# cherubicXN/neat

Measured on AMD Instinct MI355X. Metric: ray-samples/s (train step) on ABC-neat-a, higher is better.
Workload: dtype bf16; 1 GPU; C2: abc-neat-a networks, 1024 rays x 128 samples per GPU, depth samples given, train step = forward + loss + backward + Adam; rays_per_gpu=1024, samples_per_ray=128, global_rays=1024, parallelism=dp1, weights=synthetic 'rough' (seed 42), launch=hip graph replay, the whole step one launch (forward + loss + backward + Adam)

## Files before the change

include/neat_hip.h:

```cpp
#ifndef NEAT_HIP_H
#define NEAT_HIP_H
#include <stddef.h>
#ifdef __cplusplus
extern "C" {
#endif

#define NEAT_NUM_LAYERS 19
#define NEAT_FEATURE 256

typedef struct neat_net_params {
  const float* v[NEAT_NUM_LAYERS];
  const float* g[NEAT_NUM_LAYERS];
  const float* b[NEAT_NUM_LAYERS];
} neat_net_params;

typedef struct neat_net_grads {
  float* dv[NEAT_NUM_LAYERS];
  float* dg[NEAT_NUM_LAYERS];
  float* db[NEAT_NUM_LAYERS];
} neat_net_grads;

int neat_abi_version(void);

#define NEAT_F32 0
#define NEAT_BF16 1
#define NEAT_BF16X3 2
#define NEAT_F16 3
#define NEAT_F16X3 4
#define NEAT_F16X3_FASTVALUES 5

size_t neat_packed_floats(int precision);
int neat_pack_weights(const neat_net_params* net, float* packed, int precision, void* stream);

int neat_camera_rays(const float* uv, const float* pose, const float* K, int kstride, int R, float* dirs, float* origins ,
                     void* stream);
int neat_eik_points(const float* uniform, const float* origins, const float* dirs, const float* z_eik, const float* extra, int R, int J,
                    float* out, const float* z, int S, const long long* idx, void* stream);

size_t neat_sdf_ws_floats(int P, int mode, int precision);
int neat_sdf_forward(const float* packed, const neat_net_params* net, const float* x, int P, int mode, int precision,
                     float radius, float scale, float* ws,
                     float* out257, float* sdf, float* feat, float* grad, void* stream);
int neat_sdf_backward(const float* packed, const neat_net_params* net, float* ws, int P, int precision,
                      const float* d_out257, const float* d_sdf, const float* d_feat, const float* d_grad,
                      const neat_net_grads* grads, void* stream);
int neat_sdf_backward_x(const float* packed, const neat_net_params* net, float* ws, int P, int precision, float scale,
                        const float* d_out257, const float* d_sdf, const float* d_feat, const float* d_grad,
                        const neat_net_grads* grads, float* d_x, void* stream);

size_t neat_heads_ws_floats(int P, int precision);
int neat_heads_forward(const float* packed, const neat_net_params* net, const float* points, const float* normals,
                       const float* view_dirs, const float* feats, int P, int precision, float* ws,
                       float* rgb, float* lines, void* stream);

size_t neat_render_ws_floats(int R, int S, int E, int precision);
int neat_render_forward(const float* packed, const neat_net_params* net, const float* origins, const float* dirs,
                        const float* z, int R, int S, int precision, const float* beta, float beta_min, float radius, float scale, float* ws,
                        float* points, float* weights, float* sdf, float* rgb, float* lines3d, float* depth,
                        float* xyz, float* normal_map, const float* eik_points, int E, float* eik_grad, void* stream);
int neat_render_backward(const float* packed, const neat_net_params* net, float* ws, const float* dirs,
                         const float* z, int R, int S, int E, int precision, const float* beta, float beta_min,
                         const float* d_rgb, const float* d_lines3d, const float* d_depth, const float* d_xyz,
                         const float* d_eik_grad, const float* d_acc, const neat_net_grads* grads, float* dbeta_ray, float* dbeta, void* stream);

size_t neat_render_eval_ws_floats(int R, int S, int precision);
int neat_render_forward_eval(const float* packed, const neat_net_params* net, const float* origins, const float* dirs,
                             const float* z, int R, int S, int precision, const float* beta, float beta_min, float radius, float scale, float* ws,
                             float* points, float* weights, float* sdf, float* rgb, float* lines3d, float* depth,
                             float* xyz, float* normal_map, void* stream);

int neat_uniform_depths(const float* near_r, float near_s, const float* far_r, float far_s, const float* t, const float* rnd, int R, int N,
                        float* z, void* stream);

int neat_sample_pdf(const float* bins, const float* weights, int nb, int R, const float* u, int u_stride, int N, float* samples,
                    const float* z_merge, int nz, float* z_out, void* stream);

int neat_sampler_bound(const float* z, int n, int R, const float* sdf_old, const float* sdf_new, const int* order, int n_old,
                       const float* beta_in, const float* beta0, float eps, int iters, float* sdf_out, float* beta_out,
                       int* flag, void* stream);
int neat_sampler_resample(const float* z, const float* sdf, int n, int R, const float* beta, int refine, float add_tiny,
                          const float* u, int u_stride, int N, float* samples, float* z_merged, int* order, void* stream);
int neat_sampler_finish(const float* samples, int N, const float* z, int n, const int* pick, int n_extra, float near, float far,
                        int R, const int* eik_idx, float* z_vals, float* z_eik, void* stream);

int neat_sdf_values_gated(const float* packed, const neat_net_params* net, const float* x, int P, int precision, float radius,
                          float scale, float* ws, float* sdf, const int* gate, int gate_value, void* stream);
int neat_sdf_values_rays(const float* packed, const neat_net_params* net, const float* origins, const float* dirs, const float* z, int R,
                         int S, int precision, float radius, float scale, float* ws, float* sdf, const int* gate, int gate_value,
                         void* stream);
int neat_sampler_init(const float* z, int R, int n, const float* beta, float beta_min, float beta_c, float* beta0, float* beta_ray,
                      int* ctl, int nctl, void* stream);
int neat_sampler_bound_dev(const float* z, int n, int R, const float* sdf_old, const float* sdf_new, const int* order, int n_old,
                           const float* beta_in, const float* beta0, float eps, int iters, float* sdf_out, float* beta_out,
                           int* open, const int* gate, int gate_value, void* stream);
int neat_sampler_resample_dev(const float* z, const float* sdf, int n, int R, const float* beta, float add_tiny,
                              const float* u_refine, int N_refine, float* samples_refine, float* z_merged, int* order,
                              const float* u_final, int u_final_stride, int N_final, float* samples_final, float* z_final, int ld_final,
                              int* n_final, const int* open, int* cont, int round, int max_rounds, void* stream);
int neat_sampler_finish_dev(const float* samples, int N, const float* z_final, int ld_final, const int* n_final, const float* keys,
                            int n_extra, int* pick, float near, float far, int R, const int* eik_idx, float* z_vals, float* z_eik,
                            void* stream);

int neat_sdf_ldp(int P, int precision);
int neat_sdf_values_laid_out(const float* packed, const neat_net_params* net, int P, int precision, float radius, float scale, float* ws,
                             float* sdf, const int* gate, int gate_value, void* stream);
int neat_sampler_init_rays(const float* z, int R, int n, const float* beta, float beta_min, float beta_c, float* beta0, float* beta_ray,
                           int* ctl, int nctl, const float* origins, const float* dirs, float* x_fm, int ldp, const float* keys, int n_step,
                           int n_cand, int n_extra, int* pick_all, void* stream);
int neat_sampler_round(const float* z, int n, int R, const float* sdf_old, const float* sdf_new, const int* order, int n_old,
                       const float* beta_in, const float* beta0, float eps, int iters, float* sdf_out, float* beta_out, int* ctl, int round,
                       int max_rounds, float add_tiny, const float* u_refine, int N_refine, float* samples_refine, float* z_merged,
                       int* order_out, const float* origins, const float* dirs, float* x_fm, int ldp, const float* u_final,
                       int u_final_stride, int N_final, float* samples_final, float* z_final, int ld_final, void* stream);
int neat_sampler_finish_picked(const float* samples, int N, const float* z_final, int ld_final, const int* n_final, const int* pick_all,
                               int n_step, int n_extra, float near, float far, int R, const int* eik_idx, float* z_vals, float* z_eik,
                               void* stream);

int neat_encode_lines(const float* lines, int N, int H, int W, float* lmap, int* label, unsigned char* valid, void* stream);

int neat_gather_batch(const int* pool, int npool, const long long* draw, int n, int W, const float* att, const float* rgb, const int* labels,
                      const float* lines, int nlines, float* uv, float* uv_proj, float* rgb_out, float* lines_out, long long* labels_out,
                      long long* pixel_out, void* stream);

int neat_copy_batch(const void* const* src, void* const* dst, const long long* nbytes, int n, void* stream);

int neat_l3d(const float* x, const float* o, const float* d, const float* normal, int R, float* l3d, void* stream);
int neat_junction_cost(const float* cand2d, const float* gt2d, int V, int C, float* cost, void* stream);
int neat_junction_gate(const long long* rows, const long long* cols, int K, const float* cost, int C, const float* cand3d,
                       const float* cand2d, const float* cand2d_calib, int use_median, float* median, unsigned char* good, float* j3d,
                       float* j2d, float* j2d_calib, void* stream);
int neat_loss_terms(const float* rgb, const float* rgb_gt, int R, const float* gtheta, int E, const float* loc3, const float* loc2c, int K,
                    const float* glo3, const float* glo2c, int J, float* scal, float* d_rgb, float* d_gtheta, float* pair_cost,
                    float eik_grad_scale, void* stream);
int neat_loss_lines_terms(const float* pred_px, const float* pred_calib, const float* gt5, const float* Kmat, int L, float threshold, float* out3,
                          float* d_pred_calib, float grad_scale, const float* rgb, const float* rgb_gt, int R, const float* gtheta, int E,
                          const float* loc3, const float* loc2c, int K, const float* glo3, const float* glo2c, int J, float* scal, float* d_rgb,
                          float* d_gtheta, float* pair_cost, float eik_grad_scale, const float* w2c, const float* lines3d, float* d_lines3d,
                          void* stream);
int neat_loss_pairs(const long long* ri, const long long* ci, const int* n_match, int Kmax, const float* loc3, const float* loc2c,
                    const float* loc2, const float* glo3, const float* glo2c, const float* glo2, int J, const float* pair_cost, float* scal,
                    float* d_glo3, float* d_glo2c, const float* line_loss, float w_eik, float w_line, float w_j3, float w_j2, int weighted_grads,
                    float* total, const float* w2c, void* stream);
int neat_ffn_forward(const float* x, int J, const float* W0, const float* b0, const float* W1, const float* b1, const float* W2,
                     const float* b2, float* h1, float* h2, float* y, void* stream);
int neat_ffn_backward(const float* x, int J, const float* W0, const float* W1, const float* W2, const float* h1, const float* h2,
                      const float* dy, float* ws2, float* dx, float* dW0, float* db0, float* dW1, float* db1, float* dW2, float* db2,
                      void* stream);
int neat_inv_small(const float* A, int n, int lda, float* out, void* stream);
int neat_camera_mats(const float* pose, const float* K, int kstride, float* w2c, float* K3, void* stream);
int neat_project2d(const float* K, const float* w2c, const float* X, int N, float* uv, void* stream);
int neat_project2d_backward(const float* K, const float* w2c, const float* X, int N, const float* d_uv, float* d_X, void* stream);
int neat_camera_setup(const float* uv, const float* uv2, const float* pose, const float* K, int kstride, int R, float* dirs, float* origins,
                      float* dirs2, float* w2c, float* K3, void* stream);
int neat_project2d_pair(const float* K, const float* K2, const float* w2c, const float* X, int N, float* uv, float* uv2, void* stream);
int neat_line_loss(const float* pred, const float* gt, const float* weight, int R, float threshold, float* out2, float* per_line,
                   float* d_pred, void* stream);
int neat_line_losses(const float* pred_px, const float* pred_calib, const float* gt5, const float* K, int R, float threshold, float* out3,
                     float* d_pred_calib, float grad_scale, void* stream);

int neat_adam_step(float* params, const float* const* grads, const long long* seg_offsets, const int* seg_steps, int nseg,
                   float* exp_avg, float* exp_avg_sq, float lr, float beta1, float beta2, float eps, void* stream);
int neat_adam_step_coef(float* params, const float* const* grads, const long long* seg_offsets, int nseg, float* exp_avg, float* exp_avg_sq,
                        const float* coef, float beta1, float beta2, float eps, void* stream);

size_t neat_lsap_ws_bytes(int nr, int nc);
int neat_lsap(const float* cost, int nr, int nc, const unsigned char* row_mask, const unsigned char* col_mask, long long* row_ind,
              long long* col_ind, int* n_match, void* ws, void* stream);

size_t neat_dbscan_ws_bytes(int n);
int neat_dbscan_means(const float* points, int n, double eps, float* centres, unsigned char* valid, int* count, void* ws, void* stream);

int neat_parse_match(const float* lines2d, int n, const float* gt, int m, int gt_stride, float threshold, int* label, float* mindis,
                     void* stream);
size_t neat_parse_group_ws_bytes(int n, int m);
int neat_parse_group(const int* label, const float* lines3d, const float* l3d, int n, int m, float* lines, float* scores, int* count,
                     void* ws, void* stream);
size_t neat_parse_vote_ws_bytes(int J, int mcap);
int neat_parse_vote(const float* junctions, int J, const float* lines, const int* count, int mcap, float threshold, int view, int* votes,
                    int* first, void* ws, void* stream);
size_t neat_parse_graph_ws_bytes(int V, int mcap, int J);
int neat_parse_graph(const float* vlines, const float* vscores, const int* vcount, int V, int mcap, float score_threshold,
                     const float* junctions, const int* votes, const int* first, int J, float* lines_out, float* junc_out,
                     unsigned char* graph, int* pairs, float* wfi, int ecap, int* counts, void* ws, void* stream);
size_t neat_parse_visibility_ws_bytes(int ecap, int V);
int neat_parse_visibility(const float* lines, const int* n_lines, int ecap, const float* gt, int gt_stride, const int* gt_off,
                          const float* K3, const float* w2c, int V, float ckdist, int ckview, int* vis_count, float* checked,
                          int* n_checked, void* ws, void* stream);

int neat_grid_points(float* x_fm, int ldp, long long first_node, int count, const int* n, const double* b0, const double* b1, void* stream);
size_t neat_mesh_ws_bytes(int nx, int ny, int nz);
int neat_mesh_count(const float* grid, int nx, int ny, int nz, float level, void* ws, int* counts, void* stream);
int neat_mesh_emit(const float* grid, int nx, int ny, int nz, const double* b0, const double* b1, float level, void* ws, float* verts, int nv,
                   int* faces, int nf, void* stream);
int neat_unit_rows3(float* g, int n, void* stream);

int neat_volume_weights(const float* z, const float* sdf, int R, int S, const float* beta, float* weights, void* stream);

int neat_set_tuning(int key, int value);
int neat_prof_enable(int on);
int neat_prof_collect(int cls, double* total_ms, double* total_flops, int* launches, double* total_bytes);

#ifdef __cplusplus
}
#endif
#endif
```

neat_amd/_lib.py:

```python
import ctypes
import os

NUM_LAYERS = 19
ABI_VERSION = 15
PRECISIONS = {"fp32": 0, "bf16": 1, "bf16x3": 2, "fp16": 3, "fp16x3": 4}
_HERE = os.path.dirname(os.path.abspath(__file__))
LIB_PATH = os.environ.get("NEAT_HIP_LIB") or os.path.join(_HERE, "csrc", "libneat_hip.so")

c_fp = ctypes.c_void_p


class NetParams(ctypes.Structure):
    _fields_ = [("v", c_fp * NUM_LAYERS), ("g", c_fp * NUM_LAYERS), ("b", c_fp * NUM_LAYERS)]


class NetGrads(ctypes.Structure):
    _fields_ = [("dv", c_fp * NUM_LAYERS), ("dg", c_fp * NUM_LAYERS), ("db", c_fp * NUM_LAYERS)]


_SIGNATURES = {
    "neat_abi_version": (ctypes.c_int, []),
    "neat_packed_floats": (ctypes.c_size_t, [ctypes.c_int]),
    "neat_pack_weights": (ctypes.c_int, [ctypes.POINTER(NetParams), c_fp, ctypes.c_int, c_fp]),
    "neat_eik_points": (ctypes.c_int, [c_fp, c_fp, c_fp, c_fp, c_fp, ctypes.c_int, ctypes.c_int, c_fp, c_fp, ctypes.c_int, c_fp, c_fp]),
    "neat_camera_rays": (ctypes.c_int, [c_fp, c_fp, c_fp, ctypes.c_int, ctypes.c_int, c_fp, c_fp, c_fp]),
    "neat_sdf_ws_floats": (ctypes.c_size_t, [ctypes.c_int, ctypes.c_int, ctypes.c_int]),
    "neat_sdf_forward": (ctypes.c_int, [c_fp, ctypes.POINTER(NetParams), c_fp, ctypes.c_int, ctypes.c_int, ctypes.c_int,
                                        ctypes.c_float, ctypes.c_float, c_fp, c_fp, c_fp, c_fp, c_fp, c_fp]),
    "neat_sdf_backward": (ctypes.c_int, [c_fp, ctypes.POINTER(NetParams), c_fp, ctypes.c_int, ctypes.c_int, c_fp, c_fp, c_fp, c_fp,
                                         ctypes.POINTER(NetGrads), c_fp]),
    "neat_sdf_backward_x": (ctypes.c_int, [c_fp, ctypes.POINTER(NetParams), c_fp, ctypes.c_int, ctypes.c_int, ctypes.c_float, c_fp, c_fp,
                                           c_fp, c_fp, ctypes.POINTER(NetGrads), c_fp, c_fp]),
    "neat_heads_ws_floats": (ctypes.c_size_t, [ctypes.c_int, ctypes.c_int]),
    "neat_heads_forward": (ctypes.c_int, [c_fp, ctypes.POINTER(NetParams), c_fp, c_fp, c_fp, c_fp, ctypes.c_int, ctypes.c_int, c_fp,
                                          c_fp, c_fp, c_fp]),
    "neat_render_ws_floats": (ctypes.c_size_t, [ctypes.c_int, ctypes.c_int, ctypes.c_int, ctypes.c_int]),
    "neat_render_forward": (ctypes.c_int, [c_fp, ctypes.POINTER(NetParams), c_fp, c_fp, c_fp, ctypes.c_int, ctypes.c_int, ctypes.c_int,
                                           c_fp, ctypes.c_float, ctypes.c_float, ctypes.c_float, c_fp,
                                           c_fp, c_fp, c_fp, c_fp, c_fp, c_fp, c_fp, c_fp, c_fp, ctypes.c_int, c_fp, c_fp]),
    "neat_render_eval_ws_floats": (ctypes.c_size_t, [ctypes.c_int, ctypes.c_int, ctypes.c_int]),
    "neat_render_forward_eval": (ctypes.c_int, [c_fp, ctypes.POINTER(NetParams), c_fp, c_fp, c_fp, ctypes.c_int, ctypes.c_int, ctypes.c_int,
                                                c_fp, ctypes.c_float, ctypes.c_float, ctypes.c_float, c_fp,
                                                c_fp, c_fp, c_fp, c_fp, c_fp, c_fp, c_fp, c_fp, c_fp]),
    "neat_render_backward": (ctypes.c_int, [c_fp, ctypes.POINTER(NetParams), c_fp, c_fp, c_fp, ctypes.c_int, ctypes.c_int, ctypes.c_int,
                                            ctypes.c_int, c_fp, ctypes.c_float, c_fp, c_fp, c_fp, c_fp, c_fp, c_fp, ctypes.POINTER(NetGrads), c_fp, c_fp,
                                            c_fp]),
    "neat_sampler_bound": (ctypes.c_int, [c_fp, ctypes.c_int, ctypes.c_int, c_fp, c_fp, c_fp, ctypes.c_int, c_fp, c_fp,
                                          ctypes.c_float, ctypes.c_int, c_fp, c_fp, c_fp, c_fp]),
    "neat_sampler_resample": (ctypes.c_int, [c_fp, c_fp, ctypes.c_int, ctypes.c_int, c_fp, ctypes.c_int, ctypes.c_float,
                                             c_fp, ctypes.c_int, ctypes.c_int, c_fp, c_fp, c_fp, c_fp]),
    "neat_sampler_finish": (ctypes.c_int, [c_fp, ctypes.c_int, c_fp, ctypes.c_int, c_fp, ctypes.c_int, ctypes.c_float,
                                           ctypes.c_float, ctypes.c_int, c_fp, c_fp, c_fp, c_fp]),
    "neat_sample_pdf": (ctypes.c_int, [c_fp, c_fp, ctypes.c_int, ctypes.c_int, c_fp, ctypes.c_int, ctypes.c_int, c_fp, c_fp, ctypes.c_int, c_fp, c_fp]),
    "neat_uniform_depths": (ctypes.c_int, [c_fp, ctypes.c_float, c_fp, ctypes.c_float, c_fp, c_fp, ctypes.c_int, ctypes.c_int, c_fp, c_fp]),
    "neat_sdf_values_gated": (ctypes.c_int, [c_fp, ctypes.POINTER(NetParams), c_fp, ctypes.c_int, ctypes.c_int, ctypes.c_float,
                                             ctypes.c_float, c_fp, c_fp, c_fp, ctypes.c_int, c_fp]),
    "neat_sdf_values_rays": (ctypes.c_int, [c_fp, ctypes.POINTER(NetParams), c_fp, c_fp, c_fp, ctypes.c_int, ctypes.c_int, ctypes.c_int,
                                            ctypes.c_float, ctypes.c_float, c_fp, c_fp, c_fp, ctypes.c_int, c_fp]),
    "neat_sampler_init": (ctypes.c_int, [c_fp, ctypes.c_int, ctypes.c_int, c_fp, ctypes.c_float, ctypes.c_float, c_fp, c_fp, c_fp, ctypes.c_int,
                                         c_fp]),
    "neat_sampler_bound_dev": (ctypes.c_int, [c_fp, ctypes.c_int, ctypes.c_int, c_fp, c_fp, c_fp, ctypes.c_int, c_fp, c_fp,
                                              ctypes.c_float, ctypes.c_int, c_fp, c_fp, c_fp, c_fp, ctypes.c_int, c_fp]),
    "neat_sampler_resample_dev": (ctypes.c_int, [c_fp, c_fp, ctypes.c_int, ctypes.c_int, c_fp, ctypes.c_float,
                                                 c_fp, ctypes.c_int, c_fp, c_fp, c_fp,
                                                 c_fp, ctypes.c_int, ctypes.c_int, c_fp, c_fp, ctypes.c_int,
                                                 c_fp, c_fp, c_fp, ctypes.c_int, ctypes.c_int, c_fp]),
    "neat_sampler_finish_dev": (ctypes.c_int, [c_fp, ctypes.c_int, c_fp, ctypes.c_int, c_fp, c_fp, ctypes.c_int, c_fp, ctypes.c_float,
                                               ctypes.c_float, ctypes.c_int, c_fp, c_fp, c_fp, c_fp]),
    "neat_sdf_ldp": (ctypes.c_int, [ctypes.c_int, ctypes.c_int]),
    "neat_adam_step_coef": (ctypes.c_int, [c_fp, ctypes.POINTER(ctypes.c_void_p), ctypes.POINTER(ctypes.c_longlong), ctypes.c_int, c_fp, c_fp,
                                           c_fp, ctypes.c_float, ctypes.c_float, ctypes.c_float, c_fp]),
    "neat_loss_lines_terms": (ctypes.c_int, [c_fp, c_fp, c_fp, c_fp, ctypes.c_int, ctypes.c_float, c_fp, c_fp, ctypes.c_float,
                                             c_fp, c_fp, ctypes.c_int, c_fp, ctypes.c_int, c_fp, c_fp, ctypes.c_int, c_fp, c_fp, ctypes.c_int,
                                             c_fp, c_fp, c_fp, c_fp, ctypes.c_float, c_fp, c_fp, c_fp, c_fp]),
    "neat_camera_setup": (ctypes.c_int, [c_fp, c_fp, c_fp, c_fp, ctypes.c_int, ctypes.c_int, c_fp, c_fp, c_fp, c_fp, c_fp, c_fp]),
    "neat_project2d_pair": (ctypes.c_int, [c_fp, c_fp, c_fp, c_fp, ctypes.c_int, c_fp, c_fp, c_fp]),
    "neat_sdf_values_laid_out": (ctypes.c_int, [c_fp, ctypes.POINTER(NetParams), ctypes.c_int, ctypes.c_int, ctypes.c_float, ctypes.c_float, c_fp, c_fp, c_fp, ctypes.c_int, c_fp]),
    "neat_sampler_init_rays": (ctypes.c_int, [c_fp, ctypes.c_int, ctypes.c_int, c_fp, ctypes.c_float, ctypes.c_float, c_fp, c_fp, c_fp, ctypes.c_int, c_fp, c_fp, c_fp, ctypes.c_int, c_fp, ctypes.c_int, ctypes.c_int, ctypes.c_int, c_fp, c_fp]),
    "neat_sampler_round": (ctypes.c_int, [c_fp, ctypes.c_int, ctypes.c_int, c_fp, c_fp, c_fp, ctypes.c_int, c_fp, c_fp, ctypes.c_float, ctypes.c_int, c_fp, c_fp, c_fp, ctypes.c_int, ctypes.c_int, ctypes.c_float, c_fp, ctypes.c_int, c_fp, c_fp, c_fp, c_fp, c_fp, c_fp, ctypes.c_int, c_fp, ctypes.c_int, ctypes.c_int, c_fp, c_fp, ctypes.c_int, c_fp]),
    "neat_sampler_finish_picked": (ctypes.c_int, [c_fp, ctypes.c_int, c_fp, ctypes.c_int, c_fp, c_fp, ctypes.c_int, ctypes.c_int, ctypes.c_float, ctypes.c_float, ctypes.c_int, c_fp, c_fp, c_fp, c_fp]),
    "neat_encode_lines": (ctypes.c_int, [c_fp, ctypes.c_int, ctypes.c_int, ctypes.c_int, c_fp, c_fp, c_fp, c_fp]),
    "neat_gather_batch": (ctypes.c_int, [c_fp, ctypes.c_int, c_fp, ctypes.c_int, ctypes.c_int, c_fp, c_fp, c_fp, c_fp, ctypes.c_int,
                                         c_fp, c_fp, c_fp, c_fp, c_fp, c_fp, c_fp]),
    "neat_copy_batch": (ctypes.c_int, [c_fp, c_fp, c_fp, ctypes.c_int, c_fp]),
    "neat_ffn_forward": (ctypes.c_int, [c_fp, ctypes.c_int] + [c_fp] * 10),
    "neat_ffn_backward": (ctypes.c_int, [c_fp, ctypes.c_int] + [c_fp] * 15),
    "neat_l3d": (ctypes.c_int, [c_fp, c_fp, c_fp, c_fp, ctypes.c_int, c_fp, c_fp]),
    "neat_junction_cost": (ctypes.c_int, [c_fp, c_fp, ctypes.c_int, ctypes.c_int, c_fp, c_fp]),
    "neat_junction_gate": (ctypes.c_int, [c_fp, c_fp, ctypes.c_int, c_fp, ctypes.c_int, c_fp, c_fp, c_fp, ctypes.c_int, c_fp, c_fp, c_fp,
                                          c_fp, c_fp, c_fp]),
    "neat_loss_terms": (ctypes.c_int, [c_fp, c_fp, ctypes.c_int, c_fp, ctypes.c_int, c_fp, c_fp, ctypes.c_int, c_fp, c_fp, ctypes.c_int,
                                       c_fp, c_fp, c_fp, c_fp, ctypes.c_float, c_fp]),
    "neat_loss_pairs": (ctypes.c_int, [c_fp, c_fp, c_fp, ctypes.c_int, c_fp, c_fp, c_fp, c_fp, c_fp, c_fp, ctypes.c_int, c_fp, c_fp, c_fp,
                                       c_fp, c_fp, ctypes.c_float, ctypes.c_float, ctypes.c_float, ctypes.c_float, ctypes.c_int, c_fp, c_fp, c_fp]),
    "neat_camera_mats": (ctypes.c_int, [c_fp, c_fp, ctypes.c_int, c_fp, c_fp, c_fp]),
    "neat_inv_small": (ctypes.c_int, [c_fp, ctypes.c_int, ctypes.c_int, c_fp, c_fp]),
    "neat_project2d": (ctypes.c_int, [c_fp, c_fp, c_fp, ctypes.c_int, c_fp, c_fp]),
    "neat_project2d_backward": (ctypes.c_int, [c_fp, c_fp, c_fp, ctypes.c_int, c_fp, c_fp, c_fp]),
    "neat_line_loss": (ctypes.c_int, [c_fp, c_fp, c_fp, ctypes.c_int, ctypes.c_float, c_fp, c_fp, c_fp, c_fp]),
    "neat_line_losses": (ctypes.c_int, [c_fp, c_fp, c_fp, c_fp, ctypes.c_int, ctypes.c_float, c_fp, c_fp, ctypes.c_float, c_fp]),
    "neat_adam_step": (ctypes.c_int, [c_fp, ctypes.POINTER(ctypes.c_void_p), ctypes.POINTER(ctypes.c_longlong), ctypes.POINTER(ctypes.c_int),
                                      ctypes.c_int, c_fp, c_fp, ctypes.c_float, ctypes.c_float, ctypes.c_float, ctypes.c_float, c_fp]),
    "neat_lsap_ws_bytes": (ctypes.c_size_t, [ctypes.c_int, ctypes.c_int]),
    "neat_lsap": (ctypes.c_int, [c_fp, ctypes.c_int, ctypes.c_int, c_fp, c_fp, c_fp, c_fp, c_fp, c_fp, c_fp]),
    "neat_dbscan_ws_bytes": (ctypes.c_size_t, [ctypes.c_int]),
    "neat_dbscan_means": (ctypes.c_int, [c_fp, ctypes.c_int, ctypes.c_double, c_fp, c_fp, c_fp, c_fp, c_fp]),
    "neat_parse_match": (ctypes.c_int, [c_fp, ctypes.c_int, c_fp, ctypes.c_int, ctypes.c_int, ctypes.c_float, c_fp, c_fp, c_fp]),
    "neat_parse_group_ws_bytes": (ctypes.c_size_t, [ctypes.c_int, ctypes.c_int]),
    "neat_parse_group": (ctypes.c_int, [c_fp, c_fp, c_fp, ctypes.c_int, ctypes.c_int, c_fp, c_fp, c_fp, c_fp, c_fp]),
    "neat_parse_vote_ws_bytes": (ctypes.c_size_t, [ctypes.c_int, ctypes.c_int]),
    "neat_parse_vote": (ctypes.c_int, [c_fp, ctypes.c_int, c_fp, c_fp, ctypes.c_int, ctypes.c_float, ctypes.c_int, c_fp, c_fp, c_fp, c_fp]),
    "neat_parse_graph_ws_bytes": (ctypes.c_size_t, [ctypes.c_int, ctypes.c_int, ctypes.c_int]),
    "neat_parse_graph": (ctypes.c_int, [c_fp, c_fp, c_fp, ctypes.c_int, ctypes.c_int, ctypes.c_float, c_fp, c_fp, c_fp, ctypes.c_int,
                                        c_fp, c_fp, c_fp, c_fp, c_fp, ctypes.c_int, c_fp, c_fp, c_fp]),
    "neat_parse_visibility_ws_bytes": (ctypes.c_size_t, [ctypes.c_int, ctypes.c_int]),
    "neat_parse_visibility": (ctypes.c_int, [c_fp, c_fp, ctypes.c_int, c_fp, ctypes.c_int, c_fp, c_fp, c_fp, ctypes.c_int, ctypes.c_float,
                                             ctypes.c_int, c_fp, c_fp, c_fp, c_fp, c_fp]),
    "neat_grid_points": (ctypes.c_int, [c_fp, ctypes.c_int, ctypes.c_longlong, ctypes.c_int, ctypes.POINTER(ctypes.c_int),
                                        ctypes.POINTER(ctypes.c_double), ctypes.POINTER(ctypes.c_double), c_fp]),
    "neat_mesh_ws_bytes": (ctypes.c_size_t, [ctypes.c_int, ctypes.c_int, ctypes.c_int]),
    "neat_mesh_count": (ctypes.c_int, [c_fp, ctypes.c_int, ctypes.c_int, ctypes.c_int, ctypes.c_float, c_fp, c_fp, c_fp]),
    "neat_mesh_emit": (ctypes.c_int, [c_fp, ctypes.c_int, ctypes.c_int, ctypes.c_int, ctypes.POINTER(ctypes.c_double),
                                      ctypes.POINTER(ctypes.c_double), ctypes.c_float, c_fp, c_fp, ctypes.c_int, c_fp, ctypes.c_int, c_fp]),
    "neat_unit_rows3": (ctypes.c_int, [c_fp, ctypes.c_int, c_fp]),
    "neat_volume_weights": (ctypes.c_int, [c_fp, c_fp, ctypes.c_int, ctypes.c_int, c_fp, c_fp, c_fp]),
    "neat_set_tuning": (ctypes.c_int, [ctypes.c_int, ctypes.c_int]),
    "neat_prof_enable": (ctypes.c_int, [ctypes.c_int]),
    "neat_prof_collect": (ctypes.c_int, [ctypes.c_int, ctypes.POINTER(ctypes.c_double), ctypes.POINTER(ctypes.c_double),
                                         ctypes.POINTER(ctypes.c_int), ctypes.POINTER(ctypes.c_double)]),
}

_lib = None


def exported_symbols():
    return sorted(_SIGNATURES)


tuning_overrides = []


def lib():
    global _lib
    if _lib is None:
        if not os.path.exists(LIB_PATH):
            raise RuntimeError(
                f"{LIB_PATH} is missing: build it with `python -c 'import __graft_entry__ as g; g.build()'` "
                "(or neat_amd/csrc/build.sh).  neat_amd has no CPU/PyTorch fallback for the hot path.")
        l = ctypes.CDLL(LIB_PATH)
        for name, (res, args) in _SIGNATURES.items():
            fn = getattr(l, name)
            fn.restype, fn.argtypes = res, args
        _lib = l
        applied = []
        for kv in filter(None, os.environ.get("NEAT_TUNING", "").split(",")):
            k, v = kv.split("=")
            check(l.neat_set_tuning(int(k), int(v)), f"NEAT_TUNING {kv}")
            applied.append(kv)
        if applied:
            import sys
            print(f"[neat_amd] NEAT_TUNING overrides applied: {','.join(applied)}", file=sys.stderr, flush=True)
        global tuning_overrides
        tuning_overrides = applied
    return _lib


def check(code, what):
    if code != 0:
        raise RuntimeError(f"libneat_hip: {what} failed with code {code}")
```

neat_amd/csrc/kernels_junction.hpp:

```cpp
#pragma once
#include <hip/hip_runtime.h>
#include "device_util.hpp"

namespace neat {

constexpr int LSAP_WG = 1024;

struct LsapArgs {
  const float* cost;
  int nr, nc;
  const unsigned char* row_mask;
  long long* row_ind;
  long long* col_ind;
  int* n_match;
  double* wsd;
  int* wsi;
  int use_lds, lds_int_off;
  const unsigned char* col_mask;
  int cost_lds_off;
};

struct LsapKey { double val; int it; int un; };

__device__ __forceinline__ bool lsap_better(const LsapKey& a, const LsapKey& b) {
  if (a.it < 0) return false;
  if (b.it < 0) return true;
  if (a.val != b.val) return a.val < b.val;
  if (a.un != b.un) return a.un > b.un;
  return a.un ? a.it > b.it : a.it < b.it;
}

__device__ __forceinline__ LsapKey lsap_shfl_xor(const LsapKey& k, int m) {
  LsapKey o;
  o.val = __shfl_xor(k.val, m);
  o.it = __shfl_xor(k.it, m);
  o.un = __shfl_xor(k.un, m);
  return o;
}

template <class F>
__device__ int lsap_compact(int n, F flag, int* out, int* s_wave, int* s_base) {
  const int tid = threadIdx.x, lane = tid & 63, wave = tid >> 6, nw = blockDim.x >> 6;
  if (tid == 0) *s_base = 0;
  __syncthreads();
  for (int b0 = 0; b0 < n; b0 += blockDim.x) {
    const int i = b0 + tid;
    const bool f = i < n && flag(i);
    const unsigned long long bal = __ballot(f);
    const int before = __popcll(bal & ((1ull << lane) - 1ull));
    if (lane == 0) s_wave[wave] = __popcll(bal);
    __syncthreads();
    int off = *s_base;
    for (int w = 0; w < wave; ++w) off += s_wave[w];
    if (f) out[off + before] = i;
    __syncthreads();
    if (tid == 0) { int t = 0; for (int w = 0; w < nw; ++w) t += s_wave[w]; *s_base += t; }
    __syncthreads();
  }
  const int total = *s_base;
  __syncthreads();
  return total;
}

__global__ __launch_bounds__(LSAP_WG) void lsap_kernel(LsapArgs a) {
  __shared__ int s_wave[LSAP_WG / 64], s_base;
  __shared__ LsapKey s_key[LSAP_WG / 64];
  __shared__ int s_i, s_nrem, s_fail, s_done, s_nvis;
  __shared__ double s_minval;
  const int tid = threadIdx.x, nt = blockDim.x, lane = tid & 63, wave = tid >> 6, nw = nt >> 6;
  const int kmax = min(a.nr, a.nc);
  for (int k = tid; k < kmax; k += nt) { a.row_ind[k] = -1; a.col_ind[k] = -1; }

  extern __shared__ __attribute__((aligned(16))) unsigned char lsap_lds[];
  double* wsd = a.use_lds ? reinterpret_cast<double*>(lsap_lds) : a.wsd;
  int* wsi = a.use_lds ? reinterpret_cast<int*>(lsap_lds + a.lds_int_off) : a.wsi;
  int* rowlist = wsi;
  int* collist = rowlist + a.nr;
  const unsigned char* mask = a.row_mask;
  const unsigned char* cmask = a.col_mask;
  int n_eff, c_eff;
  if (!mask && !cmask) {
    for (int i = tid; i < a.nr; i += nt) rowlist[i] = i;
    for (int j = tid; j < a.nc; j += nt) collist[j] = j;
    n_eff = a.nr; c_eff = a.nc;
  } else {
    n_eff = lsap_compact(a.nr, [&](int i) { return mask ? mask[i] != 0 : true; }, rowlist, s_wave, &s_base);
    c_eff = lsap_compact(a.nc, [&](int j) { return cmask ? cmask[j] != 0 : true; }, collist, s_wave, &s_base);
  }
  const bool T = c_eff < n_eff;
  const int N = T ? c_eff : n_eff, M = T ? n_eff : c_eff;
  if (N == 0) { if (tid == 0) *a.n_match = 0; return; }
  double* u = wsd; double* v = u + N; double* sp = v + M;
  int* path = collist + a.nc; int* col4row = path + M; int* row4col = col4row + N; int* remaining = row4col + M;
  int* vis_row = remaining + M;
  int* vis_col = vis_row + N;
  int* tmp = vis_col + M;
  const float* C = a.cost;
  const int nc0 = a.nc;
  const bool staged = a.use_lds && a.cost_lds_off >= 0;
  const float* Cl = reinterpret_cast<const float*>(lsap_lds + (staged ? a.cost_lds_off : 0));
  if (staged) {
    float* dst = reinterpret_cast<float*>(lsap_lds + a.cost_lds_off);
    const int total = a.nr * a.nc;
    const int total4 = ((reinterpret_cast<size_t>(C) & 15) == 0) ? (total >> 2) : 0;
    const float4* C4 = reinterpret_cast<const float4*>(C);
    float4* d4 = reinterpret_cast<float4*>(dst);
    for (int e = tid; e < total4; e += 4 * nt) {
      float4 x[4];
#pragma unroll
      for (int q = 0; q < 4; ++q) if (e + q * nt < total4) x[q] = C4[e + q * nt];
#pragma unroll
      for (int q = 0; q < 4; ++q) if (e + q * nt < total4) d4[e + q * nt] = x[q];
    }
    for (int e = 4 * total4 + tid; e < total; e += nt) dst[e] = C[e];
  }
  const bool ident = !mask && !cmask;
  auto cost = [&](int i, int j) -> double {
    const int idx = ident ? (T ? j * nc0 + i : i * nc0 + j) : (T ? rowlist[j] * nc0 + collist[i] : rowlist[i] * nc0 + collist[j]);
    return (double)(staged ? Cl[idx] : C[idx]);
  };
  for (int i = tid; i < N; i += nt) { u[i] = 0.0; col4row[i] = -1; }
  for (int j = tid; j < M; j += nt) { v[j] = 0.0; row4col[j] = -1; }
  if (tid == 0) { s_fail = 0; s_done = 0; s_i = 0; s_nrem = M; s_minval = 0.0; s_nvis = 0; }
  __syncthreads();

  for (int cur = 0; cur < N; ++cur) {
    bool first = true;
    while (true) {
      const int i = s_i, nrem = s_nrem;
      const double minval = s_minval, ui = u[i];
      LsapKey best{INFINITY, -1, 0};
      if (first) {
        for (int it = tid; it < M; it += nt) {
          const int j = M - 1 - it;
          const double r = minval + cost(i, j) - ui - v[j];
          const bool lower = r < INFINITY;
          const double spj = lower ? r : INFINITY;
          sp[j] = spj;
          if (lower) path[j] = i;
          remaining[it] = j;
          LsapKey k{spj, it, row4col[j] == -1 ? 1 : 0};
          if (spj < INFINITY && lsap_better(k, best)) best = k;
        }
        first = false;
      } else {
        for (int it = tid; it < nrem; it += nt) {
          const int j = remaining[it];
          const double r = minval + cost(i, j) - ui - v[j];
          double spj = sp[j];
          if (r < spj) { path[j] = i; sp[j] = r; spj = r; }
          LsapKey k{spj, it, row4col[j] == -1 ? 1 : 0};
          if (spj < INFINITY && lsap_better(k, best)) best = k;
        }
      }
      for (int m = 32; m >= 1; m >>= 1) {
        LsapKey o = lsap_shfl_xor(best, m);
        if (lsap_better(o, best)) best = o;
      }
      if (lane == 0) s_key[wave] = best;
      __syncthreads();
      if (tid == 0) {
        LsapKey b = s_key[0];
        for (int w = 1; w < nw; ++w) if (lsap_better(s_key[w], b)) b = s_key[w];
        int nvis = s_nvis;
        vis_row[nvis] = i;
        if (b.it < 0) { s_fail = 1; s_done = N; }
        else {
          const double mv = b.val;
          const int j = remaining[b.it];
          vis_col[nvis] = j;
          ++nvis;
          remaining[b.it] = remaining[nrem - 1];
          if (row4col[j] != -1) { s_i = row4col[j]; s_minval = mv; s_nrem = nrem - 1; s_nvis = nvis; }
          else {
            for (int q = 0; q < nvis; ++q) {
              const int r_ = vis_row[q];
              if (r_ == cur) u[r_] += mv;
              else u[r_] += mv - sp[col4row[r_]];
            }
            for (int q = 0; q < nvis; ++q) { const int c_ = vis_col[q]; v[c_] -= mv - sp[c_]; }
            int jj = j;
            while (true) {
              const int ii = path[jj];
              row4col[jj] = ii;
              const int t = col4row[ii]; col4row[ii] = jj; jj = t;
              if (ii == cur) break;
            }
            s_done = cur + 1; s_i = cur + 1; s_nrem = M; s_minval = 0.0; s_nvis = 0;
          }
        }
      }
      __syncthreads();
      if (s_done > cur) break;
    }
    if (s_fail) break;
  }
  if (s_fail) { if (tid == 0) *a.n_match = -1; return; }
  if (!T) {
    for (int i = tid; i < N; i += nt) { a.row_ind[i] = rowlist[i]; a.col_ind[i] = collist[col4row[i]]; }
  } else {
    const int cnt = lsap_compact(M, [&](int k) { return row4col[k] != -1; }, tmp, s_wave, &s_base);
    for (int q = tid; q < cnt; q += nt) { const int k = tmp[q]; a.row_ind[q] = rowlist[k]; a.col_ind[q] = collist[row4col[k]]; }
  }
  if (tid == 0) *a.n_match = N;
}

#ifndef NEAT_ADAM_PASSES
#define NEAT_ADAM_PASSES 1
#endif
constexpr int ADAM_MAXSEG = 96, ADAM_PASSES = NEAT_ADAM_PASSES;
struct AdamSegs {
  const float* g[ADAM_MAXSEG]; long long off[ADAM_MAXSEG + 1]; float lr_over_bc1[ADAM_MAXSEG], inv_sqrt_bc2[ADAM_MAXSEG]; int nseg;
};

constexpr int ADAM_SEGS_KERNARG_OFFSET = 8;
__global__ void adam_flat_kernel(float* __restrict__ p, AdamSegs segs, float* __restrict__ m, float* __restrict__ v,
                                 long long n, float beta1, float beta2, float eps, const float* __restrict__ coef) {
  __shared__ long long s_off[ADAM_MAXSEG + 1];
  __shared__ const float* s_g[ADAM_MAXSEG];
  __shared__ float s_a1[ADAM_MAXSEG], s_a2[ADAM_MAXSEG];
  typedef const __attribute__((address_space(4))) char* karg_ptr;
  typedef const __attribute__((address_space(4))) AdamSegs* karg_segs;
  const karg_segs tab = (karg_segs)((karg_ptr)__builtin_amdgcn_kernarg_segment_ptr() + ADAM_SEGS_KERNARG_OFFSET);
  for (int t = threadIdx.x; t <= segs.nseg; t += blockDim.x) {
    s_off[t] = tab->off[t];
    if (t < segs.nseg) { s_g[t] = tab->g[t]; s_a1[t] = coef ? coef[2 * t] : tab->lr_over_bc1[t]; s_a2[t] = coef ? coef[2 * t + 1] : tab->inv_sqrt_bc2[t]; }
  }
  __syncthreads();
  for (int pass = 0; pass < ADAM_PASSES; ++pass) {
    const long long i0 = (((long long)blockIdx.x * ADAM_PASSES + pass) * blockDim.x + threadIdx.x) * 4;
    if (i0 >= n) return;
    int lo = 0, hi = segs.nseg - 1;
    while (lo < hi) { const int mid = (lo + hi + 1) >> 1; if (s_off[mid] <= i0) lo = mid; else hi = mid - 1; }
    const long long iend = i0 + 4 < n ? i0 + 4 : n;
    if (iend <= s_off[lo + 1] && iend == i0 + 4) {
      const float* gp = s_g[lo];
      if (!gp) continue;
      const float a1 = s_a1[lo], a2 = s_a2[lo];
      const float* gq = gp + (i0 - s_off[lo]);
      float4 mm = *reinterpret_cast<const float4*>(m + i0), vv = *reinterpret_cast<const float4*>(v + i0), pp = *reinterpret_cast<const float4*>(p + i0);
      float* me = reinterpret_cast<float*>(&mm); float* ve = reinterpret_cast<float*>(&vv); float* pe = reinterpret_cast<float*>(&pp);
      float ge[4];
      if ((reinterpret_cast<size_t>(gq) & 15) == 0) {
        const float4 g4 = *reinterpret_cast<const float4*>(gq);
        ge[0] = g4.x; ge[1] = g4.y; ge[2] = g4.z; ge[3] = g4.w;
      } else {
#pragma unroll
        for (int e = 0; e < 4; ++e) ge[e] = gq[e];
      }
#pragma unroll
      for (int e = 0; e < 4; ++e) {
        const float g = ge[e];
        me[e] = beta1 * me[e] + (1.0f - beta1) * g;
        ve[e] = beta2 * ve[e] + (1.0f - beta2) * g * g;
        pe[e] -= a1 * (me[e] / (sqrtf(ve[e]) * a2 + eps));
      }
      *reinterpret_cast<float4*>(m + i0) = mm; *reinterpret_cast<float4*>(v + i0) = vv; *reinterpret_cast<float4*>(p + i0) = pp;
      continue;
    }
    for (long long i = i0; i < iend; ++i) {
      while (i >= s_off[lo + 1]) ++lo;
      const float* gp = s_g[lo];
      if (!gp) continue;
      const float g = gp[i - s_off[lo]];
      const float mm = beta1 * m[i] + (1.0f - beta1) * g;
      const float vv = beta2 * v[i] + (1.0f - beta2) * g * g;
      m[i] = mm; v[i] = vv;
      p[i] -= s_a1[lo] * (mm / (sqrtf(vv) * s_a2[lo] + eps));
    }
  }
}

__device__ __forceinline__ void project_point(const float* K, const float* M, const float x[3], float cam[3], float& w) {
  float c[3];
#pragma unroll
  for (int i = 0; i < 3; ++i) c[i] = M[4 * i] * x[0] + M[4 * i + 1] * x[1] + M[4 * i + 2] * x[2] + M[4 * i + 3];
#pragma unroll
  for (int i = 0; i < 3; ++i) cam[i] = K[3 * i] * c[0] + K[3 * i + 1] * c[1] + K[3 * i + 2] * c[2];
  w = cam[2];
  if (fabsf(w) < 1e-8f) w += (w >= 0.0f) ? 1e-8f : -1e-8f;
}

__global__ void project2d_kernel(const float* __restrict__ K, const float* __restrict__ w2c, const float* __restrict__ X, int N,
                                 float* __restrict__ uv) {
  const int i = blockIdx.x * blockDim.x + threadIdx.x;
  if (i >= N) return;
  const float x[3] = {X[3 * i], X[3 * i + 1], X[3 * i + 2]};
  float cam[3], w;
  project_point(K, w2c, x, cam, w);
  uv[2 * i] = cam[0] / w; uv[2 * i + 1] = cam[1] / w;
}

__global__ void project2d_pair_kernel(const float* __restrict__ K, const float* __restrict__ K2, const float* __restrict__ w2c,
                                      const float* __restrict__ X, int N, float* __restrict__ uv, float* __restrict__ uv2) {
  const int i = blockIdx.x * blockDim.x + threadIdx.x;
  if (i >= N) return;
  const float x[3] = {X[3 * i], X[3 * i + 1], X[3 * i + 2]};
  float cam[3], w;
  project_point(K, w2c, x, cam, w);
  uv[2 * i] = cam[0] / w; uv[2 * i + 1] = cam[1] / w;
  project_point(K2, w2c, x, cam, w);
  uv2[2 * i] = cam[0] / w; uv2[2 * i + 1] = cam[1] / w;
}

__device__ __forceinline__ void project_bwd_point(const float* K, const float* w2c, const float x[3], float du, float dv, float dX[3]) {
  float cam[3], w;
  project_point(K, w2c, x, cam, w);
  const float dcam[3] = {du / w, dv / w, -(du * (cam[0] / w) + dv * (cam[1] / w)) / w};
  float dc[3];
#pragma unroll
  for (int j = 0; j < 3; ++j) dc[j] = K[j] * dcam[0] + K[3 + j] * dcam[1] + K[6 + j] * dcam[2];
#pragma unroll
  for (int j = 0; j < 3; ++j) dX[j] = w2c[j] * dc[0] + w2c[4 + j] * dc[1] + w2c[8 + j] * dc[2];
}
__global__ void project2d_bwd_kernel(const float* __restrict__ K, const float* __restrict__ w2c, const float* __restrict__ X, int N,
                                     const float* __restrict__ d_uv, float* __restrict__ d_X) {
  const int i = blockIdx.x * blockDim.x + threadIdx.x;
  if (i >= N) return;
  const float x[3] = {X[3 * i], X[3 * i + 1], X[3 * i + 2]};
  float dX[3];
  project_bwd_point(K, w2c, x, d_uv[2 * i], d_uv[2 * i + 1], dX);
#pragma unroll
  for (int j = 0; j < 3; ++j) d_X[3 * i + j] = dX[j];
}
__device__ __forceinline__ void project_bwd_calib(const float* w2c, const float x[3], float du, float dv, float dX[3]) {
  float I3[9] = {1.0f, 0.0f, 0.0f, 0.0f, 1.0f, 0.0f, 0.0f, 0.0f, 1.0f};
#pragma unroll
  for (int k = 0; k < 9; ++k) asm volatile("" : "+v"(I3[k]));
  project_bwd_point(I3, w2c, x, du, dv, dX);
}

__global__ __launch_bounds__(1024) void line_loss_kernel(const float* __restrict__ pred, const float* __restrict__ gt,
                                                         const float* __restrict__ weight, int R, float thr, float* __restrict__ out,
                                                         float* __restrict__ per_line, float* __restrict__ d_pred) {
  __shared__ float s_sum[16], s_cnt[16];
  __shared__ float s_inv;
  const int tid = threadIdx.x, lane = tid & 63, wave = tid >> 6;
  float sum = 0.0f, cnt = 0.0f;
  for (int r = tid; r < R; r += blockDim.x) {
    float p[4], g[4];
#pragma unroll
    for (int c = 0; c < 4; ++c) { p[c] = pred[4 * r + c]; g[c] = gt[4 * r + c]; }
    float ds = 0.0f, df = 0.0f;
#pragma unroll
    for (int c = 0; c < 4; ++c) { const float a = p[c] - g[c], b = p[c] - g[c ^ 2]; ds += a * a; df += b * b; }
    const bool straight = ds < df;
    float l = 0.0f;
#pragma unroll
    for (int c = 0; c < 4; ++c) l += fabsf(p[c] - (straight ? g[c] : g[c ^ 2]));
    l *= 0.25f;
    per_line[r] = l;
    if (l < thr) { sum += l * weight[r]; cnt += 1.0f; }
  }
  sum = wave_sum(sum); cnt = wave_sum(cnt);
  if (lane == 0) { s_sum[wave] = sum; s_cnt[wave] = cnt; }
  __syncthreads();
  if (tid == 0) {
    float a = 0.0f, b = 0.0f;
    for (int w = 0; w < (int)(blockDim.x >> 6); ++w) { a += s_sum[w]; b += s_cnt[w]; }
// ... 543 lines not shown
  __shared__ int lab[DBSCAN_MAXN];
  __shared__ int s_wave[16], s_base;
  const int tid = threadIdx.x, nt = blockDim.x;
  for (int i = tid; i < n; i += nt) lab[i] = dbscan_find(parent, i);
  const int maxc = n / 2;
  for (int k = tid; k < maxc; k += nt) { valid[k] = 0; centres[3 * k] = 0.f; centres[3 * k + 1] = 0.f; centres[3 * k + 2] = 0.f; }
  int* replist = reinterpret_cast<int*>(centres + 3 * maxc);
  if (tid == 0) s_base = 0;
  __syncthreads();
  const int lane = tid & 63, wave = tid >> 6, nw = nt >> 6;
  for (int b0 = 0; b0 < n; b0 += nt) {
    const int i = b0 + tid;
    const bool f = i < n && lab[i] == i && has_nb[i] != 0;
    const unsigned long long bal = __ballot(f);
    const int before = __popcll(bal & ((1ull << lane) - 1ull));
    if (lane == 0) s_wave[wave] = __popcll(bal);
    __syncthreads();
    int off = s_base;
    for (int w = 0; w < wave; ++w) off += s_wave[w];
    if (f) replist[off + before] = i;
    __syncthreads();
    if (tid == 0) { int t = 0; for (int w = 0; w < nw; ++w) t += s_wave[w]; s_base += t; }
    __syncthreads();
  }
  const int nclu = s_base;
  extern __shared__ __attribute__((aligned(8))) unsigned char dbscan_dyn[];
  if (mode == 2) {
    long long* sx = reinterpret_cast<long long*>(dbscan_dyn);
    long long* sy = sx + maxc; long long* sz = sy + maxc;
    int* cnt = reinterpret_cast<int*>(sz + maxc);
    int* rank = cnt + maxc;
    for (int k = tid; k < nclu; k += nt) { sx[k] = 0; sy[k] = 0; sz[k] = 0; cnt[k] = 0; rank[replist[k]] = k; }
    __syncthreads();
    for (int j = tid; j < n; j += nt) {
      if (has_nb[j] == 0) continue;
      const int k = rank[lab[j]];
      atomicAdd(reinterpret_cast<unsigned long long*>(&sx[k]), (unsigned long long)__double2ll_rn((double)pts[3 * j] * 4294967296.0));
      atomicAdd(reinterpret_cast<unsigned long long*>(&sy[k]), (unsigned long long)__double2ll_rn((double)pts[3 * j + 1] * 4294967296.0));
      atomicAdd(reinterpret_cast<unsigned long long*>(&sz[k]), (unsigned long long)__double2ll_rn((double)pts[3 * j + 2] * 4294967296.0));
      atomicAdd(&cnt[k], 1);
    }
    __syncthreads();
    for (int k = tid; k < nclu; k += nt) {
      const double inv = 1.0 / (4294967296.0 * (double)cnt[k]);
      centres[3 * k] = (float)((double)sx[k] * inv); centres[3 * k + 1] = (float)((double)sy[k] * inv); centres[3 * k + 2] = (float)((double)sz[k] * inv);
      valid[k] = 1;
    }
    if (tid == 0) *count = nclu;
    return;
  }
  float* dbscan_pts = reinterpret_cast<float*>(dbscan_dyn);
  const float* P = pts;
  if (mode == 1) {
    for (int i = tid; i < 3 * n; i += nt) dbscan_pts[i] = pts[i];
    P = dbscan_pts;
  }
  __syncthreads();
  for (int k = wave; k < nclu; k += nw) {
    const int r = replist[k];
    float sx = 0.f, sy = 0.f, sz = 0.f; int cnt = 0;
    for (int j = r + lane; j < n; j += 64) {
      const bool m = lab[j] == r;
      sx += m ? P[3 * j] : 0.0f; sy += m ? P[3 * j + 1] : 0.0f; sz += m ? P[3 * j + 2] : 0.0f; cnt += m ? 1 : 0;
    }
#pragma unroll
    for (int off = 32; off > 0; off >>= 1) {
      sx += __shfl_xor(sx, off); sy += __shfl_xor(sy, off); sz += __shfl_xor(sz, off); cnt += __shfl_xor(cnt, off);
    }
    if (lane == 0) {
      const float inv = 1.0f / (float)cnt;
      centres[3 * k] = sx * inv; centres[3 * k + 1] = sy * inv; centres[3 * k + 2] = sz * inv;
      valid[k] = 1;
    }
  }
  if (tid == 0) *count = nclu;
}

__device__ __forceinline__ float block_sum(float v, float* s_red) {
  v = wave_sum(v);
  const int lane = threadIdx.x & 63, wave = threadIdx.x >> 6;
  __syncthreads();
  if (lane == 0) s_red[wave] = v;
  __syncthreads();
  float t = 0.0f;
  for (int w = 0; w < (int)(blockDim.x >> 6); ++w) t += s_red[w];
  return t;
}

struct LossTermsArgs {
  const float* rgb; const float* rgb_gt; int R;
  const float* gtheta; int E;
  const float* loc3; const float* loc2c; int K;
  const float* glo3; const float* glo2c; int J;
  float* scal;
  float* d_rgb; float* d_gtheta; float* pair_cost;
  float eik_grad_scale;
};

__device__ __forceinline__ void loss_terms_body(const LossTermsArgs& a) {
  __shared__ float s_red[16];
  const int tid = threadIdx.x, nt = blockDim.x;
  float acc = 0.0f;
  const float inv_rgb = 1.0f / (float)(3 * a.R);
  for (int i = tid; i < 3 * a.R; i += nt) {
    const float d = a.rgb[i] - a.rgb_gt[i];
    acc += fabsf(d);
    a.d_rgb[i] = (d > 0.0f ? 1.0f : (d < 0.0f ? -1.0f : 0.0f)) * inv_rgb;
  }
  const float rgb_loss = block_sum(acc, s_red) * inv_rgb;
  acc = 0.0f;
  const float inv_e = a.E > 0 ? 1.0f / (float)a.E : 0.0f;
  for (int i = tid; i < a.E; i += nt) {
    const float gx = a.gtheta[3 * i], gy = a.gtheta[3 * i + 1], gz = a.gtheta[3 * i + 2];
    const float nrm = sqrtf(gx * gx + gy * gy + gz * gz);
    acc += (nrm - 1.0f) * (nrm - 1.0f);
    const float c = nrm > 0.0f ? (2.0f * (nrm - 1.0f) * inv_e / nrm) * a.eik_grad_scale : 0.0f;
    a.d_gtheta[3 * i] = c * gx; a.d_gtheta[3 * i + 1] = c * gy; a.d_gtheta[3 * i + 2] = c * gz;
  }
  const float eik = block_sum(acc, s_red) * inv_e;
  if (tid == 0) { a.scal[0] = rgb_loss; a.scal[1] = eik; }
  for (int idx = tid; idx < a.K * a.J; idx += nt) {
    const int k = idx / a.J, j = idx % a.J;
    float c3 = 0.0f, c2 = 0.0f;
#pragma unroll
    for (int c = 0; c < 3; ++c) c3 += fabsf(a.loc3[3 * k + c] - a.glo3[3 * j + c]);
#pragma unroll
    for (int c = 0; c < 2; ++c) c2 += fabsf(a.loc2c[2 * k + c] - a.glo2c[2 * j + c]);
    a.pair_cost[idx] = c3 + 0.1f * c2;
  }
}

__global__ __launch_bounds__(1024) void loss_terms_kernel(LossTermsArgs a) { loss_terms_body(a); }

struct LineLossesArgs { const float* pred_u; const float* pred_c; const float* gt5; const float* K; int R; float thr; float* out; float* d_pred_c; float grad_scale;
                        const float* w2c; const float* X3; float* d_X3; };
__global__ __launch_bounds__(1024) void loss_lines_terms_kernel(LineLossesArgs l, LossTermsArgs t) {
  if (blockIdx.x == 0) line_losses_body(l.pred_u, l.pred_c, l.gt5, l.K, l.R, l.thr, l.out, l.d_pred_c, l.grad_scale, l.w2c, l.X3, l.d_X3);
  else loss_terms_body(t);
}

struct LossPairsArgs {
  const long long* ri; const long long* ci; const int* n_match; int Kmax;
  const float* loc3; const float* loc2c; const float* loc2;
  const float* glo3; const float* glo2c; const float* glo2; int J;
  const float* pair_cost;
  float* scal;
  float* d_glo3; float* d_glo2c;
  const float* line_loss; float w_eik, w_line, w_j3, w_j2;
  int weighted_grads;
  float* total;
  const float* w2c;
};

__global__ __launch_bounds__(1024) void loss_pairs_kernel(LossPairsArgs a) {
  __shared__ float s_red[16];
  const int tid = threadIdx.x, nt = blockDim.x;
  for (int i = tid; i < 3 * a.J; i += nt) a.d_glo3[i] = 0.0f;
  for (int i = tid; i < 2 * a.J; i += nt) a.d_glo2c[i] = 0.0f;
  __syncthreads();
  const int n = max(*a.n_match, 0);
  const float inv = 1.0f / (float)max(n, 1);
  const float g3 = a.weighted_grads ? a.w_j3 : 1.0f, g2 = a.weighted_grads ? a.w_j2 : 1.0f;
  float s3 = 0.0f, s2 = 0.0f, spx = 0.0f, cnt = 0.0f;
  for (int q = tid; q < a.Kmax; q += nt) {
    const long long r = a.ri[q], c = a.ci[q];
    if (r < 0 || c < 0 || q >= n) continue;
#pragma unroll
    for (int e = 0; e < 3; ++e) {
      const float d = a.loc3[3 * r + e] - a.glo3[3 * c + e];
      s3 += fabsf(d);
      a.d_glo3[3 * c + e] = (-(d > 0.0f ? 1.0f : (d < 0.0f ? -1.0f : 0.0f)) * inv) * g3;
    }
#pragma unroll
    for (int e = 0; e < 2; ++e) {
      const float d = a.loc2c[2 * r + e] - a.glo2c[2 * c + e];
      s2 += fabsf(d);
      a.d_glo2c[2 * c + e] = (-(d > 0.0f ? 1.0f : (d < 0.0f ? -1.0f : 0.0f)) * inv) * g2;
      spx += fabsf(a.loc2[2 * r + e] - a.glo2[2 * c + e]);
    }
    if (a.pair_cost[r * a.J + c] < 10.0f) cnt += 1.0f;
  }
  s3 = block_sum(s3, s_red); s2 = block_sum(s2, s_red); spx = block_sum(spx, s_red); cnt = block_sum(cnt, s_red);
  if (a.w2c) {
    for (int j = tid; j < a.J; j += nt) {
      const float x[3] = {a.glo3[3 * j], a.glo3[3 * j + 1], a.glo3[3 * j + 2]};
      float dX[3];
      project_bwd_calib(a.w2c, x, a.d_glo2c[2 * j], a.d_glo2c[2 * j + 1], dX);
#pragma unroll
      for (int e = 0; e < 3; ++e) a.d_glo3[3 * j + e] += dX[e];
    }
  }
  if (tid == 0) {
    a.scal[2] = s3 * inv; a.scal[3] = s2 * inv; a.scal[4] = spx * inv; a.scal[5] = cnt;
    const float tot = a.scal[0] + a.w_eik * a.scal[1] + a.w_line * a.line_loss[0] + a.w_j3 * (s3 * inv) + a.w_j2 * (s2 * inv);
    a.scal[6] = tot;
    if (a.total) a.total[0] = tot;
  }
}

__global__ void l3d_kernel(const float* __restrict__ x, const float* __restrict__ o, const float* __restrict__ d,
                           const float* __restrict__ nrm, int R, float* __restrict__ l3d) {
  const int r = blockIdx.x * blockDim.x + threadIdx.x;
  if (r >= R) return;
  float den = 0.0f, num = 0.0f;
#pragma unroll
  for (int c = 0; c < 3; ++c) { den += d[3 * r + c] * nrm[3 * r + c]; num += (x[3 * r + c] - o[3 * r + c]) * nrm[3 * r + c]; }
  den += den >= 0.0f ? 1e-6f : -1e-6f;
  const float t = num / den;
#pragma unroll
  for (int c = 0; c < 3; ++c) l3d[3 * r + c] = o[3 * r + c] + d[3 * r + c] * t;
}

__global__ void junction_cost_kernel(const float* __restrict__ cand2d, const float* __restrict__ gt2d, int V, int C, float* __restrict__ cost) {
  const int idx = blockIdx.x * blockDim.x + threadIdx.x;
  if (idx >= V * C) return;
  const int v = idx / C, c = idx % C;
  const float dx = cand2d[2 * c] - gt2d[2 * v], dy = cand2d[2 * c + 1] - gt2d[2 * v + 1];
  cost[idx] = __fsqrt_rn(__fadd_rn(__fmul_rn(dx, dx), __fmul_rn(dy, dy)));
}

struct JunctionGateArgs {
  const long long* rows; const long long* cols; int K;
  const float* cost; int C;
  const float* cand3d; const float* cand2d; const float* cand2dc;
  int use_median;
  float* median;
  unsigned char* good;
  float* j3d; float* j2d; float* j2dc;
};

__global__ __launch_bounds__(1024) void junction_gate_kernel(JunctionGateArgs a) {
  __shared__ float s_m[2048];
  __shared__ int s_n;
  __shared__ float s_med;
  const int tid = threadIdx.x, nt = blockDim.x;
  if (tid == 0) { s_n = 0; s_med = 10.0f; }
  __syncthreads();
  for (int k = tid; k < a.K; k += nt) {
    const long long r = a.rows[k], c = a.cols[k];
    const bool ok = r >= 0 && c >= 0;
    s_m[k] = ok ? a.cost[r * a.C + c] : NAN;
    if (ok) atomicAdd(&s_n, 1);
  }
  __syncthreads();
  const int n = s_n;
  if (a.use_median && n > 0) {
    const int want = (n - 1) / 2;
    for (int k = tid; k < a.K; k += nt) {
      const float v = s_m[k];
      if (v != v) continue;
      int rank = 0;
      for (int j = 0; j < a.K; ++j) { const float w = s_m[j]; if (w == w && (w < v || (w == v && j < k))) ++rank; }
      if (rank == want) s_med = v;
    }
  }
  __syncthreads();
  const float thr = a.use_median ? s_med : 10.0f;
  if (tid == 0 && a.use_median) a.median[0] = s_med;
  for (int k = tid; k < a.K; k += nt) {
    const float v = s_m[k];
    const bool ok = v == v;
    a.good[k] = (ok && v < thr) ? 1 : 0;
    const long long c = ok ? a.cols[k] : 0;
#pragma unroll
    for (int e = 0; e < 3; ++e) a.j3d[3 * k + e] = ok ? a.cand3d[3 * c + e] : 0.0f;
#pragma unroll
    for (int e = 0; e < 2; ++e) { a.j2d[2 * k + e] = ok ? a.cand2d[2 * c + e] : 0.0f; a.j2dc[2 * k + e] = ok ? a.cand2dc[2 * c + e] : 0.0f; }
  }
}

}
```

neat_amd/csrc/neat_aux.hip:

```cpp
#include "kernels_sampler.hpp"
#include "kernels_junction.hpp"
#include "kernels_parse.hpp"
#include "kernels_mesh.hpp"
#include "../../include/neat_hip.h"
#include <algorithm>
#include <cmath>
#include <limits.h>
#include <math.h>

using namespace neat;

__attribute__((visibility("hidden"))) int neat_aux_set_tuning(int key, int value);

namespace {

int g_ffn_mfma = 1;
int g_sampler_ablate = 0;

#define NEAT_CHECK(expr) do { hipError_t e_ = (expr); if (e_ != hipSuccess) return (int)e_; } while (0)
inline dim3 grid1(int n, int b = 256) { return dim3((n + b - 1) / b); }

__global__ void volume_weights_kernel(const float* __restrict__ z, const float* __restrict__ sdf, int R, int S,
                                      const float* __restrict__ beta_ptr, float* __restrict__ weights) {
  const float beta = *beta_ptr;
  const int lane = threadIdx.x & 63;
  const int r = blockIdx.x * 4 + (threadIdx.x >> 6);
  if (r >= R) return;
  float carry = 0.0f;
  for (int i0 = 0; i0 < S; i0 += 64) {
    const int i = i0 + lane;
    const bool ok = i < S;
    const int p = r * S + (ok ? i : S - 1);
    const float delta = (i + 1 < S) ? z[p + 1] - z[p] : 1e10f;
    const float e = ok ? delta * laplace_sigma(sdf[p], beta) : 0.0f;
    const float incl = wave_incl_scan(e, lane);
    float excl = __shfl_up(incl, 1);
    if (lane == 0) excl = 0.0f;
    if (ok) weights[p] = (1.0f - expf(-e)) * expf(-(carry + excl));
    carry += __shfl(incl, 63);
  }
}

}

int neat_aux_set_tuning(int key, int value) {
  if (key == 28 && (value == 0 || value == 1)) { g_ffn_mfma = value; return 0; }
  if (key == 30 && value >= 0 && value <= 7) { g_sampler_ablate = value; return 0; }
  return -1;
}

extern "C" {

int neat_camera_rays(const float* uv, const float* pose, const float* K, int kstride, int R, float* dirs, float* origins, void* stream) {
  if (R <= 0) return 0;
  hipLaunchKernelGGL(camera_rays_kernel, grid1(R), dim3(256), 0, (hipStream_t)stream, uv, pose, K, kstride, R, dirs, origins);
  return (int)hipGetLastError();
}

int neat_eik_points(const float* uniform, const float* origins, const float* dirs, const float* z_eik, const float* extra, int R, int J,
                    float* out, const float* z, int S, const long long* idx, void* stream) {
  if (R <= 0 || J < 0) return R == 0 && J == 0 ? 0 : -1;
  if (!uniform || !origins || !dirs || !out || (J > 0 && !extra)) return -1;
  if (!z_eik && (!z || !idx || S <= 0)) return -1;
  hipLaunchKernelGGL(eik_points_kernel, grid1((2 * R + J) * 3), dim3(256), 0, (hipStream_t)stream, uniform, origins, dirs, z_eik, extra, R, J, out,
                     z, S, idx);
  return (int)hipGetLastError();
}

int neat_sampler_bound(const float* z, int n, int R, const float* sdf_old, const float* sdf_new, const int* order, int n_old,
                       const float* beta_in, const float* beta0, float eps, int iters, float* sdf_out, float* beta_out,
                       int* flag, void* stream) {
  if (R <= 0) return 0;
  if (n < 2 || n > SMAX || !z || !sdf_new || !beta_in || !beta0 || !sdf_out || !beta_out || !flag) return -1;
  SamplerBoundArgs a{z, n, R, sdf_old, sdf_new, order, n_old, beta_in, beta0, eps, iters, sdf_out, beta_out, flag, nullptr, 0};
  hipLaunchKernelGGL(sampler_bound_kernel, dim3(R), dim3(BOUND_T), 0, (hipStream_t)stream, a);
  return (int)hipGetLastError();
}

int neat_sampler_resample(const float* z, const float* sdf, int n, int R, const float* beta, int refine, float add_tiny,
                          const float* u, int u_stride, int N, float* samples, float* z_merged, int* order, void* stream) {
  if (R <= 0) return 0;
  if (n < 2 || n > SMAX || N < 1 || N > SMAX || !z || !sdf || !beta || !u || !samples || (refine && (!z_merged || !order))) return -1;
  SamplerResampleArgs a{};
  a.z = z; a.sdf = sdf; a.n = n; a.R = R; a.beta = beta; a.refine = refine; a.add_tiny = add_tiny; a.u = u; a.u_stride = u_stride; a.N = N;
  a.samples = samples; a.z_merged = z_merged; a.order = order;
  hipLaunchKernelGGL(sampler_resample_kernel, dim3(R), dim3(BOUND_T), 0, (hipStream_t)stream, a);
  return (int)hipGetLastError();
}

int neat_sampler_finish(const float* samples, int N, const float* z, int n, const int* pick, int n_extra, float near, float far,
                        int R, const int* eik_idx, float* z_vals, float* z_eik, void* stream) {
  if (R <= 0) return 0;
  if (N + 2 + n_extra > SMAX || !samples || !z || (n_extra > 0 && !pick) || !eik_idx || !z_vals || !z_eik) return -1;
  SamplerFinishArgs a{samples, N, z, n, pick, n_extra, near, far, R, eik_idx, z_vals, z_eik, n};
  hipLaunchKernelGGL(sampler_finish_kernel, dim3(R), dim3(64), 0, (hipStream_t)stream, a);
  return (int)hipGetLastError();
}

int neat_sample_pdf(const float* bins, const float* weights, int nb, int R, const float* u, int u_stride, int N, float* samples,
                    const float* z_merge, int nz, float* z_out, void* stream) {
  if (R <= 0) return 0;
  if (nb < 2 || nb > SMAX || N < 1 || N > SMAX || !bins || !weights || !u || !samples || (z_merge && (!z_out || nz < 0 || nz + N > SMAX))) return -1;
  SamplePdfArgs a{bins, weights, nb, R, u, u_stride, N, samples, z_merge, nz, z_out};
  hipLaunchKernelGGL(sample_pdf_kernel, dim3(R), dim3(64), 0, (hipStream_t)stream, a);
  return (int)hipGetLastError();
}

int neat_uniform_depths(const float* near_r, float near_s, const float* far_r, float far_s, const float* t, const float* rnd, int R, int N,
                        float* z, void* stream) {
  if (R <= 0 || N <= 0) return 0;
  if (!t || !z) return -1;
  hipLaunchKernelGGL(uniform_depths_kernel, dim3((R * N + 255) / 256), dim3(256), 0, (hipStream_t)stream, near_r, near_s, far_r, far_s, t, rnd, R, N, z);
  return (int)hipGetLastError();
}

int neat_sampler_init(const float* z, int R, int n, const float* beta, float beta_min, float beta_c, float* beta0, float* beta_ray,
                      int* ctl, int nctl, void* stream) {
  return neat_sampler_init_rays(z, R, n, beta, beta_min, beta_c, beta0, beta_ray, ctl, nctl, nullptr, nullptr, nullptr, 0, nullptr, 0, 0, 0,
                                nullptr, stream);
}

int neat_sampler_init_rays(const float* z, int R, int n, const float* beta, float beta_min, float beta_c, float* beta0, float* beta_ray,
                           int* ctl, int nctl, const float* origins, const float* dirs, float* x_fm, int ldp, const float* keys, int n_step,
                           int n_cand, int n_extra, int* pick_all, void* stream) {
  if (R <= 0 || n < 2 || n > SMAX || !z || !beta || !beta0 || !beta_ray || nctl < 0 || (nctl > 0 && !ctl)) return -1;
  if (x_fm && (!origins || !dirs || (long long)ldp < (long long)R * n)) return -1;
  const bool picks = keys != nullptr;
  if (picks && (!pick_all || n_step < 1 || n_cand < 1 || n_extra < 2 || n_extra > n_step || n_step * n_cand > SMAX)) return -1;
  SamplerInitArgs a{z, R, n, beta, beta_min, beta_c, beta0, beta_ray, ctl, nctl, origins, dirs, x_fm, ldp, keys, n_step, n_cand, n_extra, pick_all,
                    (R + 3) / 4, picks ? (n_step * n_cand + 255) / 256 : 0};
  hipLaunchKernelGGL(sampler_init_kernel, dim3(a.init_blocks + n_cand * a.pick_parts), dim3(256), 0, (hipStream_t)stream, a);
  return (int)hipGetLastError();
}

int neat_sampler_round(const float* z, int n, int R, const float* sdf_old, const float* sdf_new, const int* order, int n_old,
                       const float* beta_in, const float* beta0, float eps, int iters, float* sdf_out, float* beta_out, int* ctl, int round,
                       int max_rounds, float add_tiny, const float* u_refine, int N_refine, float* samples_refine, float* z_merged,
                       int* order_out, const float* origins, const float* dirs, float* x_fm, int ldp, const float* u_final,
                       int u_final_stride, int N_final, float* samples_final, float* z_final, int ld_final, void* stream) {
  if (R <= 0) return 0;
  const bool last = round + 1 >= max_rounds;
  if (n < 2 || n > SMAX || !z || !sdf_new || (order && !sdf_old) || !beta_in || !beta0 || !sdf_out || !beta_out || !ctl || round < 0 ||
      round >= max_rounds || N_final < 1 || N_final > SMAX || !u_final || !samples_final || !z_final || ld_final < n) return -1;
  if (!last && (N_refine < 1 || n + N_refine > SMAX || !u_refine || !samples_refine || !z_merged || !order_out ||
                (x_fm && (!origins || !dirs || (long long)ldp < (long long)R * N_refine)))) return -1;
  SamplerRoundArgs a{z, n, R, sdf_old, sdf_new, order, n_old, beta_in, beta0, eps, iters, sdf_out, beta_out, ctl, round, max_rounds, add_tiny,
                     u_refine, N_refine, samples_refine, z_merged, order_out, origins, dirs, x_fm, ldp, u_final, u_final_stride, N_final,
                     samples_final, z_final, ld_final, g_sampler_ablate};
  hipLaunchKernelGGL(sampler_round_kernel, dim3(R), dim3(BOUND_T), 0, (hipStream_t)stream, a);
  return (int)hipGetLastError();
}

int neat_sampler_finish_picked(const float* samples, int N, const float* z_final, int ld_final, const int* n_final, const int* pick_all,
                               int n_step, int n_extra, float near, float far, int R, const int* eik_idx, float* z_vals, float* z_eik,
                               void* stream) {
  if (R <= 0) return 0;
  if (N + 2 + n_extra > SMAX || ld_final > SMAX || !samples || !z_final || !n_final || n_extra == 1 || n_extra < 0 || n_step < 1 || !eik_idx ||
      !z_vals || !z_eik) return -1;
  SamplerFinishArgs a{samples, N, z_final, 0, pick_all, n_extra, near, far, R, eik_idx, z_vals, z_eik, ld_final};
  a.n_final = n_final; a.n_step = n_step;
  hipLaunchKernelGGL(sampler_finish_kernel, dim3(R), dim3(64), 0, (hipStream_t)stream, a);
  return (int)hipGetLastError();
}

int neat_sampler_bound_dev(const float* z, int n, int R, const float* sdf_old, const float* sdf_new, const int* order, int n_old,
                           const float* beta_in, const float* beta0, float eps, int iters, float* sdf_out, float* beta_out,
                           int* open, const int* gate, int gate_value, void* stream) {
  if (R <= 0) return 0;
  if (n < 2 || n > SMAX || !z || !sdf_new || !beta_in || !beta0 || !sdf_out || !beta_out || !open) return -1;
  SamplerBoundArgs a{z, n, R, sdf_old, sdf_new, order, n_old, beta_in, beta0, eps, iters, sdf_out, beta_out, open, gate, gate_value};
  hipLaunchKernelGGL(sampler_bound_kernel, dim3(R), dim3(BOUND_T), 0, (hipStream_t)stream, a);
  return (int)hipGetLastError();
}

int neat_sampler_resample_dev(const float* z, const float* sdf, int n, int R, const float* beta, float add_tiny,
                              const float* u_refine, int N_refine, float* samples_refine, float* z_merged, int* order,
                              const float* u_final, int u_final_stride, int N_final, float* samples_final, float* z_final, int ld_final,
                              int* n_final, const int* open, int* cont, int round, int max_rounds, void* stream) {
  if (R <= 0) return 0;
  if (n < 2 || n > SMAX || N_refine < 1 || N_final < 1 || n + N_refine > SMAX || ld_final < n || !z || !sdf || !beta || !u_refine || !u_final ||
      !samples_refine || !z_merged || !order || !samples_final || !z_final || !n_final || !open || !cont || round < 0 || round >= max_rounds)
    return -1;
  SamplerResampleArgs a{};
  a.z = z; a.sdf = sdf; a.n = n; a.R = R; a.beta = beta; a.refine = 1; a.add_tiny = add_tiny;
  a.u = u_refine; a.u_stride = 0; a.N = N_refine; a.samples = samples_refine; a.z_merged = z_merged; a.order = order;
  a.open = open; a.cont = cont; a.round = round; a.max_rounds = max_rounds;
  a.u_final = u_final; a.u_final_stride = u_final_stride; a.N_final = N_final; a.samples_final = samples_final;
  a.z_final = z_final; a.ld_final = ld_final; a.n_final = n_final;
  hipLaunchKernelGGL(sampler_resample_kernel, dim3(R), dim3(BOUND_T), 0, (hipStream_t)stream, a);
  return (int)hipGetLastError();
}

int neat_sampler_finish_dev(const float* samples, int N, const float* z_final, int ld_final, const int* n_final, const float* keys,
                            int n_extra, int* pick, float near, float far, int R, const int* eik_idx, float* z_vals, float* z_eik,
                            void* stream) {
  if (R <= 0) return 0;
  if (N + 2 + n_extra > SMAX || ld_final > SMAX || !samples || !z_final || !n_final || (n_extra > 0 && !pick) || n_extra == 1 || !eik_idx ||
      !z_vals || !z_eik) return -1;
  if (n_extra > 0) hipLaunchKernelGGL(sampler_pick_kernel, dim3(1), dim3(1024), 0, (hipStream_t)stream, n_final, keys, n_extra, pick);
  SamplerFinishArgs a{samples, N, z_final, 0, pick, n_extra, near, far, R, eik_idx, z_vals, z_eik, ld_final};
// ... 106 lines not shown
  if (!x || !W0 || !W1 || !W2 || !h1 || !h2 || !dy || !ws2 || !dx || !dW0 || !db0 || !dW1 || !db1 || !dW2 || !db2) return -1;
  float* d_a1 = ws2; float* d_a2 = ws2 + (size_t)J * FFN_H;
  hipStream_t st = (hipStream_t)stream;
  if (J > FFN_FUSED_MIN_ROWS)
    hipLaunchKernelGGL(ffn_backward_data_kernel, dim3((J + FFN_RB - 1) / FFN_RB), dim3(FFN_H), 0, st, dy, J, W0, W1, W2, h1, h2, d_a1, d_a2, dx);
  else {
    const dim3 gh((J + FFN_RB - 1) / FFN_RB, FFN_H / 32);
    const float* nobias = nullptr; const float* nogate = nullptr; float* noy2 = nullptr;
    hipLaunchKernelGGL(ffn_dense_kernel<true>, gh, dim3(256), 0, st, dy, J, 3, FFN_H, W2, nobias, h2, 0, d_a2, noy2);
    if (g_ffn_mfma) {
      const dim3 gm((J + 31) / 32, FFN_H / 32);
      hipLaunchKernelGGL(ffn_mfma_kernel<true>, gm, dim3(256), 0, st, (const float*)d_a2, J, W1, nobias, h1, 0, d_a1);
      hipLaunchKernelGGL(ffn_mfma_kernel<true>, gm, dim3(256), 0, st, (const float*)d_a1, J, W0, nobias, nogate, 0, dx);
    } else {
      hipLaunchKernelGGL(ffn_dense_kernel<true>, gh, dim3(256), 0, st, (const float*)d_a2, J, FFN_H, FFN_H, W1, nobias, h1, 0, d_a1, noy2);
      hipLaunchKernelGGL(ffn_dense_kernel<true>, gh, dim3(256), 0, st, (const float*)d_a1, J, FFN_H, FFN_H, W0, nobias, nogate, 0, dx, noy2);
    }
  }
  if (g_ffn_mfma)
    hipLaunchKernelGGL(ffn_wgrad_mfma_kernel, dim3(FFN_H / 32, FFN_H / 32, 3), dim3(64 * FFN_WNW), 0, (hipStream_t)stream, x, h1, h2, d_a1, d_a2, dy, J, dW0, db0,
                       dW1, db1, dW2, db2);
  else
  hipLaunchKernelGGL(ffn_backward_weights_kernel, dim3(FFN_H / FFN_RN, 3), dim3(64 * FFN_JG), 0, (hipStream_t)stream, x, h1, h2, d_a1, d_a2, dy, J, dW0, db0,
                     dW1, db1, dW2, db2);
  return (int)hipGetLastError();
}

int neat_loss_terms(const float* rgb, const float* rgb_gt, int R, const float* gtheta, int E, const float* loc3, const float* loc2c, int K,
                    const float* glo3, const float* glo2c, int J, float* scal, float* d_rgb, float* d_gtheta, float* pair_cost,
                    float eik_grad_scale, void* stream) {
  if (R <= 0 || !rgb || !rgb_gt || !scal || !d_rgb || E < 0 || K < 0 || J < 0) return -1;
  if ((E > 0 && (!gtheta || !d_gtheta)) || (K > 0 && J > 0 && (!loc3 || !loc2c || !glo3 || !glo2c || !pair_cost))) return -1;
  LossTermsArgs a{rgb, rgb_gt, R, gtheta, E, loc3, loc2c, (J > 0 ? K : 0), glo3, glo2c, J, scal, d_rgb, d_gtheta, pair_cost, eik_grad_scale};
  hipLaunchKernelGGL(loss_terms_kernel, dim3(1), dim3(1024), 0, (hipStream_t)stream, a);
  return (int)hipGetLastError();
}

int neat_loss_lines_terms(const float* pred_px, const float* pred_calib, const float* gt5, const float* Kmat, int L, float threshold, float* out3,
                          float* d_pred_calib, float grad_scale, const float* rgb, const float* rgb_gt, int R, const float* gtheta, int E,
                          const float* loc3, const float* loc2c, int K, const float* glo3, const float* glo2c, int J, float* scal, float* d_rgb,
                          float* d_gtheta, float* pair_cost, float eik_grad_scale, const float* w2c, const float* lines3d, float* d_lines3d,
                          void* stream) {
  if (L <= 0 || !pred_px || !pred_calib || !gt5 || !Kmat || !out3 || !d_pred_calib) return -1;
  if (d_lines3d && (!w2c || !lines3d)) return -1;
  if (R <= 0 || !rgb || !rgb_gt || !scal || !d_rgb || E < 0 || K < 0 || J < 0) return -1;
  if ((E > 0 && (!gtheta || !d_gtheta)) || (K > 0 && J > 0 && (!loc3 || !loc2c || !glo3 || !glo2c || !pair_cost))) return -1;
  LineLossesArgs l{pred_px, pred_calib, gt5, Kmat, L, threshold, out3, d_pred_calib, grad_scale, w2c, lines3d, d_lines3d};
  LossTermsArgs a{rgb, rgb_gt, R, gtheta, E, loc3, loc2c, (J > 0 ? K : 0), glo3, glo2c, J, scal, d_rgb, d_gtheta, pair_cost, eik_grad_scale};
  hipLaunchKernelGGL(loss_lines_terms_kernel, dim3(2), dim3(1024), 0, (hipStream_t)stream, l, a);
  return (int)hipGetLastError();
}

int neat_loss_pairs(const long long* ri, const long long* ci, const int* n_match, int Kmax, const float* loc3, const float* loc2c,
                    const float* loc2, const float* glo3, const float* glo2c, const float* glo2, int J, const float* pair_cost, float* scal,
                    float* d_glo3, float* d_glo2c, const float* line_loss, float w_eik, float w_line, float w_j3, float w_j2, int weighted_grads,
                    float* total, const float* w2c, void* stream) {
  if (Kmax < 0 || J <= 0 || !ri || !ci || !n_match || !loc3 || !loc2c || !loc2 || !glo3 || !glo2c || !glo2 || !pair_cost || !scal ||
      !d_glo3 || !d_glo2c || !line_loss) return -1;
  LossPairsArgs a{ri, ci, n_match, Kmax, loc3, loc2c, loc2, glo3, glo2c, glo2, J, pair_cost, scal, d_glo3, d_glo2c, line_loss, w_eik, w_line,
                  w_j3, w_j2, weighted_grads, total, w2c};
  hipLaunchKernelGGL(loss_pairs_kernel, dim3(1), dim3(1024), 0, (hipStream_t)stream, a);
  return (int)hipGetLastError();
}

int neat_l3d(const float* x, const float* o, const float* d, const float* normal, int R, float* l3d, void* stream) {
  if (R <= 0) return 0;
  if (!x || !o || !d || !normal || !l3d) return -1;
  hipLaunchKernelGGL(l3d_kernel, dim3((R + 255) / 256), dim3(256), 0, (hipStream_t)stream, x, o, d, normal, R, l3d);
  return (int)hipGetLastError();
}

int neat_junction_cost(const float* cand2d, const float* gt2d, int V, int C, float* cost, void* stream) {
  if (V <= 0 || C <= 0) return 0;
  if (!cand2d || !gt2d || !cost) return -1;
  hipLaunchKernelGGL(junction_cost_kernel, dim3((V * C + 255) / 256), dim3(256), 0, (hipStream_t)stream, cand2d, gt2d, V, C, cost);
  return (int)hipGetLastError();
}

int neat_junction_gate(const long long* rows, const long long* cols, int K, const float* cost, int C, const float* cand3d,
                       const float* cand2d, const float* cand2d_calib, int use_median, float* median, unsigned char* good, float* j3d,
                       float* j2d, float* j2d_calib, void* stream) {
  if (K <= 0) return 0;
  if (K > 2048 || !rows || !cols || !cost || !cand3d || !cand2d || !cand2d_calib || !good || !j3d || !j2d || !j2d_calib ||
      (use_median && !median)) return -1;
  JunctionGateArgs a{rows, cols, K, cost, C, cand3d, cand2d, cand2d_calib, use_median, median, good, j3d, j2d, j2d_calib};
  hipLaunchKernelGGL(junction_gate_kernel, dim3(1), dim3(1024), 0, (hipStream_t)stream, a);
  return (int)hipGetLastError();
}

int neat_inv_small(const float* A, int n, int lda, float* out, void* stream) {
  if (!A || !out || n < 1 || n > 4 || lda < n) return -1;
  hipLaunchKernelGGL(inv_small_kernel, dim3(1), dim3(64), 0, (hipStream_t)stream, A, n, lda, out);
  return (int)hipGetLastError();
}

int neat_camera_mats(const float* pose, const float* K, int kstride, float* w2c, float* K3, void* stream) {
  if (!pose || !K || !w2c || !K3 || kstride < 3) return -1;
  hipLaunchKernelGGL(camera_mats_kernel, dim3(1), dim3(64), 0, (hipStream_t)stream, pose, K, kstride, w2c, K3);
  return (int)hipGetLastError();
}

int neat_project2d(const float* K, const float* w2c, const float* X, int N, float* uv, void* stream) {
  if (N <= 0) return 0;
  if (!K || !w2c || !X || !uv) return -1;
  hipLaunchKernelGGL(project2d_kernel, dim3((N + 255) / 256), dim3(256), 0, (hipStream_t)stream, K, w2c, X, N, uv);
  return (int)hipGetLastError();
}

int neat_project2d_pair(const float* K, const float* K2, const float* w2c, const float* X, int N, float* uv, float* uv2, void* stream) {
  if (N <= 0) return 0;
  if (!K || !K2 || !w2c || !X || !uv || !uv2) return -1;
  hipLaunchKernelGGL(project2d_pair_kernel, dim3((N + 255) / 256), dim3(256), 0, (hipStream_t)stream, K, K2, w2c, X, N, uv, uv2);
  return (int)hipGetLastError();
}

int neat_camera_setup(const float* uv, const float* uv2, const float* pose, const float* K, int kstride, int R, float* dirs, float* origins,
                      float* dirs2, float* w2c, float* K3, void* stream) {
  if (R <= 0 || !uv || !pose || !K || !dirs || !origins || (uv2 && !dirs2) || !w2c || !K3 || kstride < 3) return -1;
  hipLaunchKernelGGL(camera_setup_kernel, grid1(R), dim3(256), 0, (hipStream_t)stream, uv, uv2, pose, K, kstride, R, dirs, origins, dirs2, w2c, K3);
  return (int)hipGetLastError();
}

int neat_project2d_backward(const float* K, const float* w2c, const float* X, int N, const float* d_uv, float* d_X, void* stream) {
  if (N <= 0) return 0;
  if (!K || !w2c || !X || !d_uv || !d_X) return -1;
  hipLaunchKernelGGL(project2d_bwd_kernel, dim3((N + 255) / 256), dim3(256), 0, (hipStream_t)stream, K, w2c, X, N, d_uv, d_X);
  return (int)hipGetLastError();
}

int neat_line_loss(const float* pred, const float* gt, const float* weight, int R, float threshold, float* out2, float* per_line,
                   float* d_pred, void* stream) {
  if (R <= 0 || !pred || !gt || !weight || !out2 || !per_line || !d_pred) return -1;
  hipLaunchKernelGGL(line_loss_kernel, dim3(1), dim3(1024), 0, (hipStream_t)stream, pred, gt, weight, R, threshold, out2, per_line, d_pred);
  return (int)hipGetLastError();
}

int neat_line_losses(const float* pred_px, const float* pred_calib, const float* gt5, const float* K, int R, float threshold, float* out3,
                     float* d_pred_calib, float grad_scale, void* stream) {
  if (R <= 0 || !pred_px || !pred_calib || !gt5 || !K || !out3 || !d_pred_calib) return -1;
  hipLaunchKernelGGL(line_losses_kernel, dim3(1), dim3(1024), 0, (hipStream_t)stream, pred_px, pred_calib, gt5, K, R, threshold, out3, d_pred_calib, grad_scale);
  return (int)hipGetLastError();
}

size_t neat_lsap_ws_bytes(int nr, int nc) {
  const size_t mx = (size_t)(nr > nc ? nr : nc), mn = (size_t)(nr < nc ? nr : nc);
  return (mn + 2 * mx) * sizeof(double) + ((size_t)nr + (size_t)nc + 5 * mx + 2 * mn) * sizeof(int);
}

int neat_lsap(const float* cost, int nr, int nc, const unsigned char* row_mask, const unsigned char* col_mask, long long* row_ind,
              long long* col_ind, int* n_match, void* ws, void* stream) {
  if (nr < 0 || nc < 0 || !n_match) return -1;
  if (nr == 0 || nc == 0) return (int)hipMemsetAsync(n_match, 0, sizeof(int), (hipStream_t)stream);
  if (!cost || !row_ind || !col_ind || !ws) return -1;
  const size_t mx = (size_t)(nr > nc ? nr : nc), mn = (size_t)(nr < nc ? nr : nc);
  LsapArgs a{cost, nr, nc, row_mask, row_ind, col_ind, n_match, (double*)ws, (int*)((double*)ws + mn + 2 * mx)};
  a.col_mask = col_mask;
  const size_t dbytes = (mn + 2 * mx) * sizeof(double), ibytes = ((size_t)nr + (size_t)nc + 5 * mx + 2 * mn) * sizeof(int);
  size_t lds = 0;
  constexpr size_t LSAP_LDS_MAX = 156 * 1024;
  a.cost_lds_off = -1;
  if (dbytes + ibytes <= LSAP_LDS_MAX) {
    NEAT_CHECK(lds_limit<&lsap_kernel>((int)LSAP_LDS_MAX));
    a.use_lds = 1; a.lds_int_off = (int)dbytes; lds = (dbytes + ibytes + 15) & ~(size_t)15;
    const size_t cbytes = (size_t)nr * nc * sizeof(float);
    if (lds + cbytes <= LSAP_LDS_MAX) { a.cost_lds_off = (int)lds; lds += cbytes; }
  }
  int threads = (int)((mx + 1) / 2 + 63) / 64 * 64;
  threads = threads < 64 ? 64 : (threads > LSAP_WG ? LSAP_WG : threads);
  hipLaunchKernelGGL(lsap_kernel, dim3(1), dim3(threads), lds, (hipStream_t)stream, a);
  return (int)hipGetLastError();
}

size_t neat_dbscan_ws_bytes(int n) { return (size_t)n * 2 * sizeof(int); }

int neat_dbscan_means(const float* points, int n, double eps, float* centres, unsigned char* valid, int* count, void* ws, void* stream) {
  if (n <= 0 || n > DBSCAN_MAXN || !points || !centres || !valid || !count || !ws || !(eps > 0.0)) return -1;
  int* parent = (int*)ws; int* has_nb = parent + n;
  hipLaunchKernelGGL(dbscan_init_kernel, dim3((n + 255) / 256), dim3(256), 0, (hipStream_t)stream, parent, has_nb, n);
  hipLaunchKernelGGL(dbscan_union_kernel, dim3(n), dim3(128), 0, (hipStream_t)stream, points, n, eps * eps, parent, has_nb);
  const size_t acc_bytes = (size_t)(n / 2) * 28 + (size_t)n * 4, pbytes = (size_t)n * 12;
  const int mode = acc_bytes <= 96 * 1024 ? 2 : (pbytes <= 96 * 1024 ? 1 : 0);
  if (mode) NEAT_CHECK(lds_limit<&dbscan_finish_kernel>(96 * 1024));
  hipLaunchKernelGGL(dbscan_finish_kernel, dim3(1), dim3(1024), mode == 2 ? acc_bytes : (mode == 1 ? pbytes : 0), (hipStream_t)stream, points, n,
                     parent, has_nb, centres, valid, count, mode);
  return (int)hipGetLastError();
}

int neat_volume_weights(const float* z, const float* sdf, int R, int S, const float* beta, float* weights, void* stream) {
  if (R <= 0 || S <= 0) return 0;
  hipLaunchKernelGGL(volume_weights_kernel, dim3((R + 3) / 4), dim3(256), 0, (hipStream_t)stream, z, sdf, R, S, beta, weights);
  return (int)hipGetLastError();
}

static inline size_t parse_al(size_t b) { return (b + 255) & ~(size_t)255; }
static inline int parse_tiles(int n) { return (2 * n + PARSE_TILE - 1) / PARSE_TILE; }

int neat_parse_match(const float* lines2d, int n, const float* gt, int m, int gt_stride, float threshold, int* label, float* mindis,
                     void* stream) {
  if (n < 0 || m < 0 || (m > 0 && (!gt || gt_stride < 4))) return -1;
  if (n == 0) return 0;
  if (!lines2d || !label || !mindis) return -1;
  hipLaunchKernelGGL(parse_match_kernel, grid1(n, PARSE_WG), dim3(PARSE_WG), 0, (hipStream_t)stream, lines2d, n, gt, m, gt_stride, threshold,
                     label, mindis);
  return (int)hipGetLastError();
}

size_t neat_parse_group_ws_bytes(int n, int m) {
  if (n < 0 || m < 0) return 0;
  const size_t nt = (size_t)parse_tiles(n);
  return parse_al((nt * m + 3 * (size_t)m) * sizeof(int)) + parse_al(2 * (size_t)n * sizeof(int));
}

int neat_parse_group(const int* label, const float* lines3d, const float* l3d, int n, int m, float* lines, float* scores, int* count,
                     void* ws, void* stream) {
  if (n < 0 || m < 0 || !count) return -1;
  hipStream_t st = (hipStream_t)stream;
  if (n == 0 || m == 0) return (int)hipMemsetAsync(count, 0, sizeof(int), st);
  if (!label || !lines3d || !l3d || !lines || !scores || !ws) return -1;
  const int nt = parse_tiles(n);
  int* run = (int*)ws;
  int* cnt = run + (size_t)nt * m;
  int* start = cnt + m;
  int* slot = start + m;
  int* order = (int*)((char*)ws + parse_al(((size_t)nt * m + 3 * (size_t)m) * sizeof(int)));
  NEAT_CHECK(hipMemsetAsync(run, 0, (size_t)nt * m * sizeof(int), st));
  hipLaunchKernelGGL(parse_group_tile_kernel, dim3(nt), dim3(PARSE_WG), 0, st, label, 2 * n, m, run, order, 0);
  hipLaunchKernelGGL(parse_group_scan_kernel, dim3(1), dim3(1024), 0, st, run, nt, m, cnt, start, slot, count);
  hipLaunchKernelGGL(parse_group_tile_kernel, dim3(nt), dim3(PARSE_WG), 0, st, label, 2 * n, m, run, order, 1);
  hipLaunchKernelGGL(parse_group_reduce_kernel, dim3(m), dim3(PARSE_WG), 0, st, order, cnt, start, slot, lines3d, l3d, n, lines, scores);
  return (int)hipGetLastError();
}

size_t neat_parse_vote_ws_bytes(int J, int mcap) {
  if (J <= 0 || mcap <= 0) return 0;
  const size_t nc = 2 * (size_t)mcap, k = std::min((size_t)J, nc);
  return parse_al((size_t)J * nc * sizeof(float)) + parse_al(nc) + 2 * parse_al(k * sizeof(long long)) + parse_al(sizeof(int)) +
         parse_al(neat_lsap_ws_bytes(J, (int)nc));
}

int neat_parse_vote(const float* junctions, int J, const float* lines, const int* count, int mcap, float threshold, int view, int* votes,
                    int* first, void* ws, void* stream) {
  if (J < 0 || mcap < 0 || view < 0) return -1;
  if (J == 0 || mcap == 0) return 0;
  if (!junctions || !lines || !count || !votes || !first || !ws) return -1;
  hipStream_t st = (hipStream_t)stream;
  const int nc = 2 * mcap, k = std::min(J, nc);
  char* p = (char*)ws;
  float* cost = (float*)p; p += parse_al((size_t)J * nc * sizeof(float));
  unsigned char* cmask = (unsigned char*)p; p += parse_al(nc);
  long long* rows = (long long*)p; p += parse_al((size_t)k * sizeof(long long));
  long long* cols = (long long*)p; p += parse_al((size_t)k * sizeof(long long));
  int* n_match = (int*)p; p += parse_al(sizeof(int));
  const size_t total = (size_t)J * nc;
  hipLaunchKernelGGL(parse_vote_cost_kernel, dim3((unsigned)((total + 255) / 256)), dim3(256), 0, st, junctions, J, lines, count, nc, cost, cmask);
  NEAT_CHECK(hipGetLastError());
  const int e = neat_lsap(cost, J, nc, nullptr, cmask, rows, cols, n_match, p, stream);
  if (e != 0) return e;
  hipLaunchKernelGGL(parse_vote_apply_kernel, grid1(k), dim3(256), 0, st, rows, cols, n_match, k, cost, nc, threshold, view, votes, first);
  return (int)hipGetLastError();
}

size_t neat_parse_graph_ws_bytes(int V, int mcap, int J) {
  if (V < 0 || mcap < 0 || J < 0) return 0;
  return parse_al((size_t)V * mcap * sizeof(int)) + parse_al((size_t)J * sizeof(int));
}

int neat_parse_graph(const float* vlines, const float* vscores, const int* vcount, int V, int mcap, float score_threshold,
                     const float* junctions, const int* votes, const int* first, int J, float* lines_out, float* junc_out,
                     unsigned char* graph, int* pairs, float* wfi, int ecap, int* counts, void* ws, void* stream) {
  if (V < 0 || mcap < 0 || J < 0 || ecap < 0 || !counts) return -1;
  hipStream_t st = (hipStream_t)stream;
  if ((V > 0 && mcap > 0 && (!vlines || !vscores || !vcount || !lines_out || !ws)) ||
      (J > 0 && (!junctions || !votes || !first || !junc_out || !graph || !ws)) || (ecap > 0 && (!pairs || !wfi))) return -1;
  NEAT_CHECK(hipMemsetAsync(counts, 0, 3 * sizeof(int), st));
  const int ncap = V * mcap;
  if (ncap == 0 && J == 0) return 0;
  int* idx = (int*)ws;
  int* rowcnt = (int*)((char*)ws + parse_al((size_t)V * mcap * sizeof(int)));
  hipLaunchKernelGGL(parse_select_kernel, dim3(2), dim3(1024), 0, st, vlines, vscores, vcount, V, mcap, score_threshold, junctions, votes, first,
                     J, lines_out, junc_out, idx, counts);
  if (J == 0 || ncap == 0) return (int)hipGetLastError();
  NEAT_CHECK(hipMemsetAsync(graph, 0, (size_t)J * J, st));
  hipLaunchKernelGGL(parse_graph_mark_kernel, grid1(ncap, PARSE_WG), dim3(PARSE_WG), 0, st, lines_out, junc_out, counts, ncap, J, graph);
  hipLaunchKernelGGL(parse_edge_count_kernel, dim3(J), dim3(64), 0, st, graph, counts, J, rowcnt);
  hipLaunchKernelGGL(parse_edge_write_kernel, dim3(J), dim3(64), 0, st, graph, counts, J, rowcnt, J, junc_out, ecap, pairs, wfi);
  return (int)hipGetLastError();
}

size_t neat_parse_visibility_ws_bytes(int ecap, int V) {
  if (ecap < 0 || V < 0) return 0;
  return parse_al((size_t)V * ecap) + parse_al((size_t)ecap * sizeof(int));
}

int neat_parse_visibility(const float* lines, const int* n_lines, int ecap, const float* gt, int gt_stride, const int* gt_off,
                          const float* K3, const float* w2c, int V, float ckdist, int ckview, int* vis_count, float* checked,
                          int* n_checked, void* ws, void* stream) {
  if (ecap < 0 || V < 0 || !n_checked) return -1;
  hipStream_t st = (hipStream_t)stream;
  if (ecap == 0) return (int)hipMemsetAsync(n_checked, 0, sizeof(int), st);
  if (!lines || !vis_count || !checked || !ws || (V > 0 && (!gt_off || !K3 || !w2c || gt_stride < 4))) return -1;
  unsigned char* vis = (unsigned char*)ws;
  int* idx = (int*)((char*)ws + parse_al((size_t)V * ecap));
  if (V > 0)
    hipLaunchKernelGGL(parse_vis_kernel, dim3((ecap + PARSE_WG - 1) / PARSE_WG, V), dim3(PARSE_WG), 0, st, lines, n_lines, ecap, gt, gt_stride,
                       gt_off, K3, w2c, ckdist, vis);
  hipLaunchKernelGGL(parse_vis_count_kernel, dim3(1), dim3(1024), 0, st, lines, n_lines, ecap, V, vis, ckview, vis_count, idx, checked, n_checked);
  return (int)hipGetLastError();
}

static bool mesh_axes(const int* n, const double* b0, const double* b1, MeshAxes* g) {
  if (!n || !b0 || !b1) return false;
  for (int a = 0; a < 3; ++a) {
    if (n[a] < 2 || !std::isfinite(b0[a]) || !std::isfinite(b1[a])) return false;
    g->n[a] = n[a]; g->b0[a] = b0[a]; g->b1[a] = b1[a]; g->step[a] = (b1[a] - b0[a]) / (double)(n[a] - 1);
  }
  return true;
}
static inline long long mesh_nodes(int nx, int ny, int nz) {
  if (nx < 2 || ny < 2 || nz < 2) return 0;
  const long long n = (long long)nx * ny;
  if (n > INT_MAX) return 0;
  const long long N = n * nz;
// ... 65 lines not shown
```

neat_amd/csrc/neat_net.hip:

```cpp
#include <mutex>
#include <unordered_map>
#if defined(NEAT_HALF) && NEAT_HALF
#define neat neat_f16
#include "f16_symbols.h"
#endif
#include "kernels_bf16.hpp"
#include "kernels_dw.hpp"
#include "fused_launch.hpp"
#include "../../include/neat_hip.h"
#include <algorithm>
#include <initializer_list>
#include <utility>
#include <math.h>
#include <stdio.h>
#include <stdlib.h>
#include <vector>

using namespace neat;

namespace {

constexpr int L_REND = 9, L_ATTR = 14;
const int kO[NLAYERS] = {256, 256, 256, 217, 256, 256, 256, 256, 257, 256, 256, 256, 256, 3, 256, 256, 256, 256, 6};
const int kI[NLAYERS] = {39, 256, 256, 256, 256, 256, 256, 256, 256, 289, 256, 256, 256, 256, 265, 256, 256, 256, 256};
// ... 1270 lines not shown
                                   const float* __restrict__ d_feat, const float* __restrict__ mask, int P, int ldp,
                                   float* __restrict__ abar8, const float* __restrict__ cot_slot) {
  const float scale = cot_scale_of(cot_slot);
  const int p = blockIdx.x * blockDim.x + threadIdx.x;
  const int n = blockIdx.y;
  if (p >= ldp) return;
  float v = 0.0f;
  if (p < P) {
    if (d_out257) v += d_out257[(size_t)p * 257 + n];
    if (n == 0) { if (d_sdf) v += d_sdf[p] * (1.0f - mask[p]); }
    else if (d_feat) v += d_feat[(size_t)p * 256 + (n - 1)];
  }
  abar8[(size_t)n * ldp + p] = v * scale;
}

struct InputGradArgs {
  const float *x_fm, *ae0, *aes, *e0, *es, *gh, *mask;
  const float *d_sdf, *d_grad, *cot_slot;
  float scale; int P, ldp;
  float* d_x;
};
__global__ __launch_bounds__(256) void sdf_input_grad_kernel(InputGradArgs a) {
  const int p = blockIdx.x * blockDim.x + threadIdx.x;
  if (p >= a.P) return;
  const size_t ldp = (size_t)a.ldp;
  const float inv = 1.0f / cot_scale_of(a.cot_slot);
  float xv[3], dx[3];
#pragma unroll
  for (int c = 0; c < 3; ++c) {
    const float xc = a.x_fm[c * ldp + p], gc = a.gh[c * ldp + p];
    xv[c] = xc;
    float acc = a.ae0[c * ldp + p] + a.aes[c * ldp + p];
    float f = 1.0f;
#pragma unroll
    for (int k = 0; k < 6; ++k) {
      const size_t rs = (size_t)(3 + 6 * k + c) * ldp + p, rc = (size_t)(6 + 6 * k + c) * ldp + p;
      const float sa = a.ae0[rs] + a.aes[rs], ca = a.ae0[rc] + a.aes[rc];
      const float su = a.e0[rs] + a.es[rs], cu = a.e0[rc] + a.es[rc];
      const float sn = sinf(xc * f), cs = cosf(xc * f);
      acc += f * (cs * sa - sn * ca) - f * f * (sn * su + cs * cu) * gc;
      f *= 2.0f;
    }
    dx[c] = acc * inv;
  }
  if (a.mask[p] != 0.0f) {
    const float nr = sqrtf(xv[0] * xv[0] + xv[1] * xv[1] + xv[2] * xv[2]);
    if (nr > 0.0f) {
      const float ds = a.d_sdf ? a.d_sdf[p] : 0.0f;
      float cg[3] = {0.f, 0.f, 0.f};
      if (a.d_grad) { cg[0] = a.d_grad[3 * (size_t)p]; cg[1] = a.d_grad[3 * (size_t)p + 1]; cg[2] = a.d_grad[3 * (size_t)p + 2]; }
      const float rn = 1.0f / nr;
      const float dot = (xv[0] * cg[0] + xv[1] * cg[1] + xv[2] * cg[2]) * rn;
#pragma unroll
      for (int c = 0; c < 3; ++c) {
        const float xh = xv[c] * rn;
        dx[c] -= a.scale * (xh * ds + (cg[c] - xh * dot) * rn);
      }
    }
  }
#pragma unroll
  for (int c = 0; c < 3; ++c) a.d_x[3 * (size_t)p + c] = dx[c];
}

hipError_t sdf_input_grad(const Ctx& c, const SdfWs& w, float scale, const float* d_sdf, const float* d_grad, const float* slot, float* d_x) {
  const PackLayout& L = c.L();
  hipError_t e;
  if ((e = layer(c, L.tr[0], EPI_LINEAR, in(w.m[0], 256), NOIN, nullptr, PE_ROWS, F(w.Eh))) != hipSuccess) return e;
  if ((e = layer(c, L.tr[4], EPI_REV, in(w.m[4], 256), NOIN, nullptr, 256, w.vh[6], F(w.abar8), 217, w.h[4])) != hipSuccess) return e;
  InputGradArgs a{};
  a.x_fm = w.x; a.ae0 = w.Eh; a.aes = w.abar8; a.e0 = w.e0; a.es = w.es; a.gh = w.gh; a.mask = w.mask;
  a.d_sdf = d_sdf; a.d_grad = d_grad; a.cot_slot = slot;
  a.scale = scale; a.P = c.P; a.ldp = c.ldp; a.d_x = d_x;
  ProfSlot* ps = prof_begin(c.st, 0, 0.0, (double)c.P * (4 * PE_ROWS * 4.0 + 3 * 4.0 + 3 * 4.0 + 4.0 + 4.0 + 3 * 4.0 + 3 * 4.0));
  hipLaunchKernelGGL(sdf_input_grad_kernel, grid1(c.P), dim3(256), 0, c.st, a);
  prof_end(c.st, ps);
  dbg_sync(c.st, "sdf input grad", c.P, 0, 0);
  return hipGetLastError();
}

__global__ void zero_word_kernel(float* p) { if (threadIdx.x == 0) *p = 0.0f; }
const float* cot_scale_begin(const Ctx& c, float* slot, std::initializer_list<std::pair<const float*, long long>> arrays) {
  if (!NEAT_HALF) return nullptr;
  if (arrays.size() > (size_t)COT_MAX_ARRAYS) abort();
  static const bool use_memset = getenv("NEAT_COT_MEMSET") != nullptr;
  if (use_memset) (void)hipMemsetAsync(slot, 0, sizeof(float), c.st);
  else hipLaunchKernelGGL(zero_word_kernel, dim3(1), dim3(64), 0, c.st, slot);
  CotMaxArgs a{};
  long long total = 0;
  for (const auto& it : arrays) { if (a.narr >= COT_MAX_ARRAYS) break; a.p[a.narr] = it.first; a.n[a.narr] = it.first ? it.second : 0; total += a.n[a.narr]; ++a.narr; }
  a.slot = slot;
  const int blocks = (int)std::min<long long>(1024, (total + 2047) / 2048);
  if (blocks > 0) hipLaunchKernelGGL(cot_max_kernel, dim3(blocks), dim3(256), 0, c.st, a);
  return slot;
}
struct GradUnscaleArgs { float* p[3 * NLAYERS]; int n[3 * NLAYERS]; const float* slot; };
__global__ void grad_unscale_kernel(GradUnscaleArgs a) {
  float* p = a.p[blockIdx.y];
  const int n = a.n[blockIdx.y];
  if (!p) return;
  const float inv = 1.0f / cot_scale_of(a.slot);
  for (int i = blockIdx.x * blockDim.x + threadIdx.x; i < n; i += gridDim.x * blockDim.x) p[i] *= inv;
}
void grad_unscale(const Ctx& c, const neat_net_grads* gr, int first, int count, const float* slot) {
  if (!slot) return;
  GradUnscaleArgs a{};
  for (int l = 0; l < NLAYERS; ++l) {
    const bool on = l >= first && l < first + count && gr->dv[l];
    a.p[3 * l] = on ? gr->dv[l] : nullptr; a.n[3 * l] = kO[l] * kI[l];
    a.p[3 * l + 1] = on ? gr->dg[l] : nullptr; a.n[3 * l + 1] = kO[l];
    a.p[3 * l + 2] = on ? gr->db[l] : nullptr; a.n[3 * l + 2] = kO[l];
  }
  a.slot = slot;
  hipLaunchKernelGGL(grad_unscale_kernel, dim3(64, 3 * NLAYERS), dim3(256), 0, c.st, a);
}

void export_out8(const Ctx& c, const SdfWs& w, float* out257, float* feat) {
  const int P = c.P;
  if (c.prec) {
    if (out257 || feat)
      hipLaunchKernelGGL(export_out8_kernel, dim3((P + 255) / 256, 32), dim3(256), 0, c.st, (const float*)w.sdfraw, reinterpret_cast<const u16*>(w.feat.p),
                         reinterpret_cast<const u16*>(w.featlo.p), P, c.ldp, out257, feat);
  } else {
    if (out257) hipLaunchKernelGGL(fm_to_rm_kernel, grid1(P), dim3(256), 0, c.st, w.sdfraw, P, 257, c.ldp, out257, 0);
    if (feat) hipLaunchKernelGGL(fm_to_rm_kernel, grid1(P), dim3(256), 0, c.st, w.feat.f(), P, 256, c.ldp, feat, 0);
  }
}

Ctx make_ctx(const Prec& pr, const float* packed, const neat_net_params* net, int P, void* stream) {
  Ctx c{(hipStream_t)stream, packed, net, P, round_ldp(P, pr.prec), pr.prec};
  c.x3 = pr.x3; c.hx3 = pr.hx3;
  return c;
}

}

#if !NEAT_HALF
#define NEAT_TWIN(fn) extern "C" decltype(fn) f16_##fn;
#include "twin_list.h"
#undef NEAT_TWIN
__attribute__((visibility("hidden"))) int neat_aux_set_tuning(int key, int value);
#define NEAT_F16_FWD(call) if (precision == 3) { precision = BF16; return f16_##call; } if (precision == HX3 || precision == HX3_FASTVALUES) return f16_##call;
#else
#define NEAT_F16_FWD(call)
#endif

extern "C" {

#if !NEAT_HALF
int neat_abi_version(void) { return 15; }
#endif

int neat_set_tuning(int key, int value) {
#if !NEAT_HALF
  if (key == 28 || key == 30) return neat_aux_set_tuning(key, value);
  f16_neat_set_tuning(key, value);
#endif
  if (key == 0 && (value == 2 || value == 4)) { g_pt_bf16 = value; return 0; }
  if (key == 1 && (value == 0 || value == 1)) { g_wgrad_h3 = value; return 0; }
  if (key == 2 && (value == 0 || value == 1)) { g_layer_ws = value; return 0; }
  if (key == 3 && value >= 1 && value <= 4096) { g_ws_grid = value; return 0; }
  if (key == 4 && value >= 0 && value <= 4) { g_fused_ws = value; return 0; }
  if (key == 6 && value >= 0 && value <= 2) { g_wreduce_direct = value; return 0; }
  if (key == 7 && (value == 0 || value == 1)) { g_wgrad_interleave = value; return 0; }
  if (key == 8 && (value == -1 || value == 0 || value == 2 || value == 3 || value == 6)) { g_wgrad_batch = value; return 0; }
  if (key == 5 && (value == 0 || (value >= 2 && value <= 4))) { g_fused_nt = value; return 0; }
  if (key == 9 && value >= 0 && value <= 2) { g_ws_interleave = value; return 0; }
  if (key == 10 && (value == 0 || value == 1)) { g_fused_interleave = value; return 0; }
  if (key == 11 && value >= 0 && value <= 63) { g_ws_aux_nt = value; return 0; }
  if (key == 12 && (value == 0 || value == 1)) { g_ws_wide_store = value; return 0; }
  if (key == 13 && (value == 0 || value == 1)) { g_fused_adj = value; return 0; }
  if (key == 14 && value >= 0 && value <= 2) { g_head_chain = value; return 0; }
  if (key == 15 && (value == 0 || value == 1)) { g_head_wgrad_order = value; return 0; }
  if (key == 16 && value >= 0 && value <= 2) { g_dw_fused = value; return 0; }
  if (key == 17 && value >= 0 && value <= 7) { g_dw_ablate = value; return 0; }
  if (key == 18 && value >= 1 && value <= 16) { g_dw_nsub = value; return 0; }
  if (key == 19 && (value == 0 || value == 1)) { g_wgrad_k320 = value; return 0; }
  if (key == 20 && (value == 0 || value == 1)) { g_head_l4_batched = value; return 0; }
  if (key == 21 && value >= 0 && value <= 4) { g_wgrad_narrow = value; return 0; }
  if (key == 22 && (value == 0 || value == 1)) { g_dw_lin8 = value; return 0; }
  if (key == 23 && (value == 0 || (value >= 16 && value <= DW_MAXGRID))) { g_dw_grid = value; return 0; }
  if (key == 24 && (value == 0 || value == 1)) { g_chain_pp = value; return 0; }
  if (key == 25 && (value == 0 || value == 1)) { g_dw_segments = value; return 0; }
  return -1;
}

int neat_prof_enable(int on) {
#if !NEAT_HALF
  f16_neat_prof_enable(on);
#endif
  g_prof.on = on != 0;
  g_prof.used = 0;
  return 0;
}

int neat_prof_collect(int cls, double* total_ms, double* total_flops, int* launches, double* total_bytes) {
  double ms = 0.0, fl = 0.0, by = 0.0;
  int n = 0;
  for (size_t i = 0; i < g_prof.used; ++i) {
    ProfSlot& s = g_prof.pool[i];
    if (s.cls != cls) continue;
    hipError_t e = hipEventSynchronize(s.e1);
    if (e != hipSuccess) return (int)e;
    float t = 0.0f;
    if ((e = hipEventElapsedTime(&t, s.e0, s.e1)) != hipSuccess) return (int)e;
    ms += t; fl += s.flops; by += s.bytes; ++n;
  }
#if !NEAT_HALF
  {
    double ms2 = 0.0, fl2 = 0.0, by2 = 0.0;
    int n2 = 0;
    const int rc = f16_neat_prof_collect(cls, &ms2, &fl2, &n2, &by2);
    if (rc != 0) return rc;
    ms += ms2; fl += fl2; by += by2; n += n2;
  }
#endif
  if (total_ms) *total_ms = ms;
  if (total_flops) *total_flops = fl;
  if (launches) *launches = n;
  if (total_bytes) *total_bytes = by;
  return 0;
}

size_t neat_packed_floats(int precision) {
  NEAT_F16_FWD(neat_packed_floats(precision))
  const Prec pr = resolve(precision);
  return (!pr.ok || pr.hx3 == 2) ? 0 : pack_layout(pr.prec, pr.hx3 != 0).total;
}

int neat_pack_weights(const neat_net_params* net, float* packed, int precision, void* stream) {
  NEAT_F16_FWD(neat_pack_weights(net, packed, precision, stream))
  const Prec pr = resolve(precision);
  if (pr.hx3 == 2) return -1;
  if (!net || !packed || !pr.ok) return -1;
  hipStream_t st = (hipStream_t)stream;
  const PackLayout& L = pack_layout(pr.prec, pr.hx3 != 0);
  RowScaleArgs ra;
  ra.net = to_ptrs(net);
  ra.rowscale = packed + L.rowscale_off;
  for (int l = 0; l <= NLAYERS; ++l) ra.row_off[l] = L.row_off[l];
  hipLaunchKernelGGL(rowscale_kernel, dim3((L.row_off[NLAYERS] + 3) / 4), dim3(WG), 0, st, ra);
  PackArgs2 pa;
  pa.net = ra.net; pa.rowscale = ra.rowscale;
  for (int l = 0; l <= NLAYERS; ++l) pa.row_off[l] = L.row_off[l];
  for (int i = 0; i < L.npacks; ++i) pa.d[i] = L.d[i];
  pa.npacks = L.npacks; pa.out = packed;
  hipLaunchKernelGGL(pack_kernel2, dim3(L.nblocks, 4), dim3(WG), 0, st, pa);
  if (L.npacks_lo > 0) {
    if (L.npacks_lo > MAXPACKS2) return -1;
    for (int i = 0; i < L.npacks_lo; ++i) pa.d[i] = L.d[L.npacks + i];
    pa.npacks = L.npacks_lo;
    hipLaunchKernelGGL(pack_kernel2, dim3(L.nblocks_lo, 4), dim3(WG), 0, st, pa);
  }
  return (int)hipGetLastError();
}

size_t neat_sdf_ws_floats(int P, int mode, int precision) {
  NEAT_F16_FWD(neat_sdf_ws_floats(P, mode, precision))
  const Prec pr = resolve(precision);
  return !pr.ok ? 0 : sdf_ws(nullptr, round_ldp(P, pr.prec), mode, pr.prec, pr.hx3 == 1).total;
}

struct RayPoints { const float* origins; const float* dirs; const float* z; int R, S; };
static int sdf_forward_impl(const float* packed, const neat_net_params* net, const float* x, const RayPoints* rp, int P, int mode, int precision,
                            float radius, float scale, float* ws, float* out257, float* sdf, float* feat, float* grad, void* stream,
                            bool laid_out = false) {
  const Prec pr = resolve(precision);
  if (pr.hx3 == 2 && mode != 0) return -1;
  if (P <= 0) return 0;
  if (!packed || !net || (!x && !rp && !laid_out) || !ws || !pr.ok) return -1;
  Ctx c = make_ctx(pr, packed, net, P, stream);
  SdfWs w = sdf_ws(ws, c.ldp, mode, pr.prec, pr.hx3);
  if (laid_out) {}
  else if (x) hipLaunchKernelGGL(rm_to_fm_kernel, grid1(c.ldp), dim3(256), 0, c.st, x, P, 3, c.ldp, w.x);
  else hipLaunchKernelGGL(points_from_rays_kernel, grid1(c.ldp), dim3(256), 0, c.st, rp->origins, rp->dirs, rp->z, rp->R, rp->S, c.ldp, w.x,
                          (float*)nullptr, (const float*)nullptr, 0);
  if (mode == 0 && pr.prec) {
    NEAT_CHECK(sdf_primal(c, w, false, radius, scale, sdf));
    return (int)hipGetLastError();
  }
  if (mode == 0) {
    NEAT_CHECK(sdf_primal(c, w, false));
    FINALIZE_LAUNCH(c, w.x, w.sdfraw, (const float*)nullptr,
                       (const float*)nullptr, P, c.ldp, radius, scale, w.sdf, (float*)nullptr, (float*)nullptr, sdf, (float*)nullptr,
                       P, (float*)nullptr);
    return (int)hipGetLastError();
  }
  NEAT_CHECK(sdf_primal(c, w, true));
  NEAT_CHECK(sdf_adjoint(c, w));
  FINALIZE_LAUNCH(c, w.x, w.sdfraw, w.e0, w.es, P, c.ldp, radius, scale,
                     w.sdf, w.g, w.mask, sdf, grad, P, (float*)nullptr);
  export_out8(c, w, out257, feat);
  return (int)hipGetLastError();
}

int neat_sdf_forward(const float* packed, const neat_net_params* net, const float* x, int P, int mode, int precision,
                     float radius, float scale, float* ws, float* out257, float* sdf, float* feat, float* grad,
                     void* stream) {
  NEAT_F16_FWD(neat_sdf_forward(packed, net, x, P, mode, precision, radius, scale, ws, out257, sdf, feat, grad, stream))
  if (P > 0 && !x) return -1;
  return sdf_forward_impl(packed, net, x, nullptr, P, mode, precision, radius, scale, ws, out257, sdf, feat, grad, stream);
}

int neat_sdf_values_rays(const float* packed, const neat_net_params* net, const float* origins, const float* dirs, const float* z, int R,
                         int S, int precision, float radius, float scale, float* ws, float* sdf, const int* gate, int gate_value,
                         void* stream) {
  NEAT_F16_FWD(neat_sdf_values_rays(packed, net, origins, dirs, z, R, S, precision, radius, scale, ws, sdf, gate, gate_value, stream))
  if (R <= 0 || S <= 0) return 0;
// ... 208 lines not shown
```

neat_amd/networks.py:

```python
import math

import numpy as np
import os

import torch
from torch import nn

from . import ops, rend_util
from .conf import ConfTree, from_dict
from .density import LaplaceDensity
from .ray_sampler import ErrorBoundSampler, HierarchicalSampler


def _wn_linear(in_dim, out_dim, weight_norm=True):
    lin = nn.Linear(in_dim, out_dim)
    if not weight_norm:
        raise NotImplementedError("the HIP path implements the weight-normed layers of the shipped confs")
    return lin


DEFAULT_PRECISION = "fp16x3"


def _wrap_wn(lin):
# ... 337 lines not shown
            w >= 0, torch.ones_like(w), -torch.ones_like(w))
        return (cam / w).reshape(*shape)[..., :2]

    def cluster_dbscan(self, points, eps=0.01, min_samples=2):
        from sklearn.cluster import DBSCAN
        labels = DBSCAN(eps=eps, min_samples=min_samples).fit(points).labels_
        centres = [points[labels == i].mean(axis=0) for i in range(labels.max() + 1)]
        return torch.tensor(np.array(centres).reshape(-1, 3)).float().to(self.latents.device)

    def volume_rendering(self, z_vals, sdf):
        return ops.volume_weights(z_vals, sdf, self.density.get_beta())

    def _rays(self, input, key="uv"):
        if input[key].is_cuda and input["pose"].shape[1:] == (4, 4):
            dirs, _, origins = ops.camera_rays(input[key], input["pose"], input["intrinsics"], with_origins=True)
            return dirs.reshape(-1, 3), origins
        dirs, cam = rend_util.get_camera_params(input[key], input["pose"], input["intrinsics"])
        n = dirs.shape[1]
        return dirs.reshape(-1, 3), cam.unsqueeze(1).repeat(1, n, 1).reshape(-1, 3)

    def _z_vals(self, ray_dirs, cam_loc):
        if self.z_vals_override is not None:
            z = self.z_vals_override
            idx = self._cpu_random("eik_idx", lambda: torch.randint(z.shape[-1], (z.shape[0],)), z.device)
            if z.is_cuda and self.training and not self.junction_eikonal:
                return z, (z, idx)
            return z, z.gather(1, idx.unsqueeze(-1))
        return self.ray_sampler.get_z_vals(ray_dirs, cam_loc, self)

    def render_rgb(self, input):
        assert not self.training
        ray_dirs, cam_loc = self._rays(input)
        z_vals, _ = self._z_vals(ray_dirs, cam_loc)
        return self._render(cam_loc, ray_dirs, z_vals, False)[0]

    def forward(self, input):
        intrinsics, uv, pose = input["intrinsics"], input["uv"], input["pose"]
        setup = None
        if (uv.is_cuda and pose.shape == (1, 4, 4) and intrinsics.dtype == torch.float32 and intrinsics.stride(-1) == 1
                and intrinsics.shape[0] == 1 and "uv_proj" in input and input["uv_proj"].shape == uv.shape):
            setup = ops.camera_setup(uv, input["uv_proj"], pose, intrinsics)
            ray_dirs, cam_loc = setup[0], setup[1]
        else:
            ray_dirs, cam_loc = self._rays(input)
        n_rays = ray_dirs.shape[0]
        z_vals, z_eik = self._z_vals(ray_dirs, cam_loc)
        grad_theta = None
        if self.training and not self.junction_eikonal:
            eik = self._eikonal_points(n_rays, cam_loc, ray_dirs, z_eik, None)
            rgb, lines3d, depth, xyz, weights, sdf_s, points, nmap, grad_theta = self._render(
                cam_loc, ray_dirs, z_vals, False, eik, with_eik=True)
        else:
            rgb, lines3d, depth, xyz, weights, sdf_s, points, nmap = self._render(cam_loc, ray_dirs, z_vals, not self.training)
        output = {"points": points, "rgb_values": rgb, "sdf": sdf_s, "depth": depth, "xyz": xyz}

        points3d = xyz
        main = torch.cuda.current_stream() if xyz.is_cuda else None
        side = self._side_stream(xyz.device) if (main is not None and self.use_side_stream) else None
        if setup is not None:
            w2c, K3 = setup[3], setup[4]
        elif xyz.is_cuda and pose.shape[1:] == (4, 4) and intrinsics.dtype == torch.float32 and intrinsics.stride(-1) == 1:
            w2c, K3 = ops.camera_mats(pose[0], intrinsics[0])
        else:
            w2c = ops.inv_small(pose[0])[:3]
            K3 = intrinsics[0, :3, :3]
        Rm, T = w2c[:, :3], w2c[:, 3:]
        eye = _eye3(K3.device)

        def l3d_block():
            if points3d.is_cuda:
                net = self.implicit_network
                p3_sdf, p3_grad = ops.sdf_point_normals(net.handle(), points3d, net.sdf_bounding_sphere, net.sphere_scale)
            else:
                p3_sdf, _, p3_grad = self.implicit_network.get_outputs(points3d)
            l_dirs, l_orig = (setup[2], cam_loc) if setup is not None else self._rays(input, "uv_proj")
            if points3d.is_cuda:
                l3d = ops.l3d_points(points3d, l_orig, l_dirs, p3_grad)
            else:
                den = (l_dirs * p3_grad).sum(-1)
                den = den + torch.where(den >= 0, torch.full_like(den, 1e-6), torch.full_like(den, -1e-6))
                t = (((points3d - l_orig) * p3_grad).sum(-1) / den).detach()
                l3d = l_orig + l_dirs * t.unsqueeze(-1)
            l3d_score = None
            if self.training and self.use_l3d:
                with torch.no_grad():
                    a, b = l3d - lines3d[:, 0], l3d - lines3d[:, 1]
                    l3d_score = torch.linalg.cross(a, b).norm(dim=-1) / (lines3d[:, 0] - lines3d[:, 1]).norm(dim=-1)
            return p3_sdf, l3d, l3d_score

        j3d_global = None
        if side is not None:
            side_b = self._side_stream(xyz.device, 1)
            side.wait_stream(main)
            side_b.wait_stream(main)
            if self.training:
                if self.use_side_stream & 1:
                    with torch.cuda.stream(side):
                        j3d_global = self._global_junctions()
                    j3d_global.record_stream(main)
                else:
                    j3d_global = self._global_junctions()
            if self.use_side_stream & 2:
                with torch.cuda.stream(side_b):
                    p3_sdf, l3d, l3d_score = l3d_block()
                for tns in (p3_sdf, l3d, l3d_score):
                    if tns is not None:
                        tns.record_stream(main)
            else:
                p3_sdf, l3d, l3d_score = l3d_block()
                side_b = None
            if self.training and self.use_l3d and side_b is not None:
                main.wait_stream(side_b)
                side_b = None
        else:
            side_b = None
            if self.training:
                j3d_global = self._global_junctions()
            p3_sdf, l3d, l3d_score = l3d_block()
        if xyz.is_cuda:
            K3c, w2c3 = K3.contiguous(), w2c.contiguous()
            K3 = K3c
            proj = lambda Kc, X: ops.project2d(Kc, w2c3, X)
            proj_pair = lambda X: ops.project2d_pair(K3c, eye, w2c3, X)
        else:
            K3c = K3
            proj = lambda Kc, X: self.project2D(Kc, Rm, T, X)
            proj_pair = lambda X: (proj(K3c, X), proj(eye, X))
        if xyz.is_cuda:
            lines2d, lines2d_calib = proj_pair(lines3d)
            lines2d = lines2d.detach()
        else:
            lines2d = proj(K3c, lines3d.detach())
            lines2d_calib = proj(eye, lines3d)
        if self.training:
            cand_valid = None
            if self.dbscan_enabled:
                if lines3d.is_cuda and 2 <= 2 * n_rays <= ops.DBSCAN_MAX_POINTS:
                    cand3d, cand_valid, _ = ops.dbscan_means(lines3d.detach().reshape(-1, 3), 0.01)
                else:
                    cand3d = self.cluster_dbscan(lines3d.detach().cpu().numpy().reshape(-1, 3), eps=0.01, min_samples=2)
            elif self.use_l3d:
                thr = l3d_score.median().clamp_min(0.01)
                keep = l3d_score < thr
                cand3d = torch.cat([lines3d[keep].detach().reshape(-1, 3), l3d[keep]], 0)
            else:
                cand3d = lines3d.detach().reshape(-1, 3)
            if self.dbscan_enabled or self.use_l3d:
                cand2d, cand2d_calib = proj_pair(cand3d)
            else:
                cand2d = lines2d.reshape(-1, 2)
                cand2d_calib = lines2d_calib.detach().reshape(-1, 2)
            gt2d = _device_copy(input["wireframe"][0], "vertices", cand2d.device)
            fused_gate = cand2d.is_cuda and min(gt2d.shape[0], cand2d.shape[0]) <= 2048
            cost = ops.junction_cost(cand2d, gt2d) if fused_gate else ((cand2d[None] - gt2d[:, None]) ** 2).sum(-1).sqrt()
            rows, cols, _ = ops.linear_sum_assignment(cost, None, cand_valid)
            if fused_gate:
                median, good, j3_pad, j2_pad, j2c_pad = ops.junction_gate(rows, cols, cost, cand3d, cand2d, cand2d_calib, self.use_median)
                if self.use_median:
                    output["median"] = median
            else:
                if cand_valid is None:
                    matched = cost[rows, cols]
                    pair_ok = None
                else:
                    pair_ok = rows >= 0
                    rows, cols = rows.clamp_min(0), cols.clamp_min(0)
                    matched = torch.where(pair_ok, cost[rows, cols], torch.full_like(cost[rows, cols], float("nan")))
                if self.use_median:
                    if matched.numel() == 0:
                        median = matched.new_tensor(10.0)
                    elif pair_ok is None:
                        median = matched.detach().median()
                    else:
                        median = torch.nanmedian(matched.detach())
                        median = torch.where(torch.isnan(median), torch.full_like(median, 10.0), median)
                    good = matched < median
                    output["median"] = median
                else:
                    good = matched < 10
                if pair_ok is not None:
                    good = good & pair_ok
                j2_pad, j3_pad, j2c_pad = cand2d[cols], cand3d[cols], cand2d_calib[cols]
            if side is not None:
                main.wait_stream(side)
            output = JunctionOutputs(output, good, {"j2d_local": j2_pad, "j3d_local": j3_pad, "j2d_local_calib": j2c_pad})
            output["j3d_global"] = j3d_global
            output["j2d_global"], output["j2d_global_calib"] = proj_pair(j3d_global)
            if xyz.is_cuda:
                output.calib_proj = {"w2c": w2c3, "lines3d": lines3d, "lines2d_calib": lines2d_calib, "j3d_global": j3d_global,
                                     "j2d_global_calib": output["j2d_global_calib"]}
        if side_b is not None:
            main.wait_stream(side_b)
        elif side is not None and not self.training:
            main.wait_stream(side)
        output["l3d"] = l3d
        output["points3d"] = points3d
        output["lines3d"] = lines3d
        output["lines2d_calib"] = lines2d_calib
        output["lines2d"] = lines2d
        output["sdf"] = p3_sdf.flatten()
        output["wireframe-gt"] = input["wireframe"]
        output["K"] = K3

        if self.training:
            if grad_theta is None:
                grad_theta = self._eikonal(n_rays, cam_loc, ray_dirs, z_eik, output["j3d_global"].detach())
            output["grad_theta"] = grad_theta
        else:
            output["normal_map"] = nmap
        return output

    def _global_junctions(self):
        lin = [m for m in self.ffn if isinstance(m, nn.Linear)]
        if (self.latents.is_cuda and len(self.ffn) == 5 and len(lin) == 3 and self.latents.shape[1] == 256
                and tuple(lin[0].weight.shape) == (256, 256) and tuple(lin[1].weight.shape) == (256, 256)
                and tuple(lin[2].weight.shape) == (3, 256)):
            return ops.ffn_junctions(self.latents, lin)
        return self.ffn(self.latents)

    def _side_stream(self, device, idx=0):
        key = (str(device), idx)
        if key not in self._side:
            self._side[key] = torch.cuda.Stream(device=device)
        return self._side[key]

    def _cpu_random(self, name, draw, device):
        if self.static_randoms is None:
            return _to_device_async(draw(), device, name)
        slot = self.static_randoms.get(name)
        if slot is None:
            t = draw()
            slot = {"draw": draw, "dev": t.to(device), "order": len(self.static_randoms)}
            self.static_randoms[name] = slot
        return slot["dev"]

    def _eikonal_points(self, n_rays, cam_loc, ray_dirs, z_eik, junctions):
        r = self.scene_bounding_sphere
        eik = self._cpu_random("eik_uniform", lambda: torch.empty(n_rays, 3).uniform_(-r, r), ray_dirs.device)
        if isinstance(z_eik, tuple):
            if eik.is_cuda:
                return ops.eik_points(eik, cam_loc, ray_dirs, None, junctions, z=z_eik[0], idx=z_eik[1])
            z_eik = z_eik[0].gather(1, z_eik[1].unsqueeze(-1))
        if eik.is_cuda:
            return ops.eik_points(eik, cam_loc, ray_dirs, z_eik, junctions)
        eik = torch.cat([eik, torch.addcmul(cam_loc, z_eik, ray_dirs)], 0)
        if junctions is not None:
            eik = torch.cat([eik, junctions], 0)
        return eik

    def _eikonal(self, n_rays, cam_loc, ray_dirs, z_eik, junctions):
        return self.implicit_network.gradient(self._eikonal_points(n_rays, cam_loc, ray_dirs, z_eik, junctions))
```

neat_amd/ops.py:

```python
import ctypes

import torch

from . import _lib

NET_LAYOUT = (("implicit_network", 9), ("rendering_network", 5), ("attraction_network", 5))
LAYER_OUT = [256, 256, 256, 217, 256, 256, 256, 256, 257, 256, 256, 256, 256, 3, 256, 256, 256, 256, 6]
LAYER_IN = [39, 256, 256, 256, 256, 256, 256, 256, 256, 289, 256, 256, 256, 256, 265, 256, 256, 256, 256]
N_SDF = 9


def _p(t):
    return ctypes.c_void_p(t.data_ptr()) if t is not None else None


def _stream():
    return ctypes.c_void_p(torch.cuda.current_stream().cuda_stream)


def copy_batch(pairs):
    lib = _lib.lib()
    for i0 in range(0, len(pairs), 16):
        chunk = pairs[i0:i0 + 16]
        n = len(chunk)
# ... 610 lines not shown


class LineLossesFn(torch.autograd.Function):

    @staticmethod
    def forward(ctx, pred_px, pred_calib, gt5, K, threshold):
        pu, pc, g, Kc = _f32c(pred_px.detach()), _f32c(pred_calib.detach()), _f32c(gt5.detach()), _f32c(K.detach())
        R = pc.shape[0]
        if pu.shape != (R, 4) or pc.shape != (R, 4) or g.shape != (R, 5) or Kc.numel() != 9:
            raise RuntimeError("line_losses: pred [R,4] x2, gt [R,5], K [3,3]")
        out3 = torch.empty(3, device=pc.device)
        d_pred = torch.empty(R, 4, device=pc.device)
        _lib.check(_lib.lib().neat_line_losses(_p(pu), _p(pc), _p(g), _p(Kc), R, float(threshold), _p(out3), _p(d_pred), 1.0, _stream()),
                   "neat_line_losses")
        ctx.save_for_backward(d_pred)
        ctx.set_materialize_grads(False)
        l2d, count = out3[0], out3[2]
        ctx.mark_non_differentiable(l2d, count)
        return l2d, out3[1], count

    @staticmethod
    def backward(ctx, g_l2d, g_loss, g_count):
        (d_pred,) = ctx.saved_tensors
        return None, (None if g_loss is None else g_loss * d_pred), None, None, None


def line_losses(pred_px, pred_calib, gt5, K, threshold=100.0):
    return LineLossesFn.apply(pred_px, pred_calib, gt5, K, threshold)


def inv_small(A):
    A = A.detach()
    if not A.is_cuda:
        return torch.linalg.inv_ex(A).inverse
    A = _f32c(A)
    n = A.shape[-1]
    out = torch.empty(n, n, device=A.device)
    _lib.check(_lib.lib().neat_inv_small(_p(A), n, n, _p(out), _stream()), "neat_inv_small")
    return out


class FfnFn(torch.autograd.Function):

    @staticmethod
    def forward(ctx, x, W0, b0, W1, b1, W2, b2):
        lib = _lib.lib()
        args = [_f32c(t.detach()) for t in (x, W0, b0, W1, b1, W2, b2)]
        J = args[0].shape[0]
        h1, h2 = torch.empty(J, 256, device=x.device), torch.empty(J, 256, device=x.device)
        y = torch.empty(J, 3, device=x.device)
        _lib.check(lib.neat_ffn_forward(_p(args[0]), J, *[_p(t) for t in args[1:]], _p(h1), _p(h2), _p(y), _stream()), "neat_ffn_forward")
        ctx.save_for_backward(args[0], args[1], args[3], args[5], h1, h2)
        return y

    @staticmethod
    def backward(ctx, dy):
        x, W0, W1, W2, h1, h2 = ctx.saved_tensors
        J = x.shape[0]
        dy = _f32c(dy)
        ws2 = torch.empty(2 * J * 256, device=x.device)
        dx = torch.empty_like(x)
        flat = torch.empty(2 * (256 * 256 + 256) + 3 * 256 + 3, device=x.device)
        dW0, db0, dW1, db1, dW2, db2 = flat.split([65536, 256, 65536, 256, 768, 3])
        _lib.check(_lib.lib().neat_ffn_backward(_p(x), J, _p(W0), _p(W1), _p(W2), _p(h1), _p(h2), _p(dy), _p(ws2), _p(dx), _p(dW0), _p(db0),
                                               _p(dW1), _p(db1), _p(dW2), _p(db2), _stream()), "neat_ffn_backward")
        return dx, dW0.view(256, 256), db0, dW1.view(256, 256), db1, dW2.view(3, 256), db2


def ffn_junctions(x, linears):
    l0, l1, l2 = linears
    return FfnFn.apply(x, l0.weight, l0.bias, l1.weight, l1.bias, l2.weight, l2.bias)


DBSCAN_MAX_POINTS = 8192


def dbscan_means(points, eps):
    lib = _lib.lib()
    pts = _f32c(points.detach().reshape(-1, 3))
    n = pts.shape[0]
    if n > DBSCAN_MAX_POINTS or n < 2:
        raise RuntimeError(f"dbscan_means handles 2..{DBSCAN_MAX_POINTS} points, got {n}")
    buf = torch.empty(n // 2, 4, device=pts.device)
    valid = torch.empty(n // 2, device=pts.device, dtype=torch.uint8)
    count = torch.empty(1, device=pts.device, dtype=torch.int32)
    ws = torch.empty(int(lib.neat_dbscan_ws_bytes(n)), device=pts.device, dtype=torch.uint8)
    flat = buf.view(-1)
    _lib.check(lib.neat_dbscan_means(_p(pts), n, float(eps), _p(flat), _p(valid), _p(count), _p(ws), _stream()), "neat_dbscan_means")
    return flat[:3 * (n // 2)].view(n // 2, 3), valid.view(torch.bool), count


_GRAD_ONE = {}
_UNIT_SEED = [False]


def grad_one(device):
    key = str(device)
    t = _GRAD_ONE.get(key)
    if t is None:
        if torch.device(device).type == "cuda" and torch.cuda.is_current_stream_capturing():
            return torch.ones((), device=device)
        t = _GRAD_ONE[key] = torch.ones((), device=device)
    return t


class unit_seed:

    def __init__(self, device):
        self.one = grad_one(device)

    def __enter__(self):
        self.prev, _UNIT_SEED[0] = _UNIT_SEED[0], True
        return self.one

    def __exit__(self, *exc):
        _UNIT_SEED[0] = self.prev
        return False


class LossTailFn(torch.autograd.Function):

    @staticmethod
    def forward(ctx, rgb, gtheta, glo3, glo2c, pred_calib, pred_px, gt5, Kmat, rgb_gt, loc3, loc2c, loc2, glo2, good,
                w_eik, w_line, w_j3, w_j2, threshold, lines3d=None, w2c=None):
        lib = _lib.lib()
        dev = rgb.device
        c = lambda t: None if t is None else _f32c(t.detach())
        rgb_c, gt_c, gth_c = c(rgb), c(rgb_gt.reshape(-1, 3)), c(gtheta)
        glo3_c, glo2c_c, glo2_c, loc3_c, loc2c_c, loc2_c = c(glo3), c(glo2c), c(glo2), c(loc3), c(loc2c), c(loc2)
        pc, pu, g5, Kc = c(pred_calib.reshape(-1, 4)), c(pred_px.reshape(-1, 4)), c(gt5), c(Kmat)
        R, E = rgb_c.shape[0], 0 if gth_c is None else gth_c.shape[0]
        L = pc.shape[0]
        if pu.shape != (L, 4) or g5.shape != (L, 5) or Kc.numel() != 9:
            raise RuntimeError("loss_tail: lines [L,4] x2, gt [L,5], K [3,3]")
        K = 0 if loc3_c is None else loc3_c.shape[0]
        J = 0 if glo3_c is None else glo3_c.shape[0]
        have_pairs = bool(K and J)
        scal = torch.empty(8, device=dev) if have_pairs else torch.zeros(8, device=dev)
        line3 = torch.empty(3, device=dev)
        fold = lines3d is not None and w2c is not None
        x3_c, w2c_c = (_f32c(lines3d.detach().reshape(-1, 6)), _f32c(w2c.detach())) if fold else (None, None)
        if fold and (x3_c.shape[0] != L or w2c_c.shape != (3, 4)):
            raise RuntimeError("loss_tail: lines3d [L,2,3] and w2c [3,4]")
        sizes = [R * 3, E * 3, J * 3 if have_pairs else 0, J * 2 if have_pairs else 0, L * 4, L * 6 if fold else 0]
        flat = torch.empty(sum(sizes), device=dev)
        d_rgb, d_gth, d_glo3, d_glo2c, d_pred, d_x3 = flat.split(sizes)
        d_gth = d_gth if E else None
        pair_cost = torch.empty(K, J, device=dev) if have_pairs else None
        _lib.check(lib.neat_loss_lines_terms(_p(pu), _p(pc), _p(g5), _p(Kc), L, float(threshold), _p(line3), _p(d_pred), w_line,
                                             _p(rgb_c), _p(gt_c), R, _p(gth_c), E, _p(loc3_c), _p(loc2c_c), K, _p(glo3_c), _p(glo2c_c), J,
                                             _p(scal), _p(d_rgb), _p(d_gth), _p(pair_cost), w_eik, _p(w2c_c), _p(x3_c), _p(d_x3) if fold else None,
                                             _stream()), "neat_loss_lines_terms")
        if have_pairs:
            ri, ci, n_match = linear_sum_assignment(pair_cost, good)
            loss = torch.empty((), device=dev)
            _lib.check(lib.neat_loss_pairs(_p(ri), _p(ci), _p(n_match), ri.shape[0], _p(loc3_c), _p(loc2c_c), _p(loc2_c), _p(glo3_c),
                                           _p(glo2c_c), _p(glo2_c), J, _p(pair_cost), _p(scal), _p(d_glo3), _p(d_glo2c),
                                           _ip(line3, 1), w_eik, w_line, w_j3, w_j2, 1, _p(loss), _p(w2c_c), _stream()), "neat_loss_pairs")
        else:
            loss = scal[0] + w_eik * scal[1] + w_line * line3[1]
        ctx.save_for_backward(flat)
        ctx.sizes = sizes
        ctx.set_materialize_grads(False)
        ctx.shapes = (rgb.shape, None if gtheta is None else gtheta.shape, None if glo3 is None or not have_pairs else glo3.shape,
                      None if glo2c is None or not have_pairs or fold else glo2c.shape, None if fold else pred_calib.shape,
                      lines3d.shape if fold else None)
        ctx.mark_non_differentiable(scal, line3)
        return loss, scal, line3

    @staticmethod
    def backward(ctx, g_loss, g_scal, g_line3):
        if g_loss is None:
            return (None,) * 21
        (flat,) = ctx.saved_tensors
        one = _GRAD_ONE.get(str(flat.device))
        if not (_UNIT_SEED[0] and one is not None and g_loss.data_ptr() == one.data_ptr()):
            flat = flat * g_loss
        g = flat.split(ctx.sizes)
        s_rgb, s_gth, s_glo3, s_glo2c, s_pred, s_x3 = ctx.shapes
        return (g[0].view(s_rgb),
                None if s_gth is None else g[1].view(s_gth),
                None if s_glo3 is None else g[2].view(s_glo3),
                None if s_glo2c is None else g[3].view(s_glo2c),
                None if s_pred is None else g[4].view(s_pred)) + (None,) * 14 + (None if s_x3 is None else g[5].view(s_x3), None)


def loss_tail(rgb, gtheta, glo3, glo2c, pred_calib, pred_px, gt5, Kmat, rgb_gt, loc3, loc2c, loc2, glo2, good, w_eik, w_line, w_j3, w_j2,
              threshold=100.0, lines3d=None, w2c=None):
    return LossTailFn.apply(rgb, gtheta, glo3, glo2c, pred_calib, pred_px, gt5, Kmat, rgb_gt, loc3, loc2c, loc2, glo2, good,
                            float(w_eik), float(w_line), float(w_j3), float(w_j2), float(threshold), lines3d, w2c)


def camera_setup(uv, uv_proj, pose, intrinsics):
    uv_c, pose_c, Kc = _f32c(uv.detach()), _f32c(pose.detach()), intrinsics.detach()
    if pose_c.shape != (1, 4, 4) or Kc.dtype != torch.float32 or not Kc.is_cuda or Kc.stride(-1) != 1 or Kc.shape[0] != 1:
        raise RuntimeError("camera_setup: one 4x4 pose, intrinsics with unit column stride, CUDA float32")
    R, dev = uv_c.shape[1], uv_c.device
    up = _f32c(uv_proj.detach()) if uv_proj is not None else None
    if up is not None and up.shape != uv_c.shape:
        raise RuntimeError("camera_setup: uv_proj must have uv's shape")
    dirs, origins = torch.empty(R, 3, device=dev), torch.empty(R, 3, device=dev)
    dirs2 = torch.empty(R, 3, device=dev) if up is not None else None
    w2c, K3 = torch.empty(3, 4, device=dev), torch.empty(3, 3, device=dev)
    _lib.check(_lib.lib().neat_camera_setup(_p(uv_c), _p(up), _p(pose_c), _p(Kc), int(Kc.stride(-2)), R, _p(dirs), _p(origins), _p(dirs2),
                                            _p(w2c), _p(K3), _stream()), "neat_camera_setup")
    return dirs, origins, dirs2, w2c, K3


class Project2DPairFn(torch.autograd.Function):

    @staticmethod
    def forward(ctx, K3, K3b, w2c, X):
        lib = _lib.lib()
        K3, K3b, w2c = _f32c(K3.detach()), _f32c(K3b.detach()), _f32c(w2c.detach())
        Xc = _f32c(X.detach().reshape(-1, 3))
        uv, uv2 = torch.empty(Xc.shape[0], 2, device=Xc.device), torch.empty(Xc.shape[0], 2, device=Xc.device)
        _lib.check(lib.neat_project2d_pair(_p(K3), _p(K3b), _p(w2c), _p(Xc), Xc.shape[0], _p(uv), _p(uv2), _stream()), "neat_project2d_pair")
        ctx.save_for_backward(K3, K3b, w2c, Xc)
        ctx.shape = X.shape
        ctx.set_materialize_grads(False)
        return uv.reshape(*X.shape[:-1], 2), uv2.reshape(*X.shape[:-1], 2)

    @staticmethod
    def backward(ctx, d_uv, d_uv2):
        if d_uv is None and d_uv2 is None:
            return None, None, None, None
        K3, K3b, w2c, Xc = ctx.saved_tensors
        total = None
        for Kx, d in ((K3, d_uv), (K3b, d_uv2)):
            if d is None:
                continue
            dX = torch.empty_like(Xc)
            _lib.check(_lib.lib().neat_project2d_backward(_p(Kx), _p(w2c), _p(Xc), Xc.shape[0], _p(_f32c(d.reshape(-1, 2))), _p(dX), _stream()),
                       "neat_project2d_backward")
            total = dX if total is None else total + dX
        return None, None, None, total.reshape(ctx.shape)


def project2d_pair(K3, K3b, w2c, X):
    return Project2DPairFn.apply(K3, K3b, w2c, X)


class SdfNormalsFn(torch.autograd.Function):

    @staticmethod
    def forward(ctx, handle, x, radius, scale, *params):
        lib = _lib.lib()
        ctx.set_materialize_grads(False)
        x = _f32c(x.detach())
        P = x.shape[0]
        packed, netp = handle.packed()
        prec = handle.precision
        ws = torch.empty(lib.neat_sdf_ws_floats(P, 1, prec), device=x.device, dtype=torch.float32)
        sdf, grad = torch.empty(P, 1, device=x.device), torch.empty(P, 3, device=x.device)
        _lib.check(lib.neat_sdf_forward(_p(packed), ctypes.byref(netp), _p(x), P, 1, prec, float(radius), float(scale), _p(ws),
                                        None, _p(sdf), None, _p(grad), _stream()), "neat_sdf_forward(normals)")
        ctx.handle, ctx.P, ctx.ws, ctx.packed, ctx.netp, ctx.prec = handle, P, ws, packed, netp, prec
        ctx.keep = params
        return sdf, grad

    @staticmethod
    def backward(ctx, d_sdf, d_grad):
        lib = _lib.lib()
        gr, views, _ = _grad_buffers(ctx.handle, 0, N_SDF, ctx.ws.device)
        d_sdf, d_grad = _f32c(d_sdf), _f32c(d_grad)
        _lib.check(lib.neat_sdf_backward(_p(ctx.packed), ctypes.byref(ctx.netp), _p(ctx.ws), ctx.P, ctx.prec, None, _p(d_sdf), None, _p(d_grad),
                                         ctypes.byref(gr), _stream()), "neat_sdf_backward")
        ctx.ws = None
        return (None, None, None, None, *views)


def sdf_point_normals(handle, x, radius, scale):
    if x.shape[0] == 0:
        return x.new_zeros(0, 1), x.new_zeros(0, 3)
    return SdfNormalsFn.apply(handle, x, radius, scale, *handle.tensors(0, N_SDF))


def camera_mats(pose, intrinsics):
    pose, Kc = _f32c(pose.detach()), intrinsics.detach()
    if Kc.dtype != torch.float32 or not Kc.is_cuda or Kc.stride(-1) != 1 or pose.shape != (4, 4):
        raise RuntimeError("camera_mats: pose [4,4] and intrinsics with unit column stride, CUDA float32")
    w2c, K3 = torch.empty(3, 4, device=pose.device), torch.empty(3, 3, device=pose.device)
    _lib.check(_lib.lib().neat_camera_mats(_p(pose), _p(Kc), int(Kc.stride(-2)), _p(w2c), _p(K3), _stream()), "neat_camera_mats")
    return w2c, K3


def l3d_points(x, origins, dirs, normals):
    x, o, d, n = (_f32c(t.detach().reshape(-1, 3)) for t in (x, origins, dirs, normals))
    out = torch.empty_like(x)
    _lib.check(_lib.lib().neat_l3d(_p(x), _p(o), _p(d), _p(n), x.shape[0], _p(out), _stream()), "neat_l3d")
    return out


def junction_cost(cand2d, gt2d):
    cand2d, gt2d = _f32c(cand2d.detach()), _f32c(gt2d.detach())
    V, C = gt2d.shape[0], cand2d.shape[0]
    cost = torch.empty(V, C, device=cand2d.device)
    _lib.check(_lib.lib().neat_junction_cost(_p(cand2d), _p(gt2d), V, C, _p(cost), _stream()), "neat_junction_cost")
    return cost


def junction_gate(rows, cols, cost, cand3d, cand2d, cand2d_calib, use_median):
    K = rows.shape[0]
    dev = cost.device
    cand3d, cand2d, cand2d_calib = _f32c(cand3d.detach()), _f32c(cand2d.detach()), _f32c(cand2d_calib.detach())
    median = torch.empty(1, device=dev) if use_median else None
    good = torch.empty(K, device=dev, dtype=torch.uint8)
    j3d, j2d, j2dc = torch.empty(K, 3, device=dev), torch.empty(K, 2, device=dev), torch.empty(K, 2, device=dev)
    _lib.check(_lib.lib().neat_junction_gate(_p(rows), _p(cols), K, _p(cost), cost.shape[1], _p(cand3d), _p(cand2d), _p(cand2d_calib),
                                             1 if use_median else 0, _p(median), _p(good), _p(j3d), _p(j2d), _p(j2dc), _stream()),
               "neat_junction_gate")
    return (median.reshape(()) if use_median else None), good.view(torch.bool), j3d, j2d, j2dc


def _i32(t):
    if t.dtype != torch.int32 or not t.is_cuda:
        raise RuntimeError("neat_amd parse ops need CUDA int32 tensors: got %s on %s" % (t.dtype, t.device))
    return t.contiguous()


def _ws(nbytes, device):
    return torch.empty(max(int(nbytes), 8), device=device, dtype=torch.uint8)


def _rows4(gt):
    gt = _f32c(gt.detach()) if gt.stride(-1) != 1 or gt.dtype != torch.float32 or not gt.is_cuda else gt.detach()
    if gt.dim() != 2 or gt.shape[1] < 4:
        raise RuntimeError("parse ops: ground-truth lines [m, >= 4]")
    if gt.shape[0] > 1 and gt.stride(0) < 4:
        gt = gt.contiguous()
    return gt, (int(gt.stride(0)) if gt.shape[0] > 1 else int(gt.shape[1]))


def parse_match(lines2d, gt, threshold):
    lines2d = _f32c(lines2d.detach().reshape(-1, 4))
    n, dev = lines2d.shape[0], lines2d.device
    gt, stride = _rows4(gt)
    label = torch.empty(2 * n, device=dev, dtype=torch.int32)
    mindis = torch.empty(2 * n, device=dev)
    _lib.check(_lib.lib().neat_parse_match(_p(lines2d), n, _p(gt), gt.shape[0], stride, float(threshold), _p(label), _p(mindis), _stream()),
               "neat_parse_match")
    return label, mindis


def parse_group(label, lines3d, l3d, m, out=None):
    lines3d, l3d, label = _f32c(lines3d.detach().reshape(-1, 6)), _f32c(l3d.detach().reshape(-1, 3)), _i32(label)
    n, dev = lines3d.shape[0], lines3d.device
    if label.numel() != 2 * n or l3d.shape[0] != n:
        raise RuntimeError("parse_group: label [2n], lines3d [n,2,3], l3d [n,3]")
    if out is None:
        out = (torch.empty(max(m, 1), 2, 3, device=dev), torch.empty(max(m, 1), device=dev), torch.empty(1, device=dev, dtype=torch.int32))
    lines, scores, count = out
    lib = _lib.lib()
    ws = _ws(lib.neat_parse_group_ws_bytes(n, m), dev)
    _lib.check(lib.neat_parse_group(_p(label), _p(lines3d), _p(l3d), n, m, _p(lines), _p(scores), _p(count), _p(ws), _stream()),
               "neat_parse_group")
    return lines, scores, count


def parse_vote(junctions, lines, count, threshold, view, votes, first):
    junctions, lines = _f32c(junctions.detach()), _f32c(lines.detach())
    J, mcap = junctions.shape[0], lines.shape[0]
    lib = _lib.lib()
    ws = _ws(lib.neat_parse_vote_ws_bytes(J, mcap), junctions.device)
    _lib.check(lib.neat_parse_vote(_p(junctions), J, _p(lines), _p(_i32(count)), mcap, float(threshold), int(view), _p(votes), _p(first),
                                   _p(ws), _stream()), "neat_parse_vote")


def parse_graph(vlines, vscores, vcount, score_threshold, junctions, votes, first):
    vlines, vscores, junctions = _f32c(vlines.detach()), _f32c(vscores.detach()), _f32c(junctions.detach())
    V, mcap, J = vlines.shape[0], vlines.shape[1], junctions.shape[0]
    dev = junctions.device
    ncap = V * mcap
    ecap = min(ncap, J * (J + 1) // 2)
    lib = _lib.lib()
    res = {"lines": torch.empty(max(ncap, 1), 2, 3, device=dev), "junctions": torch.empty(max(J, 1), 3, device=dev),
           "graph": torch.empty(max(J * J, 1), device=dev, dtype=torch.uint8), "pairs": torch.empty(max(ecap, 1), 2, device=dev, dtype=torch.int32),
           "wfi": torch.empty(max(ecap, 1), 2, 3, device=dev), "counts": torch.empty(3, device=dev, dtype=torch.int32), "ecap": ecap}
    ws = _ws(lib.neat_parse_graph_ws_bytes(V, mcap, J), dev)
    _lib.check(lib.neat_parse_graph(_p(vlines), _p(vscores), _p(_i32(vcount)), V, mcap, float(score_threshold), _p(junctions), _p(_i32(votes)),
                                    _p(_i32(first)), J, _p(res["lines"]), _p(res["junctions"]), _p(res["graph"]), _p(res["pairs"]),
                                    _p(res["wfi"]), ecap, _p(res["counts"]), _p(ws), _stream()), "neat_parse_graph")
    return res


def parse_visibility(lines, n_lines, gt_packed, gt_off, K3, w2c, ckdist, ckview):
    lines = _f32c(lines.detach().reshape(-1, 6))
    ecap, dev = lines.shape[0], lines.device
    V = int(gt_off.shape[0]) - 1
    gt, stride = _rows4(gt_packed) if gt_packed.shape[0] > 0 else (gt_packed, 4)
    K3, w2c = _f32c(K3.detach()), _f32c(w2c.detach())
    vis_count = torch.empty(max(ecap, 1), device=dev, dtype=torch.int32)
    checked = torch.empty(max(ecap, 1), 2, 3, device=dev)
    n_checked = torch.empty(1, device=dev, dtype=torch.int32)
    lib = _lib.lib()
    ws = _ws(lib.neat_parse_visibility_ws_bytes(ecap, V), dev)
    _lib.check(lib.neat_parse_visibility(_p(lines), _p(_i32(n_lines)) if n_lines is not None else None, ecap,
                                         _p(gt) if gt.numel() > 0 else None, stride, _p(_i32(gt_off)), _p(K3), _p(w2c), V,
                                         float(ckdist), int(ckview), _p(vis_count), _p(checked), _p(n_checked), _p(ws), _stream()),
               "neat_parse_visibility")
    return vis_count[:ecap], checked[:ecap], n_checked


def _axes3(n, b0, b1):
    n3 = [int(v) for v in n]
    lo = [float(v) for v in (b0 if hasattr(b0, "__len__") else (b0,) * 3)]
    hi = [float(v) for v in (b1 if hasattr(b1, "__len__") else (b1,) * 3)]
    if len(n3) != 3 or len(lo) != 3 or len(hi) != 3:
        raise ValueError("a grid has three axes: n, b0, b1 of length 3 (or scalar bounds)")
    return (ctypes.c_int * 3)(*n3), (ctypes.c_double * 3)(*lo), (ctypes.c_double * 3)(*hi), n3


def grid_points(x_fm, ldp, first_node, count, n, b0, b1):
    cn, c0, c1, _ = _axes3(n, b0, b1)
    _lib.check(_lib.lib().neat_grid_points(_p(x_fm), int(ldp), int(first_node), int(count), cn, c0, c1, _stream()), "neat_grid_points")


def mesh_extract(grid, b0, b1, level=0.0):
    if grid.dim() != 3:
        raise ValueError("mesh_extract: grid [nx, ny, nz]")
    grid = _f32c(grid.detach())
    cn, c0, c1, (nx, ny, nz) = _axes3(grid.shape, b0, b1)
    lib, dev = _lib.lib(), grid.device
    nbytes = lib.neat_mesh_ws_bytes(nx, ny, nz)
    if nbytes == 0:
        raise ValueError("mesh_extract: every axis needs at least 2 nodes and the grid fewer than 2^31 nodes, got %s" % ((nx, ny, nz),))
    ws = _ws(nbytes, dev)
    counts = torch.empty(2, device=dev, dtype=torch.int32)
    _lib.check(lib.neat_mesh_count(_p(grid), nx, ny, nz, float(level), _p(ws), _p(counts), _stream()), "neat_mesh_count")
    nv, nf = counts.tolist()
    if nv < 0 or nf < 0:
        raise RuntimeError("mesh_extract: more vertices or faces than int32 indexes; extract the grid in parts")
    verts = torch.empty(nv, 3, device=dev)
    faces = torch.empty(nf, 3, device=dev, dtype=torch.int32)
    _lib.check(lib.neat_mesh_emit(_p(grid), nx, ny, nz, c0, c1, float(level), _p(ws), _p(verts) if nv else None, nv,
                                  _p(faces) if nf else None, nf, _stream()), "neat_mesh_emit")
    return verts, faces


def unit_rows3_(g):
    if g.dim() != 2 or g.shape[1] != 3 or g.dtype != torch.float32 or not g.is_cuda or not g.is_contiguous():
        raise RuntimeError("unit_rows3_: contiguous CUDA float32 [n, 3]")
    _lib.check(_lib.lib().neat_unit_rows3(_p(g), g.shape[0], _stream()), "neat_unit_rows3")
    return g
```

Measured before the change: 50.78 million ray-samples/s.

## Fuse junction cost, LSAP and gating into single kernels; add single-wave LSAP

After: 49.26 million ray-samples/s. 0.97x the previous value.

```diff
diff --git a/include/neat_hip.h b/include/neat_hip.h
--- a/include/neat_hip.h
+++ b/include/neat_hip.h
@@ -166,6 +166,13 @@
 size_t neat_lsap_ws_bytes(int nr, int nc);
 int neat_lsap(const float* cost, int nr, int nc, const unsigned char* row_mask, const unsigned char* col_mask, long long* row_ind,
               long long* col_ind, int* n_match, void* ws, void* stream);
+int neat_junction_match(const float* cand2d, const float* gt2d, int V, int C, const unsigned char* cand_mask, const float* cand3d,
+                        const float* cand2d_calib, int use_median, float* cost, long long* rows, long long* cols, int* n_match,
+                        float* median, unsigned char* good, float* j3d, float* j2d, float* j2d_calib, void* ws, void* stream);
+int neat_loss_match_pairs(const unsigned char* row_mask, int K, long long* ri, long long* ci, int* n_match, const float* loc3,
+                          const float* loc2c, const float* loc2, const float* glo3, const float* glo2c, const float* glo2, int J,
+                          const float* pair_cost, float* scal, float* d_glo3, float* d_glo2c, const float* line_loss, float w_eik,
+                          float w_line, float w_j3, float w_j2, int weighted_grads, float* total, const float* w2c, void* ws, void* stream);
 
 size_t neat_dbscan_ws_bytes(int n);
 int neat_dbscan_means(const float* points, int n, double eps, float* centres, unsigned char* valid, int* count, void* ws, void* stream);
diff --git a/neat_amd/_lib.py b/neat_amd/_lib.py
--- a/neat_amd/_lib.py
+++ b/neat_amd/_lib.py
@@ -103,6 +103,10 @@
                                       ctypes.c_int, c_fp, c_fp, ctypes.c_float, ctypes.c_float, ctypes.c_float, ctypes.c_float, c_fp]),
     "neat_lsap_ws_bytes": (ctypes.c_size_t, [ctypes.c_int, ctypes.c_int]),
     "neat_lsap": (ctypes.c_int, [c_fp, ctypes.c_int, ctypes.c_int, c_fp, c_fp, c_fp, c_fp, c_fp, c_fp, c_fp]),
+    "neat_junction_match": (ctypes.c_int, [c_fp, c_fp, ctypes.c_int, ctypes.c_int, c_fp, c_fp, c_fp, ctypes.c_int] + [c_fp] * 11),
+    "neat_loss_match_pairs": (ctypes.c_int, [c_fp, ctypes.c_int, c_fp, c_fp, c_fp, c_fp, c_fp, c_fp, c_fp, c_fp, c_fp, ctypes.c_int, c_fp, c_fp,
+                                             c_fp, c_fp, c_fp, ctypes.c_float, ctypes.c_float, ctypes.c_float, ctypes.c_float, ctypes.c_int,
+                                             c_fp, c_fp, c_fp, c_fp]),
     "neat_dbscan_ws_bytes": (ctypes.c_size_t, [ctypes.c_int]),
     "neat_dbscan_means": (ctypes.c_int, [c_fp, ctypes.c_int, ctypes.c_double, c_fp, c_fp, c_fp, c_fp, c_fp]),
     "neat_parse_match": (ctypes.c_int, [c_fp, ctypes.c_int, c_fp, ctypes.c_int, ctypes.c_int, ctypes.c_float, c_fp, c_fp, c_fp]),
diff --git a/neat_amd/csrc/kernels_junction.hpp b/neat_amd/csrc/kernels_junction.hpp
--- a/neat_amd/csrc/kernels_junction.hpp
+++ b/neat_amd/csrc/kernels_junction.hpp
@@ -18,6 +18,8 @@
   int use_lds, lds_int_off;
   const unsigned char* col_mask;
   int cost_lds_off;
+  int onewave;
+  int prestaged;
 };
 
 struct LsapKey { double val; int it; int un; };
@@ -62,12 +64,21 @@
   return total;
 }
 
-__global__ __launch_bounds__(LSAP_WG) void lsap_kernel(LsapArgs a) {
+struct LsapCtx {
+  int N, M;
+  bool T, ident, staged;
+  double* u; double* v; double* sp;
+  int* rowlist; int* collist; int* path; int* col4row; int* row4col; int* remaining; int* vis_row; int* vis_col; int* tmp;
+  const float* C; const float* Cl; int nc0;
+  __device__ __forceinline__ double cost(int i, int j) const {
+    const int idx = ident ? (T ? j * nc0 + i : i * nc0 + j) : (T ? rowlist[j] * nc0 + collist[i] : rowlist[i] * nc0 + collist[j]);
+    return (double)(staged ? Cl[idx] : C[idx]);
+  }
+};
+
+__device__ __forceinline__ bool lsap_prologue(const LsapArgs& a, LsapCtx& c) {
   __shared__ int s_wave[LSAP_WG / 64], s_base;
-  __shared__ LsapKey s_key[LSAP_WG / 64];
-  __shared__ int s_i, s_nrem, s_fail, s_done, s_nvis;
-  __shared__ double s_minval;
-  const int tid = threadIdx.x, nt = blockDim.x, lane = tid & 63, wave = tid >> 6, nw = nt >> 6;
+  const int tid = threadIdx.x, nt = blockDim.x;
   const int kmax = min(a.nr, a.nc);
   for (int k = tid; k < kmax; k += nt) { a.row_ind[k] = -1; a.col_ind[k] = -1; }
 
@@ -89,17 +100,20 @@
   }
   const bool T = c_eff < n_eff;
   const int N = T ? c_eff : n_eff, M = T ? n_eff : c_eff;
-  if (N == 0) { if (tid == 0) *a.n_match = 0; return; }
-  double* u = wsd; double* v = u + N; double* sp = v + M;
-  int* path = collist + a.nc; int* col4row = path + M; int* row4col = col4row + N; int* remaining = row4col + M;
-  int* vis_row = remaining + M;
-  int* vis_col = vis_row + N;
-  int* tmp = vis_col + M;
+  if (N == 0) { if (tid == 0) *a.n_match = 0; return false; }
+  c.N = N; c.M = M; c.T = T;
+  c.rowlist = rowlist; c.collist = collist;
+  c.u = wsd; c.v = c.u + N; c.sp = c.v + M;
+  c.path = collist + a.nc; c.col4row = c.path + M; c.row4col = c.col4row + N; c.remaining = c.row4col + M;
+  c.vis_row = c.remaining + M;
+  c.vis_col = c.vis_row + N;
+  c.tmp = c.vis_col + M;
   const float* C = a.cost;
-  const int nc0 = a.nc;
+  c.C = C; c.nc0 = a.nc;
   const bool staged = a.use_lds && a.cost_lds_off >= 0;
-  const float* Cl = reinterpret_cast<const float*>(lsap_lds + (staged ? a.cost_lds_off : 0));
-  if (staged) {
+  c.staged = staged;
+  c.Cl = reinterpret_cast<const float*>(lsap_lds + (staged ? a.cost_lds_off : 0));
+  if (staged && !a.prestaged) {
     float* dst = reinterpret_cast<float*>(lsap_lds + a.cost_lds_off);
     const int total = a.nr * a.nc;
     const int total4 = ((reinterpret_cast<size_t>(C) & 15) == 0) ? (total >> 2) : 0;
@@ -114,13 +128,23 @@
     }
     for (int e = 4 * total4 + tid; e < total; e += nt) dst[e] = C[e];
   }
-  const bool ident = !mask && !cmask;
-  auto cost = [&](int i, int j) -> double {
-    const int idx = ident ? (T ? j * nc0 + i : i * nc0 + j) : (T ? rowlist[j] * nc0 + collist[i] : rowlist[i] * nc0 + collist[j]);
-    return (double)(staged ? Cl[idx] : C[idx]);
-  };
-  for (int i = tid; i < N; i += nt) { u[i] = 0.0; col4row[i] = -1; }
-  for (int j = tid; j < M; j += nt) { v[j] = 0.0; row4col[j] = -1; }
+  c.ident = !mask && !cmask;
+  for (int i = tid; i < N; i += nt) { c.u[i] = 0.0; c.col4row[i] = -1; }
+  for (int j = tid; j < M; j += nt) { c.v[j] = 0.0; c.row4col[j] = -1; }
+  return true;
+}
+
+__device__ __forceinline__ void lsap_search_wg(const LsapArgs& a, const LsapCtx& c) {
+  __shared__ int s_wave[LSAP_WG / 64], s_base;
+  __shared__ LsapKey s_key[LSAP_WG / 64];
+  __shared__ int s_i, s_nrem, s_fail, s_done, s_nvis;
+  __shared__ double s_minval;
+  const int tid = threadIdx.x, nt = blockDim.x, lane = tid & 63, wave = tid >> 6, nw = nt >> 6;
+  const int N = c.N, M = c.M;
+  const bool T = c.T;
+  double* u = c.u; double* v = c.v; double* sp = c.sp;
+  int* rowlist = c.rowlist; int* collist = c.collist; int* path = c.path; int* col4row = c.col4row; int* row4col = c.row4col;
+  int* remaining = c.remaining; int* vis_row = c.vis_row; int* vis_col = c.vis_col; int* tmp = c.tmp;
   if (tid == 0) { s_fail = 0; s_done = 0; s_i = 0; s_nrem = M; s_minval = 0.0; s_nvis = 0; }
   __syncthreads();
 
@@ -133,7 +157,7 @@
       if (first) {
         for (int it = tid; it < M; it += nt) {
           const int j = M - 1 - it;
-          const double r = minval + cost(i, j) - ui - v[j];
+          const double r = minval + c.cost(i, j) - ui - v[j];
           const bool lower = r < INFINITY;
           const double spj = lower ? r : INFINITY;
           sp[j] = spj;
@@ -146,7 +170,7 @@
       } else {
         for (int it = tid; it < nrem; it += nt) {
           const int j = remaining[it];
-          const double r = minval + cost(i, j) - ui - v[j];
+          const double r = minval + c.cost(i, j) - ui - v[j];
           double spj = sp[j];
           if (r < spj) { path[j] = i; sp[j] = r; spj = r; }
           LsapKey k{spj, it, row4col[j] == -1 ? 1 : 0};
@@ -205,6 +229,123 @@
   if (tid == 0) *a.n_match = N;
 }
 
+__device__ __forceinline__ void lsap_wave_sync() {
+  __builtin_amdgcn_fence(__ATOMIC_RELEASE, "workgroup");
+  __builtin_amdgcn_wave_barrier();
+  __builtin_amdgcn_fence(__ATOMIC_ACQUIRE, "workgroup");
+}
+
+constexpr int LSAP_WU = 8;
+__device__ __forceinline__ void lsap_search_wave(const LsapArgs& a, const LsapCtx& c) {
+  const int lane = threadIdx.x & 63;
+  const int N = c.N, M = c.M;
+  double* u = c.u; double* v = c.v; double* sp = c.sp;
+  int* path = c.path; int* col4row = c.col4row; int* row4col = c.row4col;
+  int* remaining = c.remaining; int* vis_row = c.vis_row; int* vis_col = c.vis_col;
+  bool fail = false;
+  for (int cur = 0; cur < N && !fail; ++cur) {
+    int i = cur, nrem = M, nvis = 0;
+    double minval = 0.0;
+    bool first = true;
+    while (true) {
+      const double ui = u[i];
+      LsapKey best{INFINITY, -1, 0};
+      for (int b0 = lane; b0 < nrem; b0 += 64 * LSAP_WU) {
+        int jj[LSAP_WU], un[LSAP_WU];
+        double cc[LSAP_WU], vv[LSAP_WU], ss[LSAP_WU];
+#pragma unroll
+        for (int q = 0; q < LSAP_WU; ++q) {
+          const int it = b0 + 64 * q;
+          jj[q] = it < nrem ? (first ? M - 1 - it : remaining[it]) : 0;
+        }
+#pragma unroll
+        for (int q = 0; q < LSAP_WU; ++q) {
+          const int j = jj[q];
+          cc[q] = c.cost(i, j); vv[q] = v[j]; un[q] = row4col[j] == -1 ? 1 : 0;
+          ss[q] = first ? (double)INFINITY : sp[j];
+        }
+#pragma unroll
+        for (int q = 0; q < LSAP_WU; ++q) {
+          const int it = b0 + 64 * q, j = jj[q];
+          if (it < nrem) {
+            const double r = minval + cc[q] - ui - vv[q];
+            double spj = ss[q];
+            const bool lower = r < spj;
+            if (lower) { path[j] = i; spj = r; }
+            if (lower || first) sp[j] = spj;
+            if (first) remaining[it] = j;
+            LsapKey k{spj, it, un[q]};
+            if (spj < INFINITY && lsap_better(k, best)) best = k;
+          }
+        }
+      }
+      first = false;
+      lsap_wave_sync();
+      for (int m = 32; m >= 1; m >>= 1) {
+        LsapKey o = lsap_shfl_xor(best, m);
+        if (lsap_better(o, best)) best = o;
+      }
+      if (lane == 0) vis_row[nvis] = i;
+      if (best.it < 0) { fail = true; break; }
+      const double mv = best.val;
+      const int j = remaining[best.it], last = remaining[nrem - 1], r4 = row4col[j];
+      if (lane == 0) { vis_col[nvis] = j; remaining[best.it] = last; }
+      ++nvis;
+      lsap_wave_sync();
+      if (r4 != -1) { i = r4; minval = mv; --nrem; continue; }
+      for (int q = lane; q < nvis; q += 64) {
+        const int r_ = vis_row[q];
+        if (r_ == cur) u[r_] += mv;
+        else u[r_] += mv - sp[col4row[r_]];
+        const int c_ = vis_col[q];
+        v[c_] -= mv - sp[c_];
+      }
+      lsap_wave_sync();
+      if (lane == 0) {
+        int jp = j;
+        while (true) {
+          const int ii = path[jp];
+          row4col[jp] = ii;
+          const int t = col4row[ii]; col4row[ii] = jp; jp = t;
+          if (ii == cur) break;
+        }
+      }
+      lsap_wave_sync();
+      break;
+    }
+  }
+  if (fail) { if (lane == 0) *a.n_match = -1; return; }
+  if (!c.T) {
+    for (int r = lane; r < N; r += 64) { a.row_ind[r] = c.rowlist[r]; a.col_ind[r] = c.collist[col4row[r]]; }
+  } else {
+    int base = 0;
+    for (int k0 = 0; k0 < M; k0 += 64) {
+      const int k = k0 + lane;
+      const bool f = k < M && row4col[k] != -1;
+      const unsigned long long bal = __ballot(f);
+      if (f) {
+        const int q = base + __popcll(bal & ((1ull << lane) - 1ull));
+        a.row_ind[q] = c.rowlist[k]; a.col_ind[q] = c.collist[row4col[k]];
+      }
+      base += __popcll(bal);
+    }
+  }
+  if (lane == 0) *a.n_match = N;
+}
+
+__device__ __forceinline__ void lsap_body(const LsapArgs& a) {
+  LsapCtx c;
+  if (!lsap_prologue(a, c)) return;
+  if (a.onewave) {
+    __syncthreads();
+    if (threadIdx.x < 64) lsap_search_wave(a, c);
+  } else {
+    lsap_search_wg(a, c);
+  }
+}
+
+__global__ __launch_bounds__(LSAP_WG) void lsap_kernel(LsapArgs a) { lsap_body(a); }
+
 #ifndef NEAT_ADAM_PASSES
 #define NEAT_ADAM_PASSES 1
 #endif
@@ -1054,7 +1195,7 @@
   const float* w2c;
 };
 
-__global__ __launch_bounds__(1024) void loss_pairs_kernel(LossPairsArgs a) {
+__device__ __forceinline__ void loss_pairs_body(const LossPairsArgs& a) {
   __shared__ float s_red[16];
   const int tid = threadIdx.x, nt = blockDim.x;
   for (int i = tid; i < 3 * a.J; i += nt) a.d_glo3[i] = 0.0f;
@@ -1100,6 +1241,15 @@
   }
 }
 
+__global__ __launch_bounds__(1024) void loss_pairs_kernel(LossPairsArgs a) { loss_pairs_body(a); }
+
+struct LossMatchPairsArgs { LsapArgs l; LossPairsArgs p; };
+__global__ __launch_bounds__(LSAP_WG) void loss_match_pairs_kernel(LossMatchPairsArgs a) {
+  lsap_body(a.l);
+  __syncthreads();
+  loss_pairs_body(a.p);
+}
+
 __global__ void l3d_kernel(const float* __restrict__ x, const float* __restrict__ o, const float* __restrict__ d,
                            const float* __restrict__ nrm, int R, float* __restrict__ l3d) {
   const int r = blockIdx.x * blockDim.x + threadIdx.x;
@@ -1113,12 +1263,16 @@
   for (int c = 0; c < 3; ++c) l3d[3 * r + c] = o[3 * r + c] + d[3 * r + c] * t;
 }
 
+__device__ __forceinline__ float junction_cost_at(const float* __restrict__ cand2d, const float* __restrict__ gt2d, int C, int idx) {
+  const int v = idx / C, c = idx % C;
+  const float dx = cand2d[2 * c] - gt2d[2 * v], dy = cand2d[2 * c + 1] - gt2d[2 * v + 1];
+  return __fsqrt_rn(__fadd_rn(__fmul_rn(dx, dx), __fmul_rn(dy, dy)));
+}
+
 __global__ void junction_cost_kernel(const float* __restrict__ cand2d, const float* __restrict__ gt2d, int V, int C, float* __restrict__ cost) {
   const int idx = blockIdx.x * blockDim.x + threadIdx.x;
   if (idx >= V * C) return;
-  const int v = idx / C, c = idx % C;
-  const float dx = cand2d[2 * c] - gt2d[2 * v], dy = cand2d[2 * c + 1] - gt2d[2 * v + 1];
-  cost[idx] = __fsqrt_rn(__fadd_rn(__fmul_rn(dx, dx), __fmul_rn(dy, dy)));
+  cost[idx] = junction_cost_at(cand2d, gt2d, C, idx);
 }
 
 struct JunctionGateArgs {
@@ -1131,8 +1285,7 @@
   float* j3d; float* j2d; float* j2dc;
 };
 
-__global__ __launch_bounds__(1024) void junction_gate_kernel(JunctionGateArgs a) {
-  __shared__ float s_m[2048];
+__device__ __forceinline__ void junction_gate_body(const JunctionGateArgs& a, float* s_m) {
   __shared__ int s_n;
   __shared__ float s_med;
   const int tid = threadIdx.x, nt = blockDim.x;
@@ -1171,4 +1324,26 @@
   }
 }
 
-}
+__global__ __launch_bounds__(1024) void junction_gate_kernel(JunctionGateArgs a) {
+  __shared__ float s_m[2048];
+  junction_gate_body(a, s_m);
+}
+
+struct JunctionMatchArgs { const float* cand2d; const float* gt2d; LsapArgs l; JunctionGateArgs g; };
+__global__ __launch_bounds__(LSAP_WG) void junction_match_kernel(JunctionMatchArgs a) {
+  extern __shared__ __attribute__((aligned(16))) unsigned char lsap_lds[];
+  const int total = a.l.nr * a.l.nc;
+  float* cost = const_cast<float*>(a.l.cost);
+  float* stage = (a.l.use_lds && a.l.cost_lds_off >= 0) ? reinterpret_cast<float*>(lsap_lds + a.l.cost_lds_off) : nullptr;
+  for (int idx = threadIdx.x; idx < total; idx += blockDim.x) {
+    const float d = junction_cost_at(a.cand2d, a.gt2d, a.l.nc, idx);
+    cost[idx] = d;
+    if (stage) stage[idx] = d;
+  }
+  __syncthreads();
+  lsap_body(a.l);
+  __syncthreads();
+  junction_gate_body(a.g, reinterpret_cast<float*>(lsap_lds));
+}
+
+}
diff --git a/neat_amd/csrc/neat_aux.hip b/neat_amd/csrc/neat_aux.hip
--- a/neat_amd/csrc/neat_aux.hip
+++ b/neat_amd/csrc/neat_aux.hip
@@ -15,6 +15,8 @@
 namespace {
 
 int g_ffn_mfma = 1;
+int g_lsap_path = 1;
+constexpr size_t LSAP_WAVE_MAX_SMALL = 64, LSAP_WAVE_MAX_LARGE = 4096;
 int g_sampler_ablate = 0;
 
 #define NEAT_CHECK(expr) do { hipError_t e_ = (expr); if (e_ != hipSuccess) return (int)e_; } while (0)
@@ -41,11 +43,40 @@
   }
 }
 
+template <auto Kern>
+static int lsap_plan(const float* cost, int nr, int nc, const unsigned char* row_mask, const unsigned char* col_mask, long long* row_ind,
+                     long long* col_ind, int* n_match, void* ws, bool full_wg, LsapArgs& a, size_t& lds, int& threads) {
+  const size_t mx = (size_t)(nr > nc ? nr : nc), mn = (size_t)(nr < nc ? nr : nc);
+  a = LsapArgs{cost, nr, nc, row_mask, row_ind, col_ind, n_match, (double*)ws, (int*)((double*)ws + mn + 2 * mx)};
+  a.col_mask = col_mask;
+  const size_t dbytes = (mn + 2 * mx) * sizeof(double), ibytes = ((size_t)nr + (size_t)nc + 5 * mx + 2 * mn) * sizeof(int);
+  lds = 0;
+  constexpr size_t LSAP_LDS_MAX = 156 * 1024;
+  a.cost_lds_off = -1;
+  a.use_lds = 0; a.lds_int_off = 0; a.prestaged = 0;
+  if (dbytes + ibytes <= LSAP_LDS_MAX) {
+    NEAT_CHECK(lds_limit<Kern>((int)LSAP_LDS_MAX));
+    a.use_lds = 1; a.lds_int_off = (int)dbytes; lds = (dbytes + ibytes + 15) & ~(size_t)15;
+    const size_t cbytes = (size_t)nr * nc * sizeof(float);
+    if (lds + cbytes <= LSAP_LDS_MAX) { a.cost_lds_off = (int)lds; lds += cbytes; }
+  }
+  a.onewave = g_lsap_path == 2 || (g_lsap_path == 1 && mn <= LSAP_WAVE_MAX_SMALL && mx <= LSAP_WAVE_MAX_LARGE && a.cost_lds_off >= 0);
+  if (full_wg) threads = LSAP_WG;
+  else if (a.onewave) {
+    threads = a.cost_lds_off >= 0 ? (int)(((size_t)nr * nc / 16 + 63) / 64 * 64) : 64;
+  } else {
+    threads = (int)((mx + 1) / 2 + 63) / 64 * 64;
+  }
+  threads = threads < 64 ? 64 : (threads > LSAP_WG ? LSAP_WG : threads);
+  return 0;
+}
+
 }
 
 int neat_aux_set_tuning(int key, int value) {
   if (key == 28 && (value == 0 || value == 1)) { g_ffn_mfma = value; return 0; }
   if (key == 30 && value >= 0 && value <= 7) { g_sampler_ablate = value; return 0; }
+  if (key == 31 && value >= 0 && value <= 2) { g_lsap_path = value; return 0; }
   return -1;
 }
 
@@ -458,22 +489,44 @@
   if (nr < 0 || nc < 0 || !n_match) return -1;
   if (nr == 0 || nc == 0) return (int)hipMemsetAsync(n_match, 0, sizeof(int), (hipStream_t)stream);
   if (!cost || !row_ind || !col_ind || !ws) return -1;
-  const size_t mx = (size_t)(nr > nc ? nr : nc), mn = (size_t)(nr < nc ? nr : nc);
-  LsapArgs a{cost, nr, nc, row_mask, row_ind, col_ind, n_match, (double*)ws, (int*)((double*)ws + mn + 2 * mx)};
-  a.col_mask = col_mask;
-  const size_t dbytes = (mn + 2 * mx) * sizeof(double), ibytes = ((size_t)nr + (size_t)nc + 5 * mx + 2 * mn) * sizeof(int);
-  size_t lds = 0;
-  constexpr size_t LSAP_LDS_MAX = 156 * 1024;
-  a.cost_lds_off = -1;
-  if (dbytes + ibytes <= LSAP_LDS_MAX) {
-    NEAT_CHECK(lds_limit<&lsap_kernel>((int)LSAP_LDS_MAX));
-    a.use_lds = 1; a.lds_int_off = (int)dbytes; lds = (dbytes + ibytes + 15) & ~(size_t)15;
-    const size_t cbytes = (size_t)nr * nc * sizeof(float);
-    if (lds + cbytes <= LSAP_LDS_MAX) { a.cost_lds_off = (int)lds; lds += cbytes; }
-  }
-  int threads = (int)((mx + 1) / 2 + 63) / 64 * 64;
-  threads = threads < 64 ? 64 : (threads > LSAP_WG ? LSAP_WG : threads);
+  LsapArgs a; size_t lds; int threads;
+  const int e = lsap_plan<&lsap_kernel>(cost, nr, nc, row_mask, col_mask, row_ind, col_ind, n_match, ws, false, a, lds, threads);
+  if (e != 0) return e;
   hipLaunchKernelGGL(lsap_kernel, dim3(1), dim3(threads), lds, (hipStream_t)stream, a);
+  return (int)hipGetLastError();
+}
+
+int neat_junction_match(const float* cand2d, const float* gt2d, int V, int C, const unsigned char* cand_mask, const float* cand3d,
+                        const float* cand2d_calib, int use_median, float* cost, long long* rows, long long* cols, int* n_match,
+                        float* median, unsigned char* good, float* j3d, float* j2d, float* j2d_calib, void* ws, void* stream) {
+  if (V <= 0 || C <= 0 || V > 2048 || C > 2048) return -1;
+  if (!cand2d || !gt2d || !cand3d || !cand2d_calib || !cost || !rows || !cols || !n_match || !good || !j3d || !j2d || !j2d_calib || !ws ||
+      (use_median && !median)) return -1;
+  JunctionMatchArgs a;
+  a.cand2d = cand2d; a.gt2d = gt2d;
+  size_t lds; int threads;
+  const int e = lsap_plan<&junction_match_kernel>(cost, V, C, nullptr, cand_mask, rows, cols, n_match, ws, true, a.l, lds, threads);
+  if (e != 0) return e;
+  if (!a.l.use_lds) return -1;
+  a.l.prestaged = a.l.cost_lds_off >= 0 ? 1 : 0;
+  a.g = JunctionGateArgs{rows, cols, V < C ? V : C, cost, C, cand3d, cand2d, cand2d_calib, use_median, median, good, j3d, j2d, j2d_calib};
+  hipLaunchKernelGGL(junction_match_kernel, dim3(1), dim3(threads), lds, (hipStream_t)stream, a);
+  return (int)hipGetLastError();
+}
+
+int neat_loss_match_pairs(const unsigned char* row_mask, int K, long long* ri, long long* ci, int* n_match, const float* loc3,
+                          const float* loc2c, const float* loc2, const float* glo3, const float* glo2c, const float* glo2, int J,
+                          const float* pair_cost, float* scal, float* d_glo3, float* d_glo2c, const float* line_loss, float w_eik,
+                          float w_line, float w_j3, float w_j2, int weighted_grads, float* total, const float* w2c, void* ws, void* stream) {
+  if (K <= 0 || J <= 0 || !ri || !ci || !n_match || !loc3 || !loc2c || !loc2 || !glo3 || !glo2c || !glo2 || !pair_cost || !scal ||
+      !d_glo3 || !d_glo2c || !line_loss || !ws) return -1;
+  LossMatchPairsArgs a;
+  size_t lds; int threads;
+  const int e = lsap_plan<&loss_match_pairs_kernel>(pair_cost, K, J, row_mask, nullptr, ri, ci, n_match, ws, true, a.l, lds, threads);
+  if (e != 0) return e;
+  a.p = LossPairsArgs{ri, ci, n_match, K < J ? K : J, loc3, loc2c, loc2, glo3, glo2c, glo2, J, pair_cost, scal, d_glo3, d_glo2c, line_loss,
+                      w_eik, w_line, w_j3, w_j2, weighted_grads, total, w2c};
+  hipLaunchKernelGGL(loss_match_pairs_kernel, dim3(1), dim3(threads), lds, (hipStream_t)stream, a);
   return (int)hipGetLastError();
 }
 
diff --git a/neat_amd/csrc/neat_net.hip b/neat_amd/csrc/neat_net.hip
--- a/neat_amd/csrc/neat_net.hip
+++ b/neat_amd/csrc/neat_net.hip
@@ -1446,7 +1446,7 @@
 
 int neat_set_tuning(int key, int value) {
 #if !NEAT_HALF
-  if (key == 28 || key == 30) return neat_aux_set_tuning(key, value);
+  if (key == 28 || key == 30 || key == 31) return neat_aux_set_tuning(key, value);
   f16_neat_set_tuning(key, value);
 #endif
   if (key == 0 && (value == 2 || value == 4)) { g_pt_bf16 = value; return 0; }
diff --git a/neat_amd/networks.py b/neat_amd/networks.py
--- a/neat_amd/networks.py
+++ b/neat_amd/networks.py
@@ -513,13 +513,20 @@
                 cand2d_calib = lines2d_calib.detach().reshape(-1, 2)
             gt2d = _device_copy(input["wireframe"][0], "vertices", cand2d.device)
             fused_gate = cand2d.is_cuda and min(gt2d.shape[0], cand2d.shape[0]) <= 2048
-            cost = ops.junction_cost(cand2d, gt2d) if fused_gate else ((cand2d[None] - gt2d[:, None]) ** 2).sum(-1).sqrt()
-            rows, cols, _ = ops.linear_sum_assignment(cost, None, cand_valid)
-            if fused_gate:
+            one_launch = fused_gate and 0 < min(gt2d.shape[0], cand2d.shape[0]) and max(gt2d.shape[0], cand2d.shape[0]) <= 2048
+            if one_launch:
+                cost, rows, cols, _, median, good, j3_pad, j2_pad, j2c_pad = ops.junction_match(cand2d, gt2d, cand_valid, cand3d, cand2d_calib,
+                                                                                               self.use_median)
+                if self.use_median:
+                    output["median"] = median
+            else:
+                cost = ops.junction_cost(cand2d, gt2d) if fused_gate else ((cand2d[None] - gt2d[:, None]) ** 2).sum(-1).sqrt()
+                rows, cols, _ = ops.linear_sum_assignment(cost, None, cand_valid)
+            if fused_gate and not one_launch:
                 median, good, j3_pad, j2_pad, j2c_pad = ops.junction_gate(rows, cols, cost, cand3d, cand2d, cand2d_calib, self.use_median)
                 if self.use_median:
                     output["median"] = median
-            else:
+            elif not fused_gate:
                 if cand_valid is None:
                     matched = cost[rows, cols]
                     pair_ok = None
diff --git a/neat_amd/ops.py b/neat_amd/ops.py
--- a/neat_amd/ops.py
+++ b/neat_amd/ops.py
@@ -786,11 +786,15 @@
                                              _p(scal), _p(d_rgb), _p(d_gth), _p(pair_cost), w_eik, _p(w2c_c), _p(x3_c), _p(d_x3) if fold else None,
                                              _stream()), "neat_loss_lines_terms")
         if have_pairs:
-            ri, ci, n_match = linear_sum_assignment(pair_cost, good)
+            kp = min(K, J)
+            ri, ci = torch.empty(kp, device=dev, dtype=torch.int64), torch.empty(kp, device=dev, dtype=torch.int64)
+            n_match = torch.empty(1, device=dev, dtype=torch.int32)
+            ws = torch.empty(max(int(lib.neat_lsap_ws_bytes(K, J)), 8), device=dev, dtype=torch.uint8)
             loss = torch.empty((), device=dev)
-            _lib.check(lib.neat_loss_pairs(_p(ri), _p(ci), _p(n_match), ri.shape[0], _p(loc3_c), _p(loc2c_c), _p(loc2_c), _p(glo3_c),
-                                           _p(glo2c_c), _p(glo2_c), J, _p(pair_cost), _p(scal), _p(d_glo3), _p(d_glo2c),
-                                           _ip(line3, 1), w_eik, w_line, w_j3, w_j2, 1, _p(loss), _p(w2c_c), _stream()), "neat_loss_pairs")
+            _lib.check(lib.neat_loss_match_pairs(_p(_as_u8(good)), K, _p(ri), _p(ci), _p(n_match), _p(loc3_c), _p(loc2c_c), _p(loc2_c),
+                                                 _p(glo3_c), _p(glo2c_c), _p(glo2_c), J, _p(pair_cost), _p(scal), _p(d_glo3), _p(d_glo2c),
+                                                 _ip(line3, 1), w_eik, w_line, w_j3, w_j2, 1, _p(loss), _p(w2c_c), _p(ws), _stream()),
+                       "neat_loss_match_pairs")
         else:
             loss = scal[0] + w_eik * scal[1] + w_line * line3[1]
         ctx.save_for_backward(flat)
@@ -945,6 +949,27 @@
                                              1 if use_median else 0, _p(median), _p(good), _p(j3d), _p(j2d), _p(j2dc), _stream()),
                "neat_junction_gate")
     return (median.reshape(()) if use_median else None), good.view(torch.bool), j3d, j2d, j2dc
+
+
+def junction_match(cand2d, gt2d, cand_valid, cand3d, cand2d_calib, use_median):
+    lib = _lib.lib()
+    cand2d, gt2d = _f32c(cand2d.detach()), _f32c(gt2d.detach())
+    cand3d, cand2d_calib = _f32c(cand3d.detach()), _f32c(cand2d_calib.detach())
+    V, C = gt2d.shape[0], cand2d.shape[0]
+    K = min(V, C)
+    dev = cand2d.device
+    cost = torch.empty(V, C, device=dev)
+    rows, cols = torch.empty(K, device=dev, dtype=torch.int64), torch.empty(K, device=dev, dtype=torch.int64)
+    n_match = torch.empty(1, device=dev, dtype=torch.int32)
+    median = torch.empty(1, device=dev) if use_median else None
+    good = torch.empty(K, device=dev, dtype=torch.uint8)
+    j3d, j2d, j2dc = torch.empty(K, 3, device=dev), torch.empty(K, 2, device=dev), torch.empty(K, 2, device=dev)
+    cmask = _as_u8(cand_valid)
+    ws = torch.empty(max(int(lib.neat_lsap_ws_bytes(V, C)), 8), device=dev, dtype=torch.uint8)
+    _lib.check(lib.neat_junction_match(_p(cand2d), _p(gt2d), V, C, _p(cmask), _p(cand3d), _p(cand2d_calib), 1 if use_median else 0,
+                                       _p(cost), _p(rows), _p(cols), _p(n_match), _p(median), _p(good), _p(j3d), _p(j2d), _p(j2dc), _p(ws),
+                                       _stream()), "neat_junction_match")
+    return cost, rows, cols, n_match, (median.reshape(()) if use_median else None), good.view(torch.bool), j3d, j2d, j2dc
 
 
 def _i32(t):
```
